# sair-lab/AirSLAM

Hardware: AMD Instinct MI355X
Metric: stereo detect+match pairs/sec (2x PLNet @512x512 internal: points + lines, junctions on the left + LightGlue match) (higher is better)
Workload: dtype fp16

## Files before the change

### airslam_amd/_lib.py

```python
from __future__ import annotations

import ctypes as C
import os

_HERE = os.path.dirname(os.path.abspath(__file__))
LIB_PATH = os.path.join(_HERE, "libairfe.so")


class Tuning(C.Structure):
    _fields_ = [(n, C.c_int) for n in (
        "fuse_lg_block", "gemm_small_max_m", "gemm8_min_m", "gemmr_min_m", "gemmr_wgs", "qkv_pair", "block_min_m", "lgb_tokens", "sg_kenc_gemm",
        "fold_qkv", "overlap_lines", "kf_graph", "kf_spec_rows", "fuse_dec", "assign_fused", "fold_out_proj", "desc_gather_stream", "copy_wgs")] + [("reserved", C.c_int * 5)]


class Cfg(C.Structure):
    _fields_ = [
        ("device", C.c_int), ("precision", C.c_int), ("max_batch", C.c_int), ("enc_chunk", C.c_int),
        ("max_keypoints", C.c_int), ("keypoint_threshold", C.c_float), ("remove_borders", C.c_int),
        ("nms_radius", C.c_int), ("line_threshold", C.c_float), ("line_length_threshold", C.c_float),
        ("matcher", C.c_int), ("image_width", C.c_int), ("image_height", C.c_int), ("sinkhorn_iters", C.c_int),
        ("superpoint_pack", C.c_char_p), ("plnet_s1_pack", C.c_char_p), ("lightglue_pack", C.c_char_p),
        ("superglue_pack", C.c_char_p), ("matcher_precision", C.c_int), ("line_precision", C.c_int), ("check_launches", C.c_int),
        ("tuning", C.POINTER(Tuning)),
    ]


class Stage0(C.Structure):
    _fields_ = [(n, C.c_void_p) for n in (
        "juncs_pred", "lines_pred", "iskeep", "idx_junc_to_end_min", "idx_junc_to_end_max",
        "loi_features", "loi_features_thin", "loi_features_aux")]


class BowdbFilter(C.Structure):
    _fields_ = [("ratio", C.c_float), ("min_words", C.c_int), ("d_max_index", C.c_void_p), ("d_exclude", C.c_void_p), ("exclude_words", C.c_int)]


class RelocCfg(C.Structure):
    _fields_ = [("ratio", C.c_float), ("min_words", C.c_int), ("K", C.c_int), ("outlier_rejection", C.c_int), ("min_inlier", C.c_int),
                ("pose_refinement", C.c_int), ("cam", C.c_double * 5), ("thr", C.c_double * 2)]


class LoopCfg(C.Structure):
    _fields_ = [("ratio", C.c_float), ("min_words", C.c_int), ("K", C.c_int), ("outlier_rejection", C.c_int), ("distance_rate", C.c_double),
                ("min_matches", C.c_int), ("min_points", C.c_int), ("min_inliers", C.c_int), ("cam", C.c_double * 5), ("thr", C.c_double * 2)]


class SeqPolicy(C.Structure):
    _fields_ = [("min_init_stereo_feature", C.c_int), ("min_num_match", C.c_int), ("max_num_match", C.c_int), ("tracking_point_rate", C.c_float),
                ("tracking_parallax_rate", C.c_float), ("min_x_diff", C.c_double), ("max_x_diff", C.c_double), ("max_y_diff", C.c_double),
                ("image_width", C.c_int), ("image_height", C.c_int)]


class SeqFrame(C.Structure):
    _fields_ = ([(n, C.c_int) for n in ("frame_type", "candidate", "promoted", "dropped", "enough_match", "good_stereo_point", "n_left", "n_right", "n_lines_left",
                                        "n_lines_right", "n_junctions", "n_stereo", "n_matches")] + [("_pad", C.c_int)]
                + [(n, C.c_void_p) for n in ("features_left", "features_right", "lines_left", "lines_right", "junctions", "stereo_idx", "stereo_score", "matches_idx",
                                             "matches_score")])


class DebugLinearArgs(C.Structure):
    _fields_ = ([(n, C.c_int) for n in ("prec", "M", "K", "K1", "N")] + [(n, C.c_void_p) for n in ("x1", "x2", "w", "b")]
                + [("epi", C.c_int), ("act", C.c_int), ("rowidx", C.c_void_p), ("src_rows", C.c_int), ("rot_cos", C.c_void_p), ("rot_sin", C.c_void_p),
                   ("Np", C.c_int), ("H", C.c_int), ("x32", C.c_void_p), ("d2s_hc", C.c_int), ("d2s_wc", C.c_int), ("flag", C.c_void_p),
                   ("kernel", C.c_int), ("gr_wgs", C.c_int), ("out", C.c_void_p), ("out2", C.c_void_p)])


class DebugLgBlockArgs(C.Structure):
    _fields_ = ([("prec", C.c_int), ("M", C.c_int)] + [(n, C.c_void_p) for n in ("attn", "x32", "xb", "wo", "bo", "w1", "b1", "gamma", "beta", "w2", "b2")]
                + [(n, C.c_int) for n in ("relu", "tokens_per_wg", "mixed", "nqk_n")]
                + [(n, C.c_void_p) for n in ("nqk_w", "nqk_b", "nv_w", "nv_b", "rot_cos", "rot_sin")]
                + [("Np", C.c_int)] + [(n, C.c_void_p) for n in ("q", "k", "vt")] + [("rows_past", C.c_int * 5)])


class DebugConvArgs(C.Structure):
    _fields_ = ([(n, C.c_void_p) for n in ("x", "img", "w1a", "b1a", "w", "b")] + [(n, C.c_int) for n in ("cin", "cout", "B", "H", "W", "pool", "out_pad", "relu", "wgs")]
                + [("y_words", C.c_size_t), ("y_raw", C.c_void_p)])


class DebugLgPrepareArgs(C.Structure):
    _fields_ = ([(n, C.c_int) for n in ("prec", "B", "cap", "ld", "kp_off", "normalize")] + [(n, C.c_float) for n in ("cx", "cy", "linv")]
                + [(n, C.c_void_p) for n in ("f0", "f1", "n0", "n1", "wr", "f0x", "f1x")] + [(n, C.c_int) for n in ("n0x", "n1x", "slack_rows", "rows")]
                + [(n, C.c_void_p) for n in ("x32", "xb", "rot_cos", "rot_sin", "lens")] + [("rows_past", C.c_int)])


class DebugLgAssignArgs(C.Structure):
    _fields_ = ([(n, C.c_int) for n in ("prec", "B", "n")] + [(n, C.c_void_p) for n in ("md", "x32", "w")] + [("b", C.c_float), ("lens", C.c_void_p), ("cap", C.c_int),
                ("thr", C.c_float), ("form", C.c_int)]
                + [(n, C.c_void_p) for n in ("pad", "z", "sim", "scores", "rowlse", "collse", "rowval", "rowarg", "colarg", "idx", "score", "nmatch")])


class DebugAttentionArgs(C.Structure):
    _fields_ = ([(n, C.c_int) for n in ("prec", "S", "H", "n", "cross")] + [(n, C.c_void_p) for n in ("q", "k", "v", "lens")]
                + [("canary", C.c_int), ("raw", C.c_int), ("out", C.c_void_p), ("Np", C.c_int), ("rows_past", C.c_int)])


class DebugDetectorTailArgs(C.Structure):
    _fields_ = ([(n, C.c_int) for n in ("B", "Bs", "h", "w", "cap")] + [(n, C.c_void_p) for n in ("heat", "act", "feat", "feat1", "n", "n1", "nms_map", "keep", "cand_cnt")]
                + [("nms_map_written", C.c_int)])


class DebugLinePostArgs(C.Structure):
    _fields_ = ([(n, C.c_int) for n in ("B", "nj", "ld", "h", "w", "capL", "capJ", "from_plane")]
                + [(n, C.c_void_p) for n in ("la", "sc", "m2", "heat", "lines", "nlines", "nfound", "junc", "njunc", "jfound", "jmap")])


class DebugLineMidArgs(C.Structure):
    _fields_ = ([(n, C.c_int) for n in ("B", "j2l", "s1_form", "wgs")]
                + [(n, C.c_void_p) for n in ("juncs_pred", "lines_pred", "thin", "aux", "loi", "iskeep_in", "idx_min_in", "idx_max_in", "iskeep", "idx_min", "idx_max", "counts",
                                             "keep", "pairs", "rep", "head4", "prop4", "ridx", "proj", "lines_adjusted", "scores_line", "table_dirty")])


class DebugS0DecodeArgs(C.Structure):
    _fields_ = ([(n, C.c_int) for n in ("B", "mode", "ld", "off", "want_ta8", "want_loi", "want_jnms", "prec", "wgs")] + [(n, C.c_void_p) for n in ("rows", "x", "w", "b")]
                + [("stage_floats", C.c_size_t)] + [(n, C.c_void_p) for n in ("stage", "jloc", "joff", "jnms", "ta8", "loi", "head_rows")])


SIGNATURES = {
    "airfe_copy_rows_dev": (C.c_int, [C.c_void_p, C.c_int, C.c_void_p, C.c_void_p, C.c_void_p, C.c_void_p, C.c_void_p, C.c_void_p]),
    "airfe_pack_rows_dev": (C.c_int, [C.c_void_p, C.c_int, C.c_void_p, C.c_void_p, C.c_void_p, C.c_void_p, C.c_void_p, C.c_void_p, C.c_void_p]),
    "airfe_seq_default_policy": (None, [C.POINTER(SeqPolicy)]),
    "airfe_seq_add_keyframe_check": (C.c_int, [C.POINTER(SeqPolicy), C.c_void_p, C.c_int, C.c_void_p, C.c_int, C.c_void_p, C.c_int]),
    "airfe_seq_good_stereo_points": (C.c_int, [C.POINTER(SeqPolicy), C.c_void_p, C.c_void_p, C.c_void_p, C.c_int]),
    "airfe_seq_create": (C.c_int, [C.c_void_p, C.c_void_p, C.c_int, C.POINTER(SeqPolicy), C.c_int, C.c_int, C.c_void_p, C.c_void_p, C.c_void_p, C.POINTER(C.c_void_p)]),
    "airfe_seq_destroy": (None, [C.c_void_p]),
    "airfe_seq_last_error": (C.c_char_p, [C.c_void_p]),
    "airfe_seq_begin": (C.c_int, [C.c_void_p, C.c_void_p, C.c_void_p, C.c_int, C.c_int, C.c_int, C.c_size_t]),
    "airfe_seq_end": (C.c_int, [C.c_void_p, C.POINTER(SeqFrame)]),
    "airfe_seq_step": (C.c_int, [C.c_void_p, C.c_void_p, C.c_void_p, C.c_int, C.c_int, C.c_int, C.c_size_t, C.POINTER(SeqFrame)]),
    "airfe_seq_stream": (C.c_void_p, [C.c_void_p]),
    "airfe_seq_set_outlier_rejection": (C.c_int, [C.c_void_p, C.c_int]),
    "airfe_seq_wall_split": (C.c_int, [C.c_void_p, C.POINTER(C.c_double), C.POINTER(C.c_double), C.POINTER(C.c_double), C.POINTER(C.c_int), C.POINTER(C.c_int)]),
    "airfe_default_cfg": (None, [C.POINTER(Cfg)]),
    "airfe_default_tuning": (None, [C.POINTER(Tuning)]),
    "airfe_debug_fail_next_launch": (C.c_int, [C.c_void_p, C.c_int]),
    "airfe_create": (C.c_int, [C.POINTER(Cfg), C.POINTER(C.c_void_p)]),
    "airfe_destroy": (None, [C.c_void_p]),
    "airfe_last_error": (C.c_char_p, [C.c_void_p]),
    "airfe_detect_points": (C.c_int, [C.c_void_p, C.c_void_p, C.c_int, C.c_int, C.c_int, C.c_void_p, C.c_int,
                                      C.POINTER(C.c_int)]),
    "airfe_has_line_branch": (C.c_int, [C.c_void_p]),
    "airfe_detect_plnet": (C.c_int, [C.c_void_p, C.c_void_p, C.c_int, C.c_int, C.c_int, C.POINTER(Stage0), C.c_void_p,
                                     C.c_int, C.POINTER(C.c_int), C.c_void_p, C.c_int, C.POINTER(C.c_int), C.c_void_p,
                                     C.c_int, C.POINTER(C.c_int), C.c_int]),
    "airfe_stereo_keyframe": (C.c_int, [C.c_void_p, C.c_void_p, C.c_void_p, C.c_int, C.c_int, C.c_int, C.c_void_p, C.c_void_p, C.c_int,
                                        C.POINTER(C.c_int), C.POINTER(C.c_int), C.c_void_p, C.c_void_p, C.c_int, C.POINTER(C.c_int),
                                        C.POINTER(C.c_int), C.c_void_p, C.c_int, C.POINTER(C.c_int), C.c_void_p, C.c_void_p, C.c_int,
                                        C.POINTER(C.c_int)]),
    "airfe_stereo_keyframe_tracked": (C.c_int, [C.c_void_p, C.c_void_p, C.c_void_p, C.c_int, C.c_int, C.c_int, C.c_void_p, C.c_void_p, C.c_int,
                                                C.POINTER(C.c_int), C.POINTER(C.c_int), C.c_void_p, C.c_void_p, C.c_int, C.POINTER(C.c_int),
                                                C.POINTER(C.c_int), C.c_void_p, C.c_int, C.POINTER(C.c_int), C.c_void_p, C.c_void_p, C.c_int,
                                                C.POINTER(C.c_int), C.c_void_p, C.c_int, C.c_void_p, C.c_void_p, C.POINTER(C.c_int)]),
    "airfe_track_frame": (C.c_int, [C.c_void_p, C.c_void_p, C.c_int, C.c_int, C.c_int, C.c_void_p, C.c_int, C.c_void_p, C.c_int, C.POINTER(C.c_int),
                                    C.c_void_p, C.c_void_p, C.c_int, C.POINTER(C.c_int)]),
    "airfe_promote_frame": (C.c_int, [C.c_void_p, C.c_void_p, C.c_int, C.c_int, C.c_int, C.c_void_p, C.c_int, C.POINTER(C.c_int), C.c_void_p, C.c_void_p, C.c_int,
                                      C.POINTER(C.c_int)]),
    "airfe_adopt_reference": (C.c_int, [C.c_void_p]),
    "airfe_match_lightglue": (C.c_int, [C.c_void_p, C.c_void_p, C.c_int, C.c_void_p, C.c_int, C.c_void_p, C.c_void_p,
                                        C.c_int, C.POINTER(C.c_int)]),
    "airfe_match_superglue": (C.c_int, [C.c_void_p, C.c_void_p, C.c_int, C.c_void_p, C.c_int, C.c_void_p, C.c_void_p,
                                        C.c_void_p, C.c_void_p]),
    "airfe_assign_points_to_lines": (C.c_int, [C.c_void_p, C.c_void_p, C.c_int, C.c_void_p, C.c_int, C.c_void_p, C.c_void_p,
                                               C.c_void_p, C.c_int, C.c_void_p]),
    "airfe_match_lines": (C.c_int, [C.c_void_p, C.c_void_p, C.c_void_p, C.c_int, C.c_int, C.c_void_p, C.c_void_p, C.c_int, C.c_int,
                                    C.c_void_p, C.c_int, C.c_void_p]),
    "airfe_bow_load": (C.c_int, [C.c_void_p, C.c_void_p, C.c_void_p, C.c_void_p, C.c_void_p, C.c_void_p, C.c_int]),
    "airfe_bow_transform": (C.c_int, [C.c_void_p, C.c_void_p, C.c_int, C.c_void_p, C.c_void_p]),
    "airfe_bow_transform_dev": (C.c_int, [C.c_void_p, C.c_void_p, C.c_int, C.c_void_p, C.c_void_p, C.c_void_p]),
    "airfe_bow_vector": (C.c_int, [C.c_void_p, C.c_void_p, C.c_int, C.c_void_p, C.c_void_p, C.POINTER(C.c_int), C.c_void_p]),
    "airfe_bow_vector_batch_dev": (C.c_int, [C.c_void_p, C.c_void_p, C.c_void_p, C.c_int, C.c_int] + [C.c_void_p] * 5),
    "airfe_bowdb_create": (C.c_int, [C.c_void_p, C.c_int, C.c_int, C.c_int, C.POINTER(C.c_void_p)]),
    "airfe_bowdb_destroy": (C.c_int, [C.c_void_p]),
    "airfe_bowdb_clear": (C.c_int, [C.c_void_p]),
    "airfe_bowdb_size": (C.c_int, [C.c_void_p]),
    "airfe_bowdb_add_batch_dev": (C.c_int, [C.c_void_p] * 6 + [C.c_int, C.c_int, C.c_void_p]),
    "airfe_bowdb_add": (C.c_int, [C.c_void_p] * 6 + [C.c_int, C.c_int]),
    "airfe_bowdb_query_batch_dev": (C.c_int, [C.c_void_p] * 4 + [C.c_int, C.c_int, C.POINTER(BowdbFilter)] + [C.c_void_p] * 3 + [C.c_int] + [C.c_void_p] * 4),
    "airfe_bowdb_topk_dev": (C.c_int, [C.c_void_p] * 4 + [C.c_int, C.c_int, C.c_int, C.c_void_p, C.c_void_p, C.c_void_p]),
    "airfe_bowdb_match_candidates_batch_dev": (C.c_int, [C.c_void_p] * 4 + [C.c_int, C.c_int, C.c_void_p, C.c_int, C.c_int] + [C.c_void_p] * 3 + [C.c_int] + [C.c_void_p] * 3),
    "airfe_bowdb_attach_map": (C.c_int, [C.c_void_p, C.c_int]),
    "airfe_bowdb_set_points_dev": (C.c_int, [C.c_void_p, C.c_int, C.c_int, C.c_void_p, C.c_void_p]),
    "airfe_bowdb_set_points": (C.c_int, [C.c_void_p, C.c_int, C.c_int, C.c_void_p]),
    "airfe_bowdb_get_points": (C.c_int, [C.c_void_p, C.c_int, C.c_int, C.c_void_p]),
    "airfe_bowdb_set_covisibility": (C.c_int, [C.c_void_p, C.c_void_p, C.c_void_p, C.c_void_p, C.c_int]),
    "airfe_bowdb_get_covisibility": (C.c_int, [C.c_void_p, C.c_void_p, C.c_void_p, C.c_void_p, C.c_int, C.POINTER(C.c_int)]),
    "airfe_bowdb_set_positions": (C.c_int, [C.c_void_p, C.c_int, C.c_int, C.c_void_p]),
    "airfe_bowdb_group_dev": (C.c_int, [C.c_void_p, C.c_int] + [C.c_void_p] * 3 + [C.c_int] * 3 + [C.c_void_p] * 8),
    "airfe_relocalize_batch_dev": (C.c_int, [C.c_void_p, C.c_void_p, C.POINTER(RelocCfg), C.c_void_p, C.c_void_p, C.c_int, C.c_int] + [C.c_void_p] * 9 +
                                   [C.c_int] + [C.c_void_p] * 3),
    "airfe_bowdb_set_poses": (C.c_int, [C.c_void_p, C.c_int, C.c_int, C.c_void_p]),
    "airfe_bowdb_get_poses": (C.c_int, [C.c_void_p, C.c_int, C.c_int, C.c_void_p]),
    "airfe_bowdb_set_u_right_dev": (C.c_int, [C.c_void_p, C.c_int, C.c_int, C.c_void_p, C.c_void_p]),
    "airfe_bowdb_set_u_right": (C.c_int, [C.c_void_p, C.c_int, C.c_int, C.c_void_p]),
    "airfe_bowdb_get_u_right": (C.c_int, [C.c_void_p, C.c_int, C.c_int, C.c_void_p]),
    "airfe_bowdb_attach_point_ids": (C.c_int, [C.c_void_p, C.c_int]),
    "airfe_bowdb_set_point_ids_dev": (C.c_int, [C.c_void_p, C.c_int, C.c_int, C.c_void_p, C.c_void_p]),
    "airfe_bowdb_set_point_ids": (C.c_int, [C.c_void_p, C.c_int, C.c_int, C.c_void_p]),
    "airfe_bowdb_get_point_ids": (C.c_int, [C.c_void_p, C.c_int, C.c_int, C.c_void_p]),
    "airfe_bowdb_build_covisibility_dev": (C.c_int, [C.c_void_p, C.c_void_p, C.c_void_p]),
    "airfe_bowdb_build_covisibility": (C.c_int, [C.c_void_p, C.POINTER(C.c_int)]),
    "airfe_bowdb_query_stored_batch_dev": (C.c_int, [C.c_void_p, C.c_void_p, C.c_int, C.c_float, C.c_int, C.c_int] + [C.c_void_p] * 3 + [C.c_int] +
                                           [C.c_void_p] * 4),
    "airfe_loop_detect_batch_dev": (C.c_int, [C.c_void_p, C.c_void_p, C.POINTER(LoopCfg), C.c_void_p, C.c_int] + [C.c_void_p] * 10 + [C.c_int] +
                                    [C.c_void_p] * 3),
    "airfe_set_rectify_maps": (C.c_int, [C.c_void_p, C.c_int, C.c_void_p, C.c_void_p, C.c_int, C.c_int]),
    "airfe_rectify_detect_points": (C.c_int, [C.c_void_p, C.c_int, C.c_void_p, C.c_int, C.c_int, C.c_int, C.c_void_p, C.c_void_p, C.c_int,
                                              C.POINTER(C.c_int)]),
    "airfe_rectify_batch_dev": (C.c_int, [C.c_void_p, C.c_int, C.c_void_p, C.c_int, C.c_int, C.c_int, C.c_int, C.c_size_t, C.c_void_p,
                                          C.c_int, C.c_size_t, C.c_void_p]),
    "airfe_detect_points_batch_dev": (C.c_int, [C.c_void_p, C.c_void_p, C.c_int, C.c_int, C.c_int, C.c_int, C.c_size_t,
                                                C.c_void_p, C.c_int, C.c_void_p, C.c_void_p]),
    "airfe_match_lightglue_batch_dev": (C.c_int, [C.c_void_p, C.c_void_p, C.c_void_p, C.c_void_p, C.c_void_p, C.c_int,
                                                  C.c_int, C.c_void_p, C.c_void_p, C.c_int, C.c_void_p, C.c_void_p]),
    "airfe_match_superglue_batch_dev": (C.c_int, [C.c_void_p, C.c_void_p, C.c_void_p, C.c_void_p, C.c_void_p, C.c_int, C.c_int,
                                                  C.c_void_p, C.c_void_p, C.c_void_p, C.c_void_p, C.c_void_p]),
    "airfe_stereo_batch_dev": (C.c_int, [C.c_void_p, C.c_void_p, C.c_void_p, C.c_int, C.c_int, C.c_int, C.c_int,
                                         C.c_size_t, C.c_void_p, C.c_void_p, C.c_int, C.c_void_p, C.c_void_p, C.c_void_p,
                                         C.c_void_p, C.c_int, C.c_void_p, C.c_void_p]),
    "airfe_detect_plnet_batch_dev": (C.c_int, [C.c_void_p, C.c_void_p, C.c_int, C.c_int, C.c_int, C.c_int, C.c_size_t, C.c_void_p,
                                               C.c_int, C.c_void_p, C.c_void_p, C.c_int, C.c_void_p, C.c_void_p, C.c_int, C.c_void_p,
                                               C.c_int, C.c_void_p, C.c_void_p]),
    "airfe_stereo_plnet_batch_dev": (C.c_int, [C.c_void_p, C.c_void_p, C.c_void_p, C.c_int, C.c_int, C.c_int, C.c_int, C.c_size_t,
                                               C.c_void_p, C.c_void_p, C.c_int, C.c_void_p, C.c_void_p, C.c_void_p, C.c_int, C.c_void_p,
                                               C.c_void_p, C.c_int, C.c_void_p, C.c_void_p, C.c_void_p, C.c_void_p, C.c_int, C.c_void_p,
                                               C.c_void_p]),
    "airfe_debug_plnet_j2l": (C.c_int, [C.c_void_p, C.c_int, C.c_void_p, C.c_void_p, C.c_void_p]),
    "airfe_assign_points_to_lines_batch_dev": (C.c_int, [C.c_void_p, C.c_void_p, C.c_void_p, C.c_int, C.c_void_p, C.c_void_p, C.c_int, C.c_int,
                                                         C.c_void_p, C.c_void_p, C.c_void_p, C.c_int, C.c_void_p, C.c_void_p]),
    "airfe_match_lines_batch_dev": (C.c_int, [C.c_void_p] + [C.c_void_p] * 8 + [C.c_int, C.c_int, C.c_void_p, C.c_void_p, C.c_int, C.c_int,
                                              C.c_void_p, C.c_void_p, C.c_void_p, C.c_int, C.c_void_p, C.c_void_p]),
    "airfe_fundamental_ransac": (C.c_int, [C.c_void_p, C.c_void_p, C.c_int, C.c_void_p, C.c_int, C.c_void_p, C.c_void_p, C.c_int, C.POINTER(C.c_int)]),
    "airfe_fundamental_ransac_batch_dev": (C.c_int, [C.c_void_p, C.c_void_p, C.c_void_p, C.c_void_p, C.c_void_p, C.c_int, C.c_int, C.c_void_p, C.c_void_p,
                                                     C.c_int, C.c_void_p, C.c_void_p, C.c_void_p]),
    "airfe_set_outlier_rejection": (C.c_int, [C.c_void_p, C.c_int]),
    "airfe_pnp_ransac": (C.c_int, [C.c_void_p, C.c_void_p, C.c_void_p, C.c_int, C.c_void_p, C.c_void_p, C.c_void_p, C.c_void_p, C.POINTER(C.c_int)]),
    "airfe_pnp_ransac_batch_dev": (C.c_int, [C.c_void_p, C.c_void_p, C.c_void_p, C.c_void_p, C.c_int, C.c_int, C.c_void_p, C.c_void_p, C.c_void_p,
                                             C.c_void_p, C.c_void_p, C.c_void_p]),
    "airfe_stereo_points": (C.c_int, [C.c_void_p, C.c_void_p, C.c_void_p, C.c_int, C.c_void_p, C.c_int, C.c_void_p, C.c_int, C.c_void_p, C.c_void_p,
                                      C.c_void_p, C.POINTER(C.c_int)]),
    "airfe_stereo_points_batch_dev": (C.c_int, [C.c_void_p] * 6 + [C.c_int, C.c_int, C.c_void_p, C.c_void_p, C.c_int] + [C.c_void_p] * 5),
    "airfe_stereo_lines": (C.c_int, [C.c_void_p, C.c_void_p, C.c_void_p, C.c_int, C.c_void_p, C.c_int] + [C.c_void_p] * 8),
    "airfe_stereo_lines_batch_dev": (C.c_int, [C.c_void_p] * 6 + [C.c_int, C.c_void_p, C.c_void_p, C.c_int] + [C.c_void_p] * 7),
    "airfe_stereo_line_landmarks_batch_dev": (C.c_int, [C.c_void_p] * 6 + [C.c_int] + [C.c_void_p] * 4 + [C.c_int, C.c_void_p, C.c_void_p, C.c_int,
                                                        C.c_void_p, C.c_int] + [C.c_void_p] * 8 + [C.c_int] + [C.c_void_p] * 8),
    "airfe_track_pose_batch_dev": (C.c_int, [C.c_void_p, C.c_void_p, C.c_void_p, C.c_int, C.c_void_p, C.c_int, C.c_void_p, C.c_void_p, C.c_int, C.c_int,
                                             C.c_void_p, C.c_void_p, C.c_void_p, C.c_void_p, C.c_void_p]),
    "airfe_frame_optimize": (C.c_int, [C.c_void_p, C.c_void_p, C.c_void_p, C.c_int] + [C.c_void_p] * 7 + [C.POINTER(C.c_int)]),
    "airfe_frame_optimize_batch_dev": (C.c_int, [C.c_void_p, C.c_void_p, C.c_void_p, C.c_void_p, C.c_int, C.c_int] + [C.c_void_p] * 9),
    "airfe_track_pose_opt_batch_dev": (C.c_int, [C.c_void_p, C.c_void_p, C.c_void_p, C.c_int, C.c_void_p, C.c_int, C.c_void_p, C.c_int, C.c_void_p,
                                                 C.c_void_p, C.c_int, C.c_int] + [C.c_void_p] * 9),
    "airfe_sync": (C.c_int, [C.c_void_p]),
    "airfe_superglue_status": (C.c_int, [C.c_void_p, C.c_void_p]),
    "airfe_profile_enable": (C.c_int, [C.c_void_p, C.c_int]),
    "airfe_profile_stages": (C.c_int, []),
    "airfe_profile_stage_name": (C.c_char_p, [C.c_int]),
    "airfe_profile_read": (C.c_int, [C.c_void_p, C.c_void_p, C.c_void_p, C.c_void_p, C.c_void_p]),
    "airfe_debug_detector_maps": (C.c_int, [C.c_void_p, C.c_int, C.c_void_p, C.c_void_p, C.c_void_p]),
    "airfe_debug_lightglue_scores": (C.c_int, [C.c_void_p, C.c_void_p, C.c_int, C.c_void_p, C.c_int, C.c_void_p]),
    "airfe_debug_superglue_scores": (C.c_int, [C.c_void_p, C.c_void_p, C.c_int, C.c_void_p, C.c_int, C.c_void_p]),
    "airfe_debug_lg_filter": (C.c_int, [C.c_void_p, C.c_void_p, C.c_int, C.c_int, C.c_void_p, C.c_void_p, C.c_int, C.POINTER(C.c_int)]),
    "airfe_debug_sg_decode": (C.c_int, [C.c_void_p, C.c_void_p, C.c_int, C.c_int, C.c_void_p, C.c_void_p, C.c_void_p, C.c_void_p]),
    "airfe_debug_sg_sinkhorn": (C.c_int, [C.c_void_p, C.c_void_p, C.c_void_p, C.c_int, C.c_int, C.c_float, C.c_int, C.c_int, C.c_void_p, C.POINTER(C.c_int)]),
    "airfe_debug_detector_tail": (C.c_int, [C.c_void_p, C.POINTER(DebugDetectorTailArgs)]),
    "airfe_debug_line_post": (C.c_int, [C.c_void_p, C.POINTER(DebugLinePostArgs)]),
    "airfe_debug_junctions_topk": (C.c_int, [C.c_void_p, C.c_void_p, C.c_void_p, C.c_int, C.c_void_p]),
    "airfe_debug_line_mid": (C.c_int, [C.c_void_p, C.POINTER(DebugLineMidArgs)]),
    "airfe_debug_s0_decode": (C.c_int, [C.c_void_p, C.POINTER(DebugS0DecodeArgs)]),
    "airfe_debug_lg_prepare": (C.c_int, [C.c_void_p, C.POINTER(DebugLgPrepareArgs)]),
    "airfe_debug_lg_assign": (C.c_int, [C.c_void_p, C.POINTER(DebugLgAssignArgs)]),
    "airfe_debug_plnet_stage0": (C.c_int, [C.c_void_p] + [C.c_void_p] * 10),
    "airfe_debug_plnet_s1": (C.c_int, [C.c_void_p, C.POINTER(Stage0), C.c_void_p, C.c_void_p, C.c_int, C.POINTER(C.c_int)]),
    "airfe_debug_plnet_s1_last": (C.c_int, [C.c_void_p, C.c_void_p, C.c_void_p, C.c_int, C.POINTER(C.c_int)]),
    "airfe_debug_preprocess": (C.c_int, [C.c_void_p, C.c_void_p, C.c_int, C.c_int, C.c_int, C.c_void_p]),
    "airfe_debug_conv3x3": (C.c_int, [C.c_void_p, C.c_void_p, C.c_int, C.c_int, C.c_int, C.c_int, C.c_void_p, C.c_void_p,
                                      C.c_int, C.c_int, C.c_void_p]),
    "airfe_debug_conv": (C.c_int, [C.c_void_p, C.POINTER(DebugConvArgs)]),
    "airfe_debug_trace": (C.c_int, [C.c_void_p, C.c_int]),
    "airfe_debug_trace_stop": (C.c_int, [C.c_void_p, C.c_int]),
    "airfe_debug_trace_buffer": (C.c_int, [C.c_void_p, C.c_int, C.c_void_p, C.c_size_t]),
    "airfe_debug_trace_slots": (C.c_int, [C.c_void_p]),
    "airfe_debug_trace_slot": (C.c_int, [C.c_void_p, C.c_int, C.c_char_p, C.c_int, C.POINTER(C.c_uint), C.POINTER(C.c_uint), C.POINTER(C.c_uint)]),
    "airfe_debug_trace_read": (C.c_int, [C.c_void_p, C.c_void_p, C.c_void_p, C.c_void_p]),
    "airfe_debug_gemm": (C.c_int, [C.c_void_p, C.c_void_p, C.c_int, C.c_int, C.c_void_p, C.c_void_p, C.c_int, C.c_int,
                                   C.c_void_p]),
    "airfe_debug_linear": (C.c_int, [C.c_void_p, C.POINTER(DebugLinearArgs)]),
    "airfe_debug_qkv": (C.c_int, [C.c_void_p] + [C.c_int] * 3 + [C.c_void_p] * 3 + [C.c_int] + [C.c_void_p] * 4 + [C.c_int] * 2 + [C.c_void_p] * 3),
    "airfe_debug_lg_block": (C.c_int, [C.c_void_p, C.POINTER(DebugLgBlockArgs)]),
    "airfe_debug_ln_gelu": (C.c_int, [C.c_void_p, C.c_int, C.c_void_p, C.c_void_p, C.c_void_p, C.c_int]),
    "airfe_debug_attention_args": (C.c_int, [C.c_void_p, C.POINTER(DebugAttentionArgs)]),
    "airfe_debug_attention": (C.c_int, [C.c_void_p, C.c_void_p, C.c_void_p, C.c_void_p, C.c_void_p, C.c_int, C.c_int, C.c_int, C.c_int, C.c_void_p]),
}

_lib = None


def lib() -> C.CDLL:
    global _lib
    if _lib is None:
        if not os.path.exists(LIB_PATH):
            raise RuntimeError(
                f"{LIB_PATH} is missing: build it with `python -m airslam_amd.build` "
                "(hipcc, gfx950).  airslam_amd has no CPU fallback.")
        try:
            import torch
        except Exception:
            pass
        l = C.CDLL(LIB_PATH)
        for name, (res, args) in SIGNATURES.items():
            fn = getattr(l, name)
            fn.restype = res
            fn.argtypes = args
        _lib = l
    return _lib
```

### airslam_amd/api.py

```python
from __future__ import annotations

import ctypes as C
import os
import tempfile
from typing import Dict, Optional

import numpy as np

from . import _lib, weights as W

FEAT = 259


def _pack_arg(x, tmpfiles) -> Optional[bytes]:
    if x is None:
        return None
    if isinstance(x, (str, bytes, os.PathLike)):
        return os.fsencode(x)
    f = tempfile.NamedTemporaryFile(suffix=".airfe", delete=False)
    f.close()
    W.save_pack(f.name, x)
    tmpfiles.append(f.name)
    return f.name.encode()

# ... 355 lines not shown
        n0, n1 = np.ascontiguousarray(n0, np.int32), np.ascontiguousarray(n1, np.int32)
        b, cap, ld = f0.shape
        bt = 2 if second is not None else b
        rows = 2 * bt * self.np_rows + int(slack_rows)
        out = {"x32": np.empty((rows, 256), np.float32), "xb": np.empty((rows, 256), np.float32), "rot_cos": np.empty((rows, 32), np.float32),
               "rot_sin": np.empty((rows, 32), np.float32), "lens": np.empty((2 * bt,), np.int32)}
        cx, cy, linv = normalize if normalize is not None else (0.0, 0.0, 1.0)
        a = _lib.DebugLgPrepareArgs(prec=prec, B=b, cap=cap, ld=ld, kp_off=kp_off, normalize=int(normalize is not None), cx=cx, cy=cy, linv=linv,
                                    f0=f0.ctypes.data, f1=f1.ctypes.data, n0=n0.ctypes.data, n1=n1.ctypes.data, wr=wr.ctypes.data, slack_rows=int(slack_rows),
                                    rows=rows, **{k: v.ctypes.data for k, v in out.items()})
        if second is not None:
            x0, x1 = f32(second[0]).reshape(-1, ld), f32(second[1]).reshape(-1, ld)
            k0, k1 = np.zeros((max(len(x0), 1), ld), np.float32), np.zeros((max(len(x1), 1), ld), np.float32)
            k0[:len(x0)], k1[:len(x1)] = x0, x1
            a.f0x, a.f1x, a.n0x, a.n1x = k0.ctypes.data, k1.ctypes.data, len(x0), len(x1)
        self._chk(self._l.airfe_debug_lg_prepare(self._h, C.byref(a)), "airfe_debug_lg_prepare")
        out["rows_past"], out["Np"] = int(a.rows_past), self.np_rows
        return out

    def debug_lg_assign(self, md, x32, lens, w, b, prec, form, cap=None, thr=0.1, pad=None):
        f32 = lambda t: np.ascontiguousarray(t, np.float32)
        md, x32, w = f32(md), f32(x32), f32(w)
        lens = np.ascontiguousarray(lens, np.int32).reshape(-1)
        s, n, _ = md.shape
        bb = s // 2
        cap = self.np_rows if cap is None else int(cap)
        out = {"z": np.empty((s, n), np.float32), "sim": np.empty((bb, n, n), np.float32), "scores": np.empty((bb, n, n), np.float32),
               "rowlse": np.empty((bb, n), np.float32), "collse": np.empty((bb, n), np.float32), "rowval": np.empty((bb, n), np.float32),
               "rowarg": np.empty((bb, n), np.int32), "colarg": np.empty((bb, n), np.int32), "idx": np.empty((bb, cap, 2), np.int32),
               "score": np.empty((bb, cap), np.float32), "nmatch": np.empty((bb,), np.int32)}
        assert x32.shape == md.shape and len(lens) == s and s % 2 == 0
        a = _lib.DebugLgAssignArgs(prec=prec, B=bb, n=n, md=md.ctypes.data, x32=x32.ctypes.data, w=w.ctypes.data, b=float(b), lens=lens.ctypes.data, cap=cap,
                                   thr=float(thr), form=int(form), **{k: v.ctypes.data for k, v in out.items()})
        if pad is not None:
            pad = f32(pad)
            a.pad = pad.ctypes.data
        self._chk(self._l.airfe_debug_lg_assign(self._h, C.byref(a)), "airfe_debug_lg_assign")
        return out

    def detector_maps(self, b: int = 1):
        heat = np.empty((b, 512, 512), np.float32)
        nms = np.empty((b, 512, 512), np.float32)
        desc = np.empty((b, 64, 64, 256), np.float32)
        self._chk(self._l.airfe_debug_detector_maps(self._h, b, heat.ctypes.data, nms.ctypes.data, desc.ctypes.data),
                  "airfe_debug_detector_maps")
        return heat, nms, desc

    def debug_detector_tail(self, heat, act, cap, Bs=0, h=512, w=512, sentinel=7.0, want_keep=True):
        heat, act = np.ascontiguousarray(heat, np.float32), np.ascontiguousarray(act, np.float32)
        b = heat.shape[0]
        assert heat.shape == (b, 512, 512) and act.shape == (b, 64, 64, 256)
        b0 = Bs if Bs else b
        feat, n = np.full((b0, cap, FEAT), sentinel, np.float32), np.full((b0,), -1, np.int32)
        feat1, n1 = np.full((b - b0, cap, FEAT), sentinel, np.float32), np.full((b - b0,), -1, np.int32)
        nms = np.full((b, 512, 512), np.nan, np.float32)
        keep = np.zeros((b, 64, 64), np.uint64) if want_keep and self.cfg.nms_radius == 4 else None
        cnt = np.full((b,), -1, np.int32)
        a = _lib.DebugDetectorTailArgs(B=b, Bs=int(Bs), h=int(h), w=int(w), cap=int(cap), heat=heat.ctypes.data, act=act.ctypes.data, feat=feat.ctypes.data, n=n.ctypes.data,
                                       nms_map=nms.ctypes.data, cand_cnt=cnt.ctypes.data)
        if Bs:
            a.feat1, a.n1 = feat1.ctypes.data, n1.ctypes.data
        if keep is not None:
            a.keep = keep.ctypes.data
        self._chk(self._l.airfe_debug_detector_tail(self._h, C.byref(a)), "airfe_debug_detector_tail")
        return {"feat": np.concatenate([feat, feat1]), "n": np.concatenate([n, n1]), "cand_cnt": cnt, "keep": keep, "nms_map": nms if a.nms_map_written else None}

    def debug_line_post(self, la, sc, m2, heat, cap_lines, cap_junctions, nj=None, from_plane=False, h=512, w=512, sentinel=7.0, jmap=None):
        la, sc, heat = np.ascontiguousarray(la, np.float32), np.ascontiguousarray(sc, np.float32), np.ascontiguousarray(heat, np.float32)
        m2 = np.ascontiguousarray(m2, np.int32).reshape(-1)
        b, ld = sc.shape
        nj = b if nj is None else int(nj)
        assert la.shape == (b, ld, 4) and heat.shape == (b, 512, 512) and len(m2) == b
        out = {"lines": np.full((b, cap_lines, 4), sentinel, np.float64), "nlines": np.full((b,), -1, np.int32), "nfound": np.full((b,), -1, np.int32),
               "junc": np.full((nj, cap_junctions, FEAT), sentinel, np.float32), "njunc": np.full((nj,), -1, np.int32), "jfound": np.full((nj,), -1, np.int32)}
        a = _lib.DebugLinePostArgs(B=b, nj=nj, ld=ld, h=int(h), w=int(w), capL=int(cap_lines), capJ=int(cap_junctions), from_plane=int(bool(from_plane)), la=la.ctypes.data,
                                   sc=sc.ctypes.data, m2=m2.ctypes.data, heat=heat.ctypes.data, **{k: v.ctypes.data for k, v in out.items()})
        if jmap is not None:
            jmap = np.ascontiguousarray(jmap, np.uint8)
            assert jmap.shape == (nj, 512, 512)
            a.jmap = jmap.ctypes.data
        self._chk(self._l.airfe_debug_line_post(self._h, C.byref(a)), "airfe_debug_line_post")
        return out

    def debug_line_mid(self, juncs_pred, lines_pred, thin, aux, loi, iskeep=None, idx_min=None, idx_max=None, j2l=0, s1_form=2, wgs=0):
        f = lambda x: np.ascontiguousarray(x, np.float32)
        juncs_pred, lines_pred, thin, aux, loi = f(juncs_pred), f(lines_pred), f(thin), f(aux), f(loi)
        b, n, cap = juncs_pred.shape[0], 3 * 128 * 128, 45056
        assert juncs_pred.shape == (b, 300, 2) and lines_pred.shape == (b, n, 4) and thin.shape == aux.shape == (b, 4, 128, 128) and loi.shape == (b, 128 * 128, 128)
        poison = lambda shape, dt: np.full(shape, -1, np.int32).view(dt) if dt == np.float32 else np.full(shape, -1, np.int32)
        out = {"iskeep": poison((b, n), np.float32), "idx_min": poison((b, n), np.float32), "idx_max": poison((b, n), np.float32), "counts": poison((b, 2), np.int32),
               "keep": poison((b, n), np.int32), "pairs": poison((b, cap, 2), np.int32), "rep": poison((b, cap), np.int32), "head4": poison((b, cap, 4), np.float32),
               "prop4": poison((b, cap, 4), np.float32), "ridx": poison((b, 300, 4), np.int32), "proj": poison((b, 300, 256), np.float32),
               "lines_adjusted": poison((b, cap, 4), np.float32), "scores_line": poison((b, cap), np.float32), "table_dirty": poison((b,), np.int32)}
        a = _lib.DebugLineMidArgs(B=b, j2l=int(j2l), s1_form=int(s1_form), wgs=int(wgs), juncs_pred=juncs_pred.ctypes.data, lines_pred=lines_pred.ctypes.data,
                                  thin=thin.ctypes.data, aux=aux.ctypes.data, loi=loi.ctypes.data, **{k: v.ctypes.data for k, v in out.items()})
        ins = [None if x is None else f(x) for x in (iskeep, idx_min, idx_max)]
        for name, x in zip(("iskeep_in", "idx_min_in", "idx_max_in"), ins):
            if x is not None:
                assert x.shape == (b, n)
                setattr(a, name, x.ctypes.data)
        self._chk(self._l.airfe_debug_line_mid(self._h, C.byref(a)), "airfe_debug_line_mid")
        return out

    S0_STAGE = {"lines_pred": (600, 3 * 16384 * 4), "thin": (600 + 7 * 3 * 16384, 4 * 16384), "aux": (600 + 7 * 3 * 16384 + 4 * 16384, 4 * 16384)}
    S0_STAGE_FLOATS = (600 + 7 * 3 * 16384 + 8 * 16384 + 63) // 64 * 64

    def debug_s0_decode(self, rows=None, ld=160, off=128, ta8=True, loi=False, jnms=True, x=None, w=None, b=None, prec=1, wgs=0, two_pass=False):
        f = lambda t: np.ascontiguousarray(t, np.float32)
        npx, sf = 128 * 128, self.S0_STAGE_FLOATS
        a = _lib.DebugS0DecodeArgs(want_ta8=int(bool(ta8)), want_loi=int(bool(loi)), want_jnms=int(bool(jnms)), prec=int(prec), wgs=int(wgs), stage_floats=sf)
        if rows is not None:
            assert x is None and not two_pass
            rows = f(rows)
            bb = rows.shape[0]
            assert rows.shape == (bb, npx, ld)
            a.mode, a.ld, a.off, a.rows = 0, int(ld), int(off), rows.ctypes.data
        else:
            x, w, b = f(x), f(w), f(b)
            bb = x.shape[0] // npx
            assert x.shape == (bb * npx, 128) and w.shape == (17, 128) and b.shape == (17,)
            a.mode, a.x, a.w, a.b = (2 if two_pass else 1), x.ctypes.data, w.ctypes.data, b.ctypes.data
        poison = lambda *shape: np.full(shape, -1, np.int32).view(np.float32)
        out = {"stage": poison(bb, sf), "jloc": poison(bb, 128, 128), "joff": poison(bb, 2, 128, 128), "jnms": poison(bb, 128, 128), "ta8": poison(bb, npx, 8),
               "loi": poison(128, 128, 128)}
        if two_pass:
            out["head_rows"] = poison(bb, npx, 32)
        a.B = bb
        for k, v in out.items():
            setattr(a, k, v.ctypes.data)
        self._chk(self._l.airfe_debug_s0_decode(self._h, C.byref(a)), "airfe_debug_s0_decode")
        for k, (o, n) in self.S0_STAGE.items():
            v = out["stage"][:, o:o + n]
            out[k] = v.reshape(bb, 3 * npx, 4) if k == "lines_pred" else v.reshape(bb, 4, 128, 128)
        return out

    def debug_junctions_topk(self, jloc, joff):
        jloc, joff = np.ascontiguousarray(jloc, np.float32), np.ascontiguousarray(joff, np.float32)
        b = jloc.shape[0]
        assert jloc.shape == (b, 128, 128) and joff.shape == (b, 2, 128, 128)
        out = np.full((b, 300, 2), np.nan, np.float32)
        self._chk(self._l.airfe_debug_junctions_topk(self._h, jloc.ctypes.data, joff.ctypes.data, b, out.ctypes.data), "airfe_debug_junctions_topk")
        return out

    def debug_preprocess(self, gray):
        gray = np.ascontiguousarray(gray, np.uint8)
        out = np.empty((512, 512), np.float32)
        self._chk(self._l.airfe_debug_preprocess(self._h, gray.ctypes.data, gray.shape[0], gray.shape[1], gray.strides[0],
                                                 out.ctypes.data), "airfe_debug_preprocess")
        return out

    def debug_conv3x3(self, x, w, b, pool=False):
        x = np.ascontiguousarray(x, np.float32); w = np.ascontiguousarray(w, np.float32); b = np.ascontiguousarray(b, np.float32)
        bb, cin, hh, ww = x.shape
        cout = w.shape[0]
        ho, wo = (hh // 2, ww // 2) if pool else (hh, ww)
        y = np.empty((bb, cout, ho, wo), np.float32)
        self._chk(self._l.airfe_debug_conv3x3(self._h, x.ctypes.data, bb, cin, hh, ww, w.ctypes.data, b.ctypes.data, cout,
                                              int(pool), y.ctypes.data), "airfe_debug_conv3x3")
        return y

    def debug_conv(self, w, b, prec, x=None, img=None, w1a=None, b1a=None, pool=False, out_pad=1, relu=True, wgs=256):
        f32 = lambda t: None if t is None else np.ascontiguousarray(t, np.float32)
        x, img, w1a, b1a, w, b = map(f32, (x, img, w1a, b1a, w, b))
        src = x if x is not None else img
        bb, hh, ww = src.shape[0], src.shape[-2], src.shape[-1]
        cout, cin = w.shape[0], w.shape[1]
# ... 698 lines not shown
```

### airslam_amd/csrc/airfe.hip

```cpp
#include "airfe_host.h"

namespace airfe_host {
thread_local std::string g_err;

int fail(airfe_ctx* c, const std::string& m) {
  if (c) c->err = m;
  g_err = m;
  return 1;
}

int fail_noexcept(airfe_ctx* c, const char* what, const char* detail) noexcept {
  try {
    std::string m = std::string("airfe: C++ exception at the C boundary (") + what + "): " + (detail ? detail : "unknown");
    if (c) c->err = m;
    g_err = m;
  } catch (...) {
  }
  return 1;
}

int launch_status(airfe_ctx* c) {
  std::string m;
  if (c->launch_err.empty()) {
    const hipError_t e = hipGetLastError();
// ... 705 lines not shown


int airfe_has_line_branch(const airfe_ctx* c) { return c && c->has_s0 && c->has_s1; }

static int upload_stage0(airfe_ctx* c, const airfe_plnet_stage0* s0, hipStream_t st) {
  c->wf_counted = false;
  const size_t NP = KEEP_CAP;
  float* d = c->s0_stage;
  HIPCHK(c, hipMemcpyAsync(d + SG_JUNCS, s0->juncs_pred, 600 * 4, hipMemcpyHostToDevice, st));
  HIPCHK(c, hipMemcpyAsync(d + SG_LP, s0->lines_pred, NP * 16, hipMemcpyHostToDevice, st));
  HIPCHK(c, hipMemcpyAsync(d + SG_KEEP, s0->iskeep, NP * 4, hipMemcpyHostToDevice, st));
  HIPCHK(c, hipMemcpyAsync(d + SG_MIN, s0->idx_junc_to_end_min, NP * 4, hipMemcpyHostToDevice, st));
  HIPCHK(c, hipMemcpyAsync(d + SG_MAX, s0->idx_junc_to_end_max, NP * 4, hipMemcpyHostToDevice, st));
  HIPCHK(c, hipMemcpyAsync(c->s0_loi, s0->loi_features, (size_t)128 * 128 * 128 * 4, hipMemcpyHostToDevice, st));
  HIPCHK(c, hipMemcpyAsync(d + SG_THIN, s0->loi_features_thin, (size_t)4 * 128 * 128 * 4, hipMemcpyHostToDevice, st));
  HIPCHK(c, hipMemcpyAsync(d + SG_AUX, s0->loi_features_aux, (size_t)4 * 128 * 128 * 4, hipMemcpyHostToDevice, st));
  return 0;
}

int airfe_detect_plnet(airfe_ctx* c, const uint8_t* gray, int h, int w, int stride, const airfe_plnet_stage0* s0, float* feat,
                       int cap, int* n, double* lines, int capL, int* nlines, float* junc, int capJ, int* njunc,
                       int want_junctions) try {
  AIRFE_ENTER(c);
  if (nlines) *nlines = 0;
  if (njunc) *njunc = 0;
  const bool lines_on = (s0 || c->has_s0);
  if (!lines_on) return airfe_detect_points(c, gray, h, w, stride, feat, cap, n);
  if (!c->has_s1) return fail(c, "PLNet stage-1 weights were not loaded (cfg.plnet_s1_pack)");
  if (cap < c->cfg.max_keypoints) return fail(c, "feature capacity < max_keypoints");
  hipStream_t st = c->stream;
  if (upload_image(c, gray, h, w, stride)) return 1;
  if (detect_dev(c, c->st_img.p, 1, h, w, stride, (size_t)h * stride, c->st_feat0, c->Np, c->st_n0, st)) return 1;
  if (s0) {
    if (upload_stage0(c, s0, st)) return 1;
  } else if (line_branch_dev(c, st, 0, 1, false)) {
    return 1;
  }
  int* nl_d = c->d_nlines;
  int *nj_d = c->d_njunc, *njf_d = c->d_njunc + c->Lmax;
  if (line_tail_dev(c, 0, 1, s0 ? c->s0_loi : nullptr, h, w, c->d_lines, LINE_CAP, nl_d, nl_d + c->Lmax, c->junc_feat, JUNC_CAP, nj_d, njf_d,
                    want_junctions ? 1 : 0, st))
    return 1;
  const size_t fbytes = 64 + (size_t)c->cfg.max_keypoints * AIRFE_FEAT_DIM * 4;
  if (ensure_pin(c, fbytes + 64)) return 1;
  int* cnt = reinterpret_cast<int*>(c->pin + fbytes);
  cnt[0] = cnt[1] = cnt[2] = 0;
  HIPCHK(c, hipMemcpyAsync(c->pin, c->io_in, fbytes, hipMemcpyDeviceToHost, st));
  HIPCHK(c, hipMemcpyAsync(cnt, nl_d, 4, hipMemcpyDeviceToHost, st));
  if (want_junctions) {
    HIPCHK(c, hipMemcpyAsync(cnt + 1, nj_d, 4, hipMemcpyDeviceToHost, st));
    HIPCHK(c, hipMemcpyAsync(cnt + 2, njf_d, 4, hipMemcpyDeviceToHost, st));
  }
  HIPCHK(c, hipStreamSynchronize(st));
  if (saturation_status(c)) return 1;
  const int nn = std::min(*reinterpret_cast<const int*>(c->pin), c->cfg.max_keypoints);
  if (nn > 0) memcpy(feat, c->pin + 64, (size_t)nn * AIRFE_FEAT_DIM * 4);
  *n = nn;
  const int nl = cnt[0], nj = cnt[1], njf = cnt[2];
  if (njf > JUNC_CAP) return fail(c, "detect_plnet: more junctions than the device arena holds (JUNC_CAP)");
  if (nl > capL || nj > capJ) return fail(c, "detect_plnet: lines / junctions do not fit the caller's buffers (capL, capJ)");
  const size_t lb = (nl > 0 && lines) ? (size_t)nl * 32 : 0, jb = (nj > 0 && junc) ? (size_t)nj * AIRFE_FEAT_DIM * 4 : 0;
  if (lb + jb) {
    if (ensure_pin(c, lb + jb)) return 1;
    if (lb) HIPCHK(c, hipMemcpyAsync(c->pin, c->d_lines, lb, hipMemcpyDeviceToHost, st));
    if (jb) HIPCHK(c, hipMemcpyAsync(c->pin + lb, c->junc_feat, jb, hipMemcpyDeviceToHost, st));
    HIPCHK(c, hipStreamSynchronize(st));
    if (lb) memcpy(lines, c->pin, lb);
    if (jb) memcpy(junc, c->pin + lb, jb);
  }
  if (nlines) *nlines = nl;
  if (njunc) *njunc = nj;
  return 0;
} AIRFE_CATCH(c)

static int plnet_lines_batch(airfe_ctx* c, int B, int h, int w, double* d_lines, int capL, int* d_nlines, float* d_junc, int capJ,
                             int* d_njunc, int nj, int* d_found, hipStream_t st, int phase = 3) {
  if (!c->has_s0 || !c->has_s1) return fail(c, "the batched PLNet path needs the line branch (line.* in the detector pack) and cfg.plnet_s1_pack");
  if (c->prec == 2) return fail(c, "plnet_lines_batch is the 2-byte batch path (fp32 mode goes image by image: plnet_batch_f32)");
  if (B > c->Lmax) return fail(c, "batch exceeds the line-path arena");
  if (capL < 1 || !d_lines || !d_nlines) return fail(c, "detect_plnet_batch: no line output");
  if (nj < 0 || nj > B || (nj > 0 && (!d_junc || !d_njunc || capJ < 1))) return fail(c, "detect_plnet_batch: bad junction arguments");
  if ((phase & 1) && line_branch_dev(c, st, 0, B, false)) return 1;
  bool partial = false;
  if ((phase & 2) && nj > 0 && !c->desc_dense_valid) {
    dense_desc_head(c, nj, st);
    c->desc_dense_valid = true;
    partial = nj != c->last_B;
  }
  int* lfound = d_found ? d_found : c->d_nlines + c->Lmax;
  int* jfound = d_found ? d_found + B : c->d_njunc + c->Lmax;
  const int rc = line_tail_dev(c, 0, B, nullptr, h, w, d_lines, capL, d_nlines, lfound, d_junc, capJ, d_njunc, jfound, nj, st, phase);
  if (partial) c->desc_dense_valid = false;
  return rc;
}

static int plnet_batch_f32(airfe_ctx* c, const uint8_t* d_gray, int B, int h, int w, int stride, size_t img_stride, float* d_feat, int cap, int* d_n,
                           double* d_lines, int capL, int* d_nlines, float* d_junc, int capJ, int* d_njunc, int nj, int* lfound, int* jfound, hipStream_t st) {
  if (!c->has_s0 || !c->has_s1) return fail(c, "the batched PLNet path needs the line branch (line.* in the detector pack) and cfg.plnet_s1_pack");
  if (capL < 1 || !d_lines || !d_nlines) return fail(c, "detect_plnet_batch: no line output");
  if (nj < 0 || nj > B || (nj > 0 && (!d_junc || !d_njunc || capJ < 1))) return fail(c, "detect_plnet_batch: bad junction arguments");
  for (int b = 0; b < B; ++b) {
    const bool jn = b < nj;
    const int rc = detect_dev(c, d_gray + (size_t)b * img_stride, 1, h, w, stride, img_stride, d_feat + (size_t)b * cap * AIRFE_FEAT_DIM, cap, d_n + b, st);
    if (rc || line_branch_dev(c, st, 0, 1, false)) return 1;
    if (line_tail_dev(c, 0, 1, nullptr, h, w, d_lines + (size_t)b * capL * 4, capL, d_nlines + b, lfound ? lfound + b : c->d_nlines + c->Lmax,
                      jn ? d_junc + (size_t)b * capJ * AIRFE_FEAT_DIM : nullptr, capJ, jn ? d_njunc + b : nullptr, jn ? (jfound ? jfound + b : c->d_njunc + c->Lmax) : nullptr,
                      jn ? 1 : 0, st, 3))
      return 1;
  }
  return 0;
}

int airfe_detect_plnet_batch_dev(airfe_ctx* c, const uint8_t* d_gray, int B, int h, int w, int stride, size_t img_stride, float* d_feat,
                                 int cap, int* d_n, double* d_lines, int capL, int* d_nlines, float* d_junc, int capJ, int* d_njunc,
                                 int junction_images, int* d_found, void* stream) try {
  AIRFE_ENTER(c);
  hipStream_t st = stream ? (hipStream_t)stream : c->stream;
  if (c->prec == 2)
    return plnet_batch_f32(c, d_gray, B, h, w, stride, img_stride, d_feat, cap, d_n, d_lines, capL, d_nlines, d_junc, capJ, d_njunc, junction_images, d_found,
                           d_found ? d_found + B : nullptr, st);
  if (detect_dev(c, d_gray, B, h, w, stride, img_stride, d_feat, cap, d_n, st)) return 1;
  return plnet_lines_batch(c, B, h, w, d_lines, capL, d_nlines, d_junc, capJ, d_njunc, junction_images, d_found, st);
} AIRFE_CATCH(c)

static int stereo_plnet_dev(airfe_ctx* c, const uint8_t* d_left, const uint8_t* d_right, int B, int h, int w, int stride,
                            size_t img_stride, float* d_featL, float* d_featR, int cap, int* d_nL, int* d_nR, double* d_lines,
                            int capL, int* d_nlines, float* d_juncL, int capJ, int* d_njuncL, int* d_found, int32_t* d_idx,
                            float* d_score, int mcap, int* d_nmatch, hipStream_t st, const std::function<int(hipStream_t)>* after_detect = nullptr,
                            const std::function<int(hipStream_t)>* after_lines = nullptr, const LgSecondPair* x2 = nullptr) {
  if (c->prec == 2) {
    if (x2) return fail(c, "stereo_plnet_batch: the second (temporal) pair rides in a 2-byte forward (precision fp16 / bf16)");
    if (plnet_batch_f32(c, d_left, B, h, w, stride, img_stride, d_featL, cap, d_nL, d_lines, capL, d_nlines, d_juncL, capJ, d_njuncL, d_juncL ? B : 0, d_found,
                        d_found ? d_found + 2 * B : nullptr, st) ||
        plnet_batch_f32(c, d_right, B, h, w, stride, img_stride, d_featR, cap, d_nR, d_lines + (size_t)B * capL * 4, capL, d_nlines + B, nullptr, 0, nullptr, 0,
                        d_found ? d_found + B : nullptr, nullptr, st))
      return 1;
    if (after_detect && (*after_detect)(st)) return 1;
    if (after_lines && (*after_lines)(st)) return 1;
    if (!d_idx) return 0;
    return lightglue_dev(c, d_featL, d_nL, d_featR, d_nR, B, cap, AIRFE_FEAT_DIM, 1, 1, d_idx, d_score, mcap, d_nmatch, nullptr, st, nullptr);
  }
  if (!(2 * B <= c->Dmax))
    return fail(c, "stereo_plnet_batch: needs the one-pass stereo detector (detector + LightGlue packs loaded, 2 B <= 2 max_batch)");
  const uint32_t enc_only = (1u << ST_PREPROCESS) | (1u << ST_CONV1_FUSED) | (1u << ST_CONV3X3_C64);
  const bool overlap = c->overlap_lines && (c->prof_mask & ~enc_only) == 0;
  if (detect_dev2(c, d_left, d_right, B, h, w, stride, img_stride, d_featL, d_featR, cap, d_nL, d_nR, st)) return 1;
  if (after_detect && (!d_idx || !overlap) && (*after_detect)(st)) return 1;
  if (!d_idx) {
    if (plnet_lines_batch(c, 2 * B, h, w, d_lines, capL, d_nlines, d_juncL, capJ, d_njuncL, d_juncL ? B : 0, d_found, st)) return 1;
    return after_lines ? (*after_lines)(st) : 0;
  }
  if (!overlap) {
    if (plnet_lines_batch(c, 2 * B, h, w, d_lines, capL, d_nlines, d_juncL, capJ, d_njuncL, d_juncL ? B : 0, d_found, st)) return 1;
    if (after_lines && (*after_lines)(st)) return 1;
    return lightglue_dev(c, d_featL, d_nL, d_featR, d_nR, B, cap, AIRFE_FEAT_DIM, 1, 1, d_idx, d_score, mcap, d_nmatch, nullptr, st, x2);
  }
  HIPCHK(c, hipEventRecord(c->ev_fork, st));
  HIPCHK(c, hipStreamWaitEvent(c->stream2, c->ev_fork, 0));
  int rc = 0;
  if (after_detect && (*after_detect)(c->stream2)) rc = 1;
  const bool lg_first = B <= 4;
  if (!rc && lg_first) rc = lightglue_dev(c, d_featL, d_nL, d_featR, d_nR, B, cap, AIRFE_FEAT_DIM, 1, 1, d_idx, d_score, mcap, d_nmatch, nullptr, st, x2);
  if (!rc) rc = plnet_lines_batch(c, 2 * B, h, w, d_lines, capL, d_nlines, d_juncL, capJ, d_njuncL, d_juncL ? B : 0, d_found, c->stream2);
  if (!rc && after_lines && (*after_lines)(c->stream2)) rc = 1;
  if (!rc && !lg_first) rc = lightglue_dev(c, d_featL, d_nL, d_featR, d_nR, B, cap, AIRFE_FEAT_DIM, 1, 1, d_idx, d_score, mcap, d_nmatch, nullptr, st, x2);
  HIPCHK(c, hipEventRecord(c->ev_join, c->stream2));
  HIPCHK(c, hipStreamWaitEvent(st, c->ev_join, 0));
// ... 509 lines not shown
```

### airslam_amd/csrc/airfe_debug.hip

```cpp
#include "airfe_host.h"

struct DbgTmp {
  airfe_ctx h;
  DbgTmp() {}
  explicit DbgTmp(int prec) { h.prec = h.pack_prec = prec; }
  ~DbgTmp() { for (void* p : h.allocs) (void)hipFree(p); }
};

static std::vector<uint16_t> dbg_conv_x(const float* x, int B, int cin, int H, int W, int prec) {
  std::vector<uint16_t> xin((size_t)B * (H + 2) * (W + 2) * cin, 0);
  for (int bb = 0; bb < B; ++bb)
    for (int ci = 0; ci < cin; ++ci)
      for (int yy = 0; yy < H; ++yy)
        for (int xx = 0; xx < W; ++xx)
          xin[(((size_t)bb * (H + 2) + yy + 1) * (W + 2) + xx + 1) * cin + ci] = cvt2(x[(((size_t)bb * cin + ci) * H + yy) * W + xx], prec);
  return xin;
}
static std::vector<uint16_t> dbg_conv_slabs(const float* w, int cin, int cout, int prec) {
  const int nci = cin / 64;
  return pack_slabs(cout / 64, 9 * nci, prec, [&](int feat, int s, int k) {
    const int tap = s / nci, cc = s % nci, ci = cc * 64 + k;
    return w[((size_t)feat * cin + ci) * 9 + tap];
  });
}
// ... 13 lines not shown
} AIRFE_CATCH(c)

int airfe_debug_conv3x3(airfe_ctx* c, const float* x, int B, int cin, int H, int W, const float* w, const float* b, int cout,
                        int pool, float* y) try {
  AIRFE_ENTER(c);
  if ((cin != 64 && cin != 128) || cout % 64 || W % 16 || H % 16) return fail(c, "debug_conv3x3: unsupported shape");
  const int prec = c->prec;
  const int Ho = pool ? H / 2 : H, Wo = pool ? W / 2 : W;
  const size_t ywords = (size_t)B * (Ho + 2) * (Wo + 2) * cout;
  DbgTmp t(prec);
  airfe_ctx& tmp = t.h;
  ConvArgs a;
  a.X = dupload(&tmp, dbg_conv_x(x, B, cin, H, W, prec)); a.Wp = dupload(&tmp, dbg_conv_slabs(w, cin, cout, prec));
  a.bias = dupload(&tmp, std::vector<float>(b, b + cout)); a.Y = dalloc<uint16_t>(&tmp, ywords);
  if (!a.X || !a.Wp || !a.bias || !a.Y) return fail(c, "debug_conv3x3: allocation failed");
  a.B = B; a.H = H; a.W = W; a.CIN = cin; a.COUT = cout;
  a.pool = pool; a.out_pad = 1; a.relu = 1;
  launch_conv3x3(prec, a, c->stream);
  HIPCHK(c, hipStreamSynchronize(c->stream));
  std::vector<uint16_t> yo(ywords);
  HIPCHK(c, hipMemcpy(yo.data(), a.Y, ywords * 2, hipMemcpyDeviceToHost));
  for (int bb = 0; bb < B; ++bb)
    for (int co = 0; co < cout; ++co)
      for (int yy = 0; yy < Ho; ++yy)
        for (int xx = 0; xx < Wo; ++xx)
          y[(((size_t)bb * cout + co) * Ho + yy) * Wo + xx] = back2(yo[(((size_t)bb * (Ho + 2) + yy + 1) * (Wo + 2) + xx + 1) * cout + co], prec);
  return 0;
} AIRFE_CATCH(c)

int airfe_debug_fail_next_launch(airfe_ctx* c, int stage) try {
  AIRFE_ENTER(c);
  if (stage < -1 || stage >= ST_COUNT) return fail(c, "debug_fail_next_launch: no such stage");
  c->fail_stage = stage;
  return 0;
} AIRFE_CATCH(c)

int airfe_debug_gemm(airfe_ctx* c, const float* x, int M, int K, const float* w, const float* b, int N, int relu, float* y) try {
  AIRFE_ENTER(c);
  if (K != 128 && K != 256 && K != 512) return fail(c, "debug_gemm: K must be 128, 256 or 512");
  const int prec = c->prec, Mp = (M + 127) / 128 * 128, Np8 = (N + 7) / 8 * 8;
  std::vector<uint16_t> xin((size_t)Mp * K, 0);
  for (size_t i = 0; i < (size_t)M * K; ++i) xin[i] = cvt2(x[i], prec);
  DbgTmp t(prec);
  airfe_ctx& tmp = t.h;
  LinW lw;
  if (!make_linear(&tmp, w, b, K, N, lw)) return fail(c, "debug_gemm: allocation failed");
  uint16_t* dx = dupload(&tmp, xin);
  float* dy = dalloc<float>(&tmp, (size_t)Mp * Np8);
  int rc = 0;
  if (!dx || !dy) rc = fail(c, "debug_gemm: allocation failed");
  if (!rc) {
    GemmArgs g;
    g.X1 = dx; g.ld1 = K; g.K1 = K; g.Wp = lw.w; g.bias = lw.b; g.M = Mp; g.N = N; g.cb_total = lw.cbt;
    g.epi = EPI_STORE_F32; g.act = relu ? ACT_RELU : ACT_NONE; g.out = dy; g.ldo = Np8;
    g.small_max = c->gemm_small_max; g.g8_min = c->gemm8_min; g.gr_min = c->gemmr_min; g.gr_wgs = c->gemmr_wgs;
    launch_gemm(prec, K, false, g, c->stream);
    if (hipStreamSynchronize(c->stream) != hipSuccess) rc = fail(c, "debug_gemm: kernel failed");
  }
  if (!rc) {
    std::vector<float> yo((size_t)Mp * Np8);
    (void)hipMemcpy(yo.data(), dy, yo.size() * 4, hipMemcpyDeviceToHost);
    for (int m = 0; m < M; ++m)
      for (int n = 0; n < N; ++n) y[(size_t)m * N + n] = yo[(size_t)m * Np8 + n];
  }
  return rc;
} AIRFE_CATCH(c)

}

static std::vector<uint16_t> dbg_rows2(const float* x, int rows, int cols, int rows_cap, int prec) {
  std::vector<uint16_t> v((size_t)rows_cap * cols, 0);
  if (x)
    for (size_t i = 0; i < (size_t)rows * cols; ++i) v[i] = cvt2(x[i], prec);
  return v;
}
static std::vector<float> dbg_rows4(const float* x, int rows, int cols, int rows_cap) {
  std::vector<float> v((size_t)rows_cap * cols, 0.f);
  if (x) memcpy(v.data(), x, (size_t)rows * cols * sizeof(float));
  return v;
}
template <class T>
static T* dbg_canary(airfe_ctx* tmp, size_t n) {
  T* p = dalloc<T>(tmp, n, false);
  if (p) (void)hipMemset(p, 0xFF, std::max<size_t>(n, 1) * sizeof(T));
  return p;
}
static void dbg_back2(const std::vector<uint16_t>& v, size_t n, int prec, float* out) {
  for (size_t i = 0; i < n; ++i) out[i] = back2(v[i], prec);
}

extern "C" {

int airfe_debug_conv(airfe_ctx* c, airfe_debug_conv_args* a) try {
  AIRFE_ENTER(c);
  if (!a || !a->w || !a->b || !a->y_raw) return fail(c, "debug_conv: null argument");
  const bool fused = a->img != nullptr;
  if (fused == (a->x != nullptr)) return fail(c, "debug_conv: exactly one of x (plain form) and img (fused conv1a -> conv1b) must be given");
  const int cin = a->cin, cout = a->cout, B = a->B, H = a->H, W = a->W, pool = a->pool, opad = a->out_pad, prec = c->prec;
  if (prec != 0 && prec != 1) return fail(c, "debug_conv: the context's precision must be fp16 or bf16");
  if (a->wgs < 1 || a->wgs > 256) return fail(c, "debug_conv: wgs must lie in 1 .. 256");
  if (cin != 64 && cin != 128) return fail(c, "debug_conv: cin must be 64 or 128");
  if (cout < 64 || cout % 64 || (cin == 128 && cout % 128)) return fail(c, "debug_conv: cout must be a multiple of 64 (of 128 when cin is 128)");
  if (B < 1 || H < 16 || W < 16 || H % 16 || W % 16) return fail(c, "debug_conv: B >= 1, H and W multiples of 16");
  if ((pool != 0 && pool != 1) || (opad != 0 && opad != 1) || (a->relu != 0 && a->relu != 1)) return fail(c, "debug_conv: pool, out_pad and relu are 0 or 1");
  if (pool && !opad) return fail(c, "debug_conv: a pooled layer always feeds another conv (out_pad = 1); pool with out_pad = 0 is no form of the arena");
  if (fused && (cin != 64 || cout != 64 || !pool || !opad || !a->relu || !a->w1a || !a->b1a))
    return fail(c, "debug_conv: the fused form is conv1a -> conv1b: cin = cout = 64, pool = 1, out_pad = 1, relu = 1, w1a and b1a given");
  const int Ho = pool ? H / 2 : H, Wo = pool ? W / 2 : W;
  const size_t guard = (size_t)(Wo + 2 * opad) * cout, words = (size_t)B * (Ho + 2 * opad) * guard, total = words + 2 * guard;
  if (a->y_words != total) return fail(c, "debug_conv: y_words must be (B (Ho + 2 out_pad) + 2) (Wo + 2 out_pad) cout");
  DbgTmp t(prec);
  airfe_ctx& tmp = t.h;
  ConvArgs g;
  if (fused) {
    std::vector<float> im((size_t)B * (H + 2) * (W + 2), 0.f);
    for (int bb = 0; bb < B; ++bb)
      for (int yy = 0; yy < H; ++yy) memcpy(&im[((size_t)bb * (H + 2) + yy + 1) * (W + 2) + 1], a->img + ((size_t)bb * H + yy) * W, (size_t)W * sizeof(float));
    g.img = dupload(&tmp, im);
    g.w1a = dupload(&tmp, std::vector<float>(a->w1a, a->w1a + 64 * 9));
    g.b1a = dupload(&tmp, std::vector<float>(a->b1a, a->b1a + 64));
  } else {
    g.X = dupload(&tmp, dbg_conv_x(a->x, B, cin, H, W, prec));
  }
  g.Wp = dupload(&tmp, dbg_conv_slabs(a->w, cin, cout, prec));
  g.bias = dupload(&tmp, std::vector<float>(a->b, a->b + cout));
  uint16_t* dy = dbg_canary<uint16_t>(&tmp, total);
  if ((fused ? !g.img || !g.w1a || !g.b1a : !g.X) || !g.Wp || !g.bias || !dy) return fail(c, "debug_conv: allocation failed");
  g.Y = dy + guard;
  g.B = B; g.H = H; g.W = W; g.CIN = cin; g.COUT = cout; g.pool = pool; g.out_pad = opad; g.relu = a->relu; g.wgs = a->wgs;
  if (fused) launch_conv64r(prec, g, c->stream);
  else launch_conv3x3(prec, g, c->stream);
  if (hipStreamSynchronize(c->stream) != hipSuccess || launch_status(c)) return fail(c, "debug_conv: kernel failed");
  HIPCHK(c, hipMemcpy(a->y_raw, dy, total * 2, hipMemcpyDeviceToHost));
  return 0;
} AIRFE_CATCH(c)

int airfe_debug_linear(airfe_ctx* c, const airfe_debug_linear_args* a) try {
  AIRFE_ENTER(c);
  if (!a || !a->x1 || !a->w || !a->b || !a->out) return fail(c, "debug_linear: null argument");
  const int prec = a->prec, M = a->M, K = a->K, N = a->N, epi = a->epi, kern = a->kernel, K1 = a->x2 ? a->K1 : K;
  if ((prec != 0 && prec != 1) || M < 1 || N < 1 || (K != 128 && K != 256 && K != 512) || K1 < 32 || K1 % 32 || K1 > K || (a->x2 && K1 == K) ||
      epi < EPI_STORE || epi > EPI_SOFTMAX_D2S || kern < AIRFE_DEBUG_KERNEL_DISPATCH || kern > AIRFE_DEBUG_KERNEL_GEMMR_GATHER128 || (a->act != ACT_NONE && a->act != ACT_RELU))
    return fail(c, "debug_linear: bad argument");
  const bool trans = epi == EPI_HEADS_T, heads = epi == EPI_HEADS || trans, d2s = epi == EPI_SOFTMAX_D2S;
  if (heads && ((a->H != 4 && a->H != 0) || a->Np < 16 || a->Np % 16 || M % a->Np || (epi == EPI_HEADS ? (N != 256 && N != 512) || (N == 512 && !a->out2) : N != 256)))
    return fail(c, "debug_linear: head layouts need H = 4, M = S * Np with Np a multiple of 16, N = 256 (or 512 with out2 for EPI_HEADS)");
  if ((a->rot_cos || a->rot_sin) && (epi != EPI_HEADS || !a->rot_cos || !a->rot_sin)) return fail(c, "debug_linear: rotary is an EPI_HEADS form");
  if (epi == EPI_RESID && (!a->x32 || N % 64)) return fail(c, "debug_linear: EPI_RESID needs x32 and N a multiple of 64");
  if (d2s && (K != 256 || N != 65 || a->x2 || a->rowidx || a->act || a->d2s_hc < 1 || a->d2s_wc < 1 || M % (a->d2s_hc * a->d2s_wc) || M % 16 ||
              (kern != AIRFE_DEBUG_KERNEL_DISPATCH && kern != AIRFE_DEBUG_KERNEL_GEMM8)))
    return fail(c, "debug_linear: EPI_SOFTMAX_D2S is launch_gemm8's head kernel: K = 256, N = 65, dense rows, M = B * hc * wc, M % 16 == 0");
  if (a->rowidx) {
    if (kern != AIRFE_DEBUG_KERNEL_GEMM8 && kern != AIRFE_DEBUG_KERNEL_GEMMR_GATHER && kern != AIRFE_DEBUG_KERNEL_GEMMR_GATHER128)
      return fail(c, "debug_linear: a row gather runs in gemm8, gemmr_gather or gemmr_gather128 only");
    if (a->src_rows < 1) return fail(c, "debug_linear: rowidx needs src_rows");
    for (int r = 0; r < M; ++r)
      if (a->rowidx[r] < 0 || a->rowidx[r] >= a->src_rows) return fail(c, "debug_linear: rowidx entry outside 0 .. src_rows - 1");
  }
  static const int row_tile[7] = {128, 32, 128, 256, 32, 32, 64};
  const int Mp = d2s ? M : (M + row_tile[kern] - 1) / row_tile[kern] * row_tile[kern];
  const int xrows = a->rowidx ? a->src_rows : Mp;
  const int ldo = (epi == EPI_STORE || epi == EPI_STORE_F32) ? (N + 7) / 8 * 8 : N;
  const int Sg = heads ? (Mp + a->Np - 1) / a->Np : 0, S = heads ? M / a->Np : 0;
  DbgTmp t(prec);
  airfe_ctx& tmp = t.h;
  LinW lw;
  if (!make_linear(&tmp, a->w, a->b, K, N, lw)) return fail(c, "debug_linear: allocation failed");
// ... 462 lines not shown
  if (a->h < 1 || a->w < 1 || cap < c->cfg.max_keypoints) return fail(c, "debug_detector_tail: empty image or feature capacity < max_keypoints");
  if (a->keep && c->cfg.nms_radius != 4) return fail(c, "debug_detector_tail: the keep plane exists on the radius-4 path only");
  const size_t px = (size_t)B * R * R, cells = (size_t)B * (R / 8) * (R / 8);
  for (size_t i = 0; i < px; ++i)
    if (!(a->heat[i] >= 0.f && a->heat[i] <= 1.f)) return fail(c, "debug_detector_tail: scores must lie in [0, 1]");
  std::vector<uint16_t> act(cells * 256);
  for (size_t i = 0; i < act.size(); ++i) act[i] = cvt2(a->act[i], c->prec);
  const int B0 = two ? Bs : B, B1 = two ? B - Bs : 0;
  DbgTmp t;
  float* dfeat = dupload(&t.h, std::vector<float>(a->feat, a->feat + (size_t)B0 * cap * AIRFE_FEAT_DIM));
  int* dn = dupload(&t.h, std::vector<int>(a->n, a->n + B0));
  float* dfeat1 = two ? dupload(&t.h, std::vector<float>(a->feat1, a->feat1 + (size_t)B1 * cap * AIRFE_FEAT_DIM)) : nullptr;
  int* dn1 = two ? dupload(&t.h, std::vector<int>(a->n1, a->n1 + B1)) : nullptr;
  if (!dfeat || !dn || (two && (!dfeat1 || !dn1))) return fail(c, "debug_detector_tail: allocation failed");
  hipStream_t st = c->stream;
  clear_saturation(c);
  HIPCHK(c, hipMemcpyAsync(c->heat, a->heat, px * 4, hipMemcpyHostToDevice, st));
  HIPCHK(c, hipMemcpyAsync(c->aDa, act.data(), act.size() * 2, hipMemcpyHostToDevice, st));
  const bool sparse_desc = B > 2 && cap * 4 <= (R / 8) * (R / 8) && cap <= 1024;
  if (!sparse_desc && dense_desc_head(c, B, st)) { (void)hipStreamSynchronize(st); return 1; }
  c->desc_dense_valid = !sparse_desc;
  c->last_B = B;
  const int rc = detect_tail_dev(c, B, Bs, two, sparse_desc, a->h, a->w, dfeat, dfeat1, cap, dn, dn1, st);
  HIPCHK(c, hipStreamSynchronize(st));
  if (rc) return 1;
  if (saturation_status(c)) return 1;
  HIPCHK(c, hipMemcpy(a->feat, dfeat, (size_t)B0 * cap * AIRFE_FEAT_DIM * 4, hipMemcpyDeviceToHost));
  HIPCHK(c, hipMemcpy(a->n, dn, (size_t)B0 * 4, hipMemcpyDeviceToHost));
  if (two) {
    HIPCHK(c, hipMemcpy(a->feat1, dfeat1, (size_t)B1 * cap * AIRFE_FEAT_DIM * 4, hipMemcpyDeviceToHost));
    HIPCHK(c, hipMemcpy(a->n1, dn1, (size_t)B1 * 4, hipMemcpyDeviceToHost));
  }
  a->nms_map_written = c->cfg.nms_radius > 0 && c->nms_map_valid;
  if (a->nms_map && a->nms_map_written) HIPCHK(c, hipMemcpy(a->nms_map, c->heat_nms, px * 4, hipMemcpyDeviceToHost));
  if (a->keep) HIPCHK(c, hipMemcpy(a->keep, c->nms_mask, cells * 8, hipMemcpyDeviceToHost));
  if (a->cand_cnt) HIPCHK(c, hipMemcpy(a->cand_cnt, c->cand_cnt, (size_t)B * 4, hipMemcpyDeviceToHost));
  return 0;
} AIRFE_CATCH(c)

int airfe_debug_line_post(airfe_ctx* c, airfe_debug_line_post_args* a) try {
  AIRFE_ENTER(c);
  if (!c->has_sp || !c->has_s1 || !c->s1_la || !c->jmap) return fail(c, "debug_line_post: the line path is not loaded (cfg.plnet_s1_pack)");
  if (c->cfg.nms_radius != 4) return fail(c, "debug_line_post: both junction score sources exist on the radius-4 path only");
  if (!a || !a->la || !a->sc || !a->m2 || !a->heat || !a->lines || !a->nlines || !a->nfound) return fail(c, "debug_line_post: null argument");
  const int B = a->B, nj = a->nj, ld = a->ld, capL = a->capL, capJ = a->capJ, R = AIRFE_INTERNAL_SIZE;
  if (B < 1 || B > c->Lmax || B > c->Dmax || nj < 0 || nj > B || ld < 1 || ld > LINE_CAP || capL < 1 || capJ < 1 || a->h < 1 || a->w < 1)
    return fail(c, "debug_line_post: bad argument (1 <= B <= the arena's images, 0 <= nj <= B, 1 <= ld <= 45056, capL, capJ >= 1)");
  if (nj > 0 && (!a->junc || !a->njunc || !a->jfound)) return fail(c, "debug_line_post: nj > 0 needs the junction outputs");
  for (int b = 0; b < B; ++b)
    if (a->m2[b] < 0 || a->m2[b] > ld) return fail(c, "debug_line_post: every m2 must lie in 0 .. ld");
  DbgTmp t;
  double* dlines = dupload(&t.h, std::vector<double>(a->lines, a->lines + (size_t)B * capL * 4));
  float* djunc = nj > 0 ? dupload(&t.h, std::vector<float>(a->junc, a->junc + (size_t)nj * capJ * AIRFE_FEAT_DIM)) : nullptr;
  int* dcnt = dbg_canary<int>(&t.h, (size_t)4 * B);
  if (!dlines || (nj > 0 && !djunc) || !dcnt) return fail(c, "debug_line_post: allocation failed");
  hipStream_t st = c->stream;
  clear_saturation(c);
  std::vector<int> counts((size_t)B * LINE_CNT_LD, 0);
  for (int b = 0; b < B; ++b) {
    counts[(size_t)b * LINE_CNT_LD + 1] = a->m2[b];
    HIPCHK(c, hipMemcpyAsync(c->s1_la + (size_t)b * LINE_CAP * 4, a->la + (size_t)b * ld * 4, (size_t)ld * 16, hipMemcpyHostToDevice, st));
    HIPCHK(c, hipMemcpyAsync(c->s1_sc + (size_t)b * LINE_CAP, a->sc + (size_t)b * ld, (size_t)ld * 4, hipMemcpyHostToDevice, st));
  }
  HIPCHK(c, hipMemcpyAsync(c->wf_counts, counts.data(), counts.size() * 4, hipMemcpyHostToDevice, st));
  c->wf_counted = false;
  HIPCHK(c, hipMemcpyAsync(c->heat, a->heat, (size_t)B * R * R * 4, hipMemcpyHostToDevice, st));
  c->nms_map_valid = !a->from_plane;
  launch_nms512_candidates(c->heat, c->nms_map_valid ? c->heat_nms : nullptr, c->nms_mask, B, c->cfg.keypoint_threshold, c->cfg.remove_borders, c->cand, c->cand_cnt,
                           R * R, st);
  const float ws = (float)a->w / (float)R, hs = (float)a->h / (float)R;
  if (nj > 0) launch_zero16(c->jmap, (size_t)nj * R * R, st);
  launch_line_filter(c->s1_la, c->s1_sc, c->wf_counts, c->cfg.remove_borders, c->cfg.line_threshold, c->cfg.line_length_threshold, ws, hs, R, c->jmap, nj, dlines, capL,
                     dcnt, dcnt + B, LINE_CAP, B, st);
  if (nj > 0 && a->jmap) HIPCHK(c, hipMemcpyAsync(c->jmap, a->jmap, (size_t)nj * R * R, hipMemcpyHostToDevice, st));
  if (nj > 0) {
    const bool from_mask = c->cfg.nms_radius > 0 && !c->nms_map_valid;
    const float* hsel = c->cfg.nms_radius > 0 && !from_mask ? c->heat_nms : c->heat;
    const unsigned long long* mask = from_mask ? reinterpret_cast<const unsigned long long*>(c->nms_mask) : nullptr;
    launch_junction_scan(c->jmap, hsel, R, c->cfg.remove_borders, djunc, capJ, dcnt + 2 * B, dcnt + 3 * B, c->d_njunc + 2 * c->Lmax, nj, st, mask);
  }
  HIPCHK(c, hipStreamSynchronize(st));
  if (launch_status(c)) return 1;
  if (saturation_status(c)) return 1;
  HIPCHK(c, hipMemcpy(a->lines, dlines, (size_t)B * capL * 32, hipMemcpyDeviceToHost));
  HIPCHK(c, hipMemcpy(a->nlines, dcnt, (size_t)B * 4, hipMemcpyDeviceToHost));
  HIPCHK(c, hipMemcpy(a->nfound, dcnt + B, (size_t)B * 4, hipMemcpyDeviceToHost));
  if (nj > 0) {
    HIPCHK(c, hipMemcpy(a->junc, djunc, (size_t)nj * capJ * AIRFE_FEAT_DIM * 4, hipMemcpyDeviceToHost));
    HIPCHK(c, hipMemcpy(a->njunc, dcnt + 2 * B, (size_t)nj * 4, hipMemcpyDeviceToHost));
    HIPCHK(c, hipMemcpy(a->jfound, dcnt + 3 * B, (size_t)nj * 4, hipMemcpyDeviceToHost));
  }
  return 0;
} AIRFE_CATCH(c)

int airfe_debug_line_mid(airfe_ctx* c, airfe_debug_line_mid_args* a) try {
  AIRFE_ENTER(c);
  if (!c->has_sp || !c->has_s0 || !c->has_s1 || !c->s0_stage || !c->l_ta8) return fail(c, "debug_line_mid: the line path is not loaded (line.* tensors, cfg.plnet_s1_pack)");
  if (!a || !a->juncs_pred || !a->lines_pred || !a->thin || !a->aux || !a->loi || !a->iskeep || !a->idx_min || !a->idx_max || !a->counts || !a->keep || !a->pairs || !a->rep ||
      !a->head4 || !a->prop4 || !a->ridx || !a->proj || !a->lines_adjusted || !a->scores_line || !a->table_dirty)
    return fail(c, "debug_line_mid: null argument");
  const int B = a->B, form = a->s1_form, NP = KEEP_CAP, NPX = 128 * 128;
  if (B < 1 || B > c->Lmax) return fail(c, "debug_line_mid: 1 <= B <= the arena's images");
  if (a->j2l < 0 || a->j2l > 2 || form < 0 || form > 3) return fail(c, "debug_line_mid: j2l is 0 .. 2, s1_form 0 .. 3");
  if (form <= 1 && B != 1) return fail(c, "debug_line_mid: forms 0 and 1 (CHW tensors, head rows) hold one image");
  if (a->j2l == 0 && (!a->iskeep_in || !a->idx_min_in || !a->idx_max_in)) return fail(c, "debug_line_mid: j2l = 0 needs iskeep_in, idx_min_in and idx_max_in");
  if (a->wgs < 0 || a->wgs > 512) return fail(c, "debug_line_mid: wgs must lie in 0 .. 512");
  if (form == 3)
    for (int i = 0; i < 6; ++i)
      if (!c->s1_wsplit[i]) return fail(c, "debug_line_mid: form 3 needs the split stage-1 weights");
  for (size_t i = 0; i < (size_t)B * 600; ++i)
    if (!std::isfinite(a->juncs_pred[i])) return fail(c, "debug_line_mid: junction coordinates must be finite");
  for (size_t i = 0; i < (size_t)B * NP * 4; ++i)
    if (!std::isfinite(a->lines_pred[i])) return fail(c, "debug_line_mid: proposal coordinates must be finite");
  hipStream_t st = c->stream;
  float* d = c->s0_stage;
  clear_saturation(c);
  std::vector<float> ta8((size_t)B * NPX * 8);
  for (int b = 0; b < B; ++b)
    for (int ch = 0; ch < 8; ++ch) {
      const float* src = (ch < 4 ? a->thin : a->aux) + ((size_t)b * 4 + (ch & 3)) * NPX;
      for (int p = 0; p < NPX; ++p) ta8[((size_t)b * NPX + p) * 8 + ch] = src[p];
    }
  HIPCHK(c, hipMemcpyAsync(c->l_ta8, ta8.data(), ta8.size() * 4, hipMemcpyHostToDevice, st));
  for (int b = 0; b < B; ++b) {
    float* s = d + (size_t)b * SG_STRIDE;
    HIPCHK(c, hipMemcpyAsync(s + SG_JUNCS, a->juncs_pred + (size_t)b * 600, 600 * 4, hipMemcpyHostToDevice, st));
    HIPCHK(c, hipMemcpyAsync(s + SG_LP, a->lines_pred + (size_t)b * NP * 4, (size_t)NP * 16, hipMemcpyHostToDevice, st));
    HIPCHK(c, hipMemcpyAsync(s + SG_THIN, a->thin + (size_t)b * 4 * NPX, (size_t)4 * NPX * 4, hipMemcpyHostToDevice, st));
    HIPCHK(c, hipMemcpyAsync(s + SG_AUX, a->aux + (size_t)b * 4 * NPX, (size_t)4 * NPX * 4, hipMemcpyHostToDevice, st));
    if (a->j2l == 0) {
      HIPCHK(c, hipMemcpyAsync(s + SG_KEEP, a->iskeep_in + (size_t)b * NP, (size_t)NP * 4, hipMemcpyHostToDevice, st));
      HIPCHK(c, hipMemcpyAsync(s + SG_MIN, a->idx_min_in + (size_t)b * NP, (size_t)NP * 4, hipMemcpyHostToDevice, st));
      HIPCHK(c, hipMemcpyAsync(s + SG_MAX, a->idx_max_in + (size_t)b * NP, (size_t)NP * 4, hipMemcpyHostToDevice, st));
    } else {
      HIPCHK(c, hipMemsetAsync(s + SG_KEEP, 0xFF, (size_t)3 * NP * 4, st));
    }
  }
  static_assert(SG_MIN == SG_KEEP + KEEP_CAP && SG_MAX == SG_MIN + KEEP_CAP, "iskeep | min | max are contiguous");
  const size_t L = (size_t)B;
  HIPCHK(c, hipMemsetAsync(c->wf_counts, 0xFF, L * LINE_CNT_LD * 4, st));
  HIPCHK(c, hipMemsetAsync(c->wf_keep, 0xFF, L * KEEP_CAP * 4, st));
  HIPCHK(c, hipMemsetAsync(c->wf_pairs, 0xFF, L * LINE_CAP * 8, st));
  HIPCHK(c, hipMemsetAsync(c->wf_rep, 0xFF, L * LINE_CAP * 4, st));
  HIPCHK(c, hipMemsetAsync(c->wf_prop, 0xFF, L * LINE_CAP * 16, st));
  HIPCHK(c, hipMemsetAsync(c->s1_la, 0xFF, L * LINE_CAP * 16, st));
  HIPCHK(c, hipMemsetAsync(c->s1_sc, 0xFF, L * LINE_CAP * 4, st));
  HIPCHK(c, hipMemsetAsync(c->s1_jfeat, 0xFF, L * 300 * 256 * 4, st));
  HIPCHK(c, hipMemsetAsync(c->l_ridx, 0xFF, L * 1200 * 4, st));
  bool counted = false;
  if (a->j2l) counted = launch_s0_j2l(d + SG_LP, d + SG_JUNCS, 300, NP, 10.0f, d + SG_KEEP, d + SG_MIN, d + SG_MAX, c->wf_counts, B, SG_STRIDE, a->j2l == 1 ? 1 : 0, st);
  if (a->j2l == 2 && !counted) { (void)hipStreamSynchronize(st); return fail(c, "debug_line_mid: the cell search did not leave the per-workgroup counts (the line path's form)"); }
  launch_wireframe(d + SG_KEEP, d + SG_MIN, d + SG_MAX, NP, 300, c->wf_table, c->wf_keep, c->wf_pairs, c->wf_rep, KEEP_CAP, LINE_CAP, c->wf_counts, counted, d + SG_JUNCS,
                   d + SG_LP, c->s1_la, c->wf_prop, B, SG_STRIDE, st);
  c->wf_counted = false;
  HIPCHK(c, hipStreamSynchronize(st));
  if (launch_status(c)) return 1;
  HIPCHK(c, hipMemcpy(a->head4, c->s1_la, L * LINE_CAP * 16, hipMemcpyDeviceToHost));
  if (form != 3) HIPCHK(c, hipMemsetAsync(c->s1_la, 0xFF, L * LINE_CAP * 16, st));
  std::vector<float> chw, head, lrows;
  if (form == 0) {
    chw.resize((size_t)128 * NPX);
    for (int p = 0; p < NPX; ++p)
      for (int ch = 0; ch < 128; ++ch) chw[(size_t)ch * NPX + p] = a->loi[(size_t)p * 128 + ch];
    HIPCHK(c, hipMemcpyAsync(c->s0_loi, chw.data(), chw.size() * 4, hipMemcpyHostToDevice, st));
    launch_plnet_s1(d + SG_JUNCS, d + SG_LP, c->wf_keep, c->wf_pairs, c->wf_rep, c->wf_counts, c->s0_loi, 0, nullptr, nullptr, d + SG_THIN, d + SG_AUX, c->s1_w, c->s1_la,
                    c->s1_sc, KEEP_CAP, LINE_CAP, B, SG_STRIDE, st, a->wgs);
// ... 150 lines not shown
```

### airslam_amd/csrc/airfe_detect.hip

```cpp
#include "airfe_host.h"

namespace airfe_host {

int ensure_tables(airfe_ctx* c, int h, int w) {
  if (c->tab_w == w && c->tab_h == h) return 0;
  const auto xt = resize_table(AIRFE_INTERNAL_SIZE, w), yt = resize_table(AIRFE_INTERNAL_SIZE, h);
  if (c->tab_w != -1) HIPCHK(c, hipDeviceSynchronize());
  HIPCHK(c, hipMemcpyAsync(c->xtab, xt.data(), xt.size() * 4, hipMemcpyHostToDevice, c->stream));
  HIPCHK(c, hipMemcpyAsync(c->ytab, yt.data(), yt.size() * 4, hipMemcpyHostToDevice, c->stream));
  HIPCHK(c, hipStreamSynchronize(c->stream));
  c->tab_w = w;
  c->tab_h = h;
  return 0;
}

int run_conv(airfe_ctx* c, const ConvW& w, const uint16_t* x, uint16_t* y, int B, int H, int W, int pool, int out_pad,
             hipStream_t st) {
  ConvArgs a;
  a.X = x; a.Wp = w.w; a.bias = w.b; a.Y = y;
  a.B = B; a.H = H; a.W = W; a.CIN = w.cin; a.COUT = w.cout;
  a.pool = pool; a.out_pad = out_pad; a.relu = 1;
  const double px = (double)B * H * W;
  const double ob = px / (pool ? 4 : 1) * w.cout * 2;
  {
// ... 150 lines not shown
    if (run_conv(c, c->c4b, c->a4a, c->a4b, B, R / 8, R / 8, 0, 1, st)) return 1;
    if (run_conv(c, c->cPa, c->a4b, c->aPa, B, R / 8, R / 8, 0, 0, st)) return 1;
    if (run_conv(c, c->cDa, c->a4b, c->aDa, B, R / 8, R / 8, 0, 0, st)) return 1;
    const int cells = B * (R / 8) * (R / 8);
    {
      GemmArgs g;
      g.X1 = c->aPa; g.ld1 = 256; g.K1 = 256; g.Wp = c->cPb.w; g.bias = c->cPb.b;
      g.M = cells; g.N = 65; g.cb_total = c->cPb.cbt; g.epi = EPI_STORE_F32; g.out = c->logits; g.ldo = 72;
      g.small_max = c->gemm_small_max; g.g8_min = c->gemm8_min; g.gr_min = c->gemmr_min; g.gr_wgs = c->gemmr_wgs;
      g.epi = EPI_SOFTMAX_D2S; g.out = c->heat; g.d2s_hc = R / 8; g.d2s_wc = R / 8; g.flag = c->sat_flag;
      ProfScope ps(c, ST_HEAD_GEMM, st, 2.0 * cells * 256 * 65, (double)cells * (512 + 256));
      launch_gemm8(c->prec, 256, false, g, st);
    }
    sparse_desc = B > 2 && cap * 4 <= (R / 8) * (R / 8) && cap <= 1024;
    if (!sparse_desc && dense_desc_head(c, B, st)) return 1;
    c->desc_dense_valid = !sparse_desc;
    c->last_B = B;
  }
  return detect_tail_dev(c, B, Bs, d_gray1 != nullptr, sparse_desc, h, w, d_feat, d_feat1, cap, d_n, d_n1, st);
}

int detect_dev(airfe_ctx* c, const uint8_t* d_gray, int B, int h, int w, int stride, size_t img_stride, float* d_feat,
               int cap, int* d_n, hipStream_t st) {
  return detect_dev2(c, d_gray, nullptr, B, h, w, stride, img_stride, d_feat, nullptr, cap, d_n, nullptr, st);
}

void junctions_topk_dev(airfe_ctx* c, int nb, hipStream_t st) {
  const int F = 128, ccap = F * F;
  launch_candidates_nms3(c->l_jloc, nb, F, F, 1e-30f, c->l_cand, c->l_cand_cnt, ccap, st);
  SelectExtra jx;
  jx.sort_all = 1;
  launch_select_list(c->l_cand, c->l_cand_cnt, ccap, nb, F, 300, 320, c->l_sel, c->l_nsel, st, &jx);
  launch_s0_juncs(c->l_sel, c->l_nsel, c->l_joff, c->s0_stage + SG_JUNCS, 300, 320, nb, SG_STRIDE, st);
}

int line_branch_dev(airfe_ctx* c, hipStream_t st, int i0, int nb, bool chw) {
  if (!c->has_s0) return fail(c, "the detector pack carries no line branch (line.* tensors)");
  if (!c->s0_stage) return fail(c, "the line path arena is not allocated (cfg.plnet_s1_pack)");
  if (nb < 1 || nb > c->Lmax || i0 < 0 || i0 + nb > c->Dmax) return fail(c, "line branch: image range outside the arena");
  const int NP = KEEP_CAP, F = 128;
  float* d = c->s0_stage;
  const bool fused = c->prec == 2 || chw;
  if (fused && (nb != 1 || i0 != 0)) return fail(c, "the fused line head (fp32 mode, inspection hook) runs one image at a time");
  c->line_sparse = !fused;
  bool head_done = false;
  if (c->prec == 2) {
    launch_conv3x3_f32(c->f3a, c->f_cL1.w, c->f_cL1.b, c->fL1, 1, F, F, 128, 128, 0, st);
    GemmF32Args g;
    g.X1 = c->fL1; g.ld1 = 128; g.K1 = 128; g.K = 128; g.W = c->f_cLh.w; g.bias = c->f_cLh.b; g.M = F * F; g.N = 145; g.Y = c->l_head; g.ldy = 160;
    launch_gemm_f32(g, st);
  } else {
    if (run_conv(c, c->cL1, c->a3a + (size_t)i0 * (F + 2) * (F + 2) * 128, c->l_feat, nb, F, F, 0, 0, st)) return 1;
    if (!fused && c->fuse_dec) {
      ProfScope ps(c, ST_PL_DECODE, st, 2.0 * nb * F * F * 128 * 17, (double)nb * F * F * (256 + 92));
      launch_s0_head_decode(c->prec, c->l_feat, c->cLh_dec.w, c->cLh_dec.b, d + SG_LP, c->l_jloc, nullptr, c->l_joff, c->l_ta8, nb, SG_STRIDE,
                            st);
      head_done = true;
    } else {
      const LinW& hw = fused ? c->cLh : c->cLh_dec;
      GemmArgs g;
      g.X1 = c->l_feat; g.ld1 = 128; g.K1 = 128; g.Wp = hw.w; g.bias = hw.b;
      g.M = nb * F * F; g.N = hw.N; g.cb_total = hw.cbt; g.epi = EPI_STORE_F32; g.out = fused ? c->l_head : c->l_dec; g.ldo = fused ? 160 : 32;
      g.small_max = c->gemm_small_max; g.g8_min = c->gemm8_min; g.gr_min = c->gemmr_min; g.gr_wgs = c->gemmr_wgs;
      if (!fused) g.small_max = 1 << 30;
      ProfScope ps(c, ST_HEAD_GEMM, st, 2.0 * nb * F * F * 128 * hw.N, (double)nb * F * F * (256 + 4.0 * g.ldo));
      launch_gemm(c->prec, 128, false, g, st);
    }
  }
  {
  ProfScope ps(c, ST_PL_DECODE, st, 0, (double)nb * (128.0 * 128 * (17 * 4 + 3 * 16 + 11 * 4) + 3.0 * 49152 * (16 + 12)));
  if (head_done) {
  } else if (fused)
    launch_s0_decode(c->l_head, 160, 128, d + SG_LP, c->l_jloc, nullptr, c->l_joff, d + SG_THIN, d + SG_AUX, chw ? c->s0_loi : nullptr, c->l_ta8, nb,
                     SG_STRIDE, st);
  else
    launch_s0_decode(c->l_dec, 32, 0, d + SG_LP, c->l_jloc, nullptr, c->l_joff, d + SG_THIN, d + SG_AUX, nullptr, c->l_ta8, nb, SG_STRIDE, st);
  hipStream_t s3 = st;
  junctions_topk_dev(c, nb, s3);
  c->wf_counted = launch_s0_j2l(d + SG_LP, d + SG_JUNCS, 300, NP, 10.0f, d + SG_KEEP, d + SG_MIN, d + SG_MAX, c->wf_counts, nb, SG_STRIDE, chw ? 1 : 0, s3);
  }
  return launch_status(c);
}

int line_tail_dev(airfe_ctx* c, int i0, int nb, const float* loi_chw, int h, int w, double* d_lines, int capL, int* d_nlines, int* d_lfound,
                  float* d_junc, int capJ, int* d_njunc, int* d_jfound, int nj, hipStream_t st, int phase) {
  if (!c->has_s1) return fail(c, "PLNet stage-1 weights were not loaded (cfg.plnet_s1_pack)");
  if (nb < 1 || nb > c->Lmax || nj < 0 || nj > nb) return fail(c, "line path: image range outside the arena");
  const int R = AIRFE_INTERNAL_SIZE, NP = KEEP_CAP;
  float* d = c->s0_stage;
  const float ws = (float)w / (float)R, hs = (float)h / (float)R;
  if (phase & 1) {
  hipStream_t s4 = st;
  if (nj > 0) launch_zero16(c->jmap, (size_t)nj * R * R, s4);
  {
  ProfScope ps(c, ST_PL_STAGE1, st, 0, (double)nb * 49152 * 12);
  launch_wireframe(d + SG_KEEP, d + SG_MIN, d + SG_MAX, NP, 300, c->wf_table, c->wf_keep, c->wf_pairs, c->wf_rep, KEEP_CAP, LINE_CAP,
                   c->wf_counts, c->wf_counted, d + SG_JUNCS, d + SG_LP, c->s1_la, c->wf_prop, nb, SG_STRIDE, s4);
  c->wf_counted = false;
  if (loi_chw) {
    launch_plnet_s1(d + SG_JUNCS, d + SG_LP, c->wf_keep, c->wf_pairs, c->wf_rep, c->wf_counts, loi_chw, 0, nullptr, nullptr, d + SG_THIN, d + SG_AUX,
                    c->s1_w, c->s1_la, c->s1_sc, KEEP_CAP, LINE_CAP, nb, SG_STRIDE, st);
  } else {
    if (c->line_sparse) {
      const int M = nb * 1200, Mp = (M + 255) / 256 * 256;
      hipStream_t s5 = st;
      launch_s1_junc_rows(d + SG_JUNCS, 300, c->l_ridx, nb, SG_STRIDE, s5);
      if (Mp > M) HIPCHK(c, hipMemsetAsync(c->l_ridx + M, 0, (size_t)(Mp - M) * 4, s5));
      GemmArgs g;
      g.X1 = c->l_feat; g.ld1 = 128; g.K1 = 128; g.Wp = c->cLh_loi.w; g.bias = c->cLh_loi.b; g.rowidx = c->l_ridx;
      g.M = Mp; g.N = 128; g.cb_total = c->cLh_loi.cbt; g.epi = EPI_STORE_F32; g.out = c->l_lrows; g.ldo = 128;
      g.gr_wgs = c->gemmr_wgs;
      if (c->desc_gather_stream && Mp >= c->gemmr_min && c->prec != 2 && gemmr_gather128_applicable(g)) launch_gemmr_gather128(c->prec, g, s5);
      else launch_gemm8(c->prec, 128, false, g, s5);
      if (c->cfg.line_precision == 3) launch_s1h_junc_proj(d + SG_JUNCS, c->l_lrows, 300, c->s1_wsplit[4], c->s1_wsplit[5], c->s1_jfeat, nb, SG_STRIDE, s5);
      else launch_s1_junc_proj(d + SG_JUNCS, nullptr, 0, 0, c->l_lrows, 300, c->s1_w[0], c->s1_jfeat, nb, SG_STRIDE, s5);
    } else {
      launch_s1_junc_proj(d + SG_JUNCS, c->l_head, (size_t)128 * 128 * 160, 160, nullptr, 300, c->s1_w[0], c->s1_jfeat, nb, SG_STRIDE, st);
    }
    if (c->cfg.line_precision == 3)
      launch_plnet_s1h(c->wf_pairs, c->wf_counts, c->s1_jfeat, c->l_ta8, c->s1_wsplit, c->s1_w, c->s1_la, c->wf_prop, c->s1_sc, LINE_CAP, nb, st);
    else
      launch_plnet_s1(d + SG_JUNCS, d + SG_LP, c->wf_keep, c->wf_pairs, c->wf_rep, c->wf_counts, nullptr, 0, c->s1_jfeat, c->l_ta8, d + SG_THIN,
                      d + SG_AUX, c->s1_w, c->s1_la, c->s1_sc, KEEP_CAP, LINE_CAP, nb, SG_STRIDE, st);
  }
  }
  ProfScope ps(c, ST_PL_FILTER, st, 0, (double)nb * R * R);
  launch_line_filter(c->s1_la, c->s1_sc, c->wf_counts, c->cfg.remove_borders, c->cfg.line_threshold, c->cfg.line_length_threshold, ws, hs, R,
                     c->jmap, nj, d_lines, capL, d_nlines, d_lfound, LINE_CAP, nb, st);
  }
  if ((phase & 2) && nj > 0) {
    ProfScope ps(c, ST_PL_FILTER, st, 0, (double)nj * R * R * 2);
    const bool from_mask = c->cfg.nms_radius > 0 && !c->nms_map_valid;
    if (from_mask && c->cfg.nms_radius != 4) return fail(c, "line path: the NMS'd score maps of this batch were not kept");
    const float* hsel = (c->cfg.nms_radius > 0 && !from_mask ? c->heat_nms : c->heat) + (size_t)i0 * R * R;
    const unsigned long long* mask = from_mask ? reinterpret_cast<const unsigned long long*>(c->nms_mask) + (size_t)i0 * (R / 8) * (R / 8) : nullptr;
    launch_junction_scan(c->jmap, hsel, R, c->cfg.remove_borders, d_junc, capJ, d_njunc, d_jfound, c->d_njunc + 2 * c->Lmax, nj, st, mask);
    if (!c->desc_dense_valid) return fail(c, "line path: the dense descriptor map of this batch was not made");
    launch_sample_desc(c->desc + (size_t)i0 * (R / 8) * (R / 8) * 256, nj, R / 8, R / 8, d_junc, d_njunc, capJ, ws, hs,
                       c->desc_normalised ? 0 : 1, st);
  }
  return launch_status(c);
}

}
```

### airslam_amd/csrc/airfe_host.h

```cpp
#pragma once
#include "../../include/airfe.h"
#include "../../include/airfe_debug.h"

#include <hip/hip_runtime.h>

#include <algorithm>
#include <cmath>
#include <cstdio>
#include <cstdlib>
#include <cstring>
#include <functional>
#include <map>
#include <string>
#include <vector>

#include "kernels.h"
#include "common.h"

using namespace airfe;


namespace airfe_host {

extern thread_local std::string g_err;
// ... 245 lines not shown
  ProfScope(airfe_ctx* c_, int stage_, hipStream_t st_, double flops, double bytes) : c(c_), st(st_), on((c_->prof_mask >> stage_) & 1u), stage(stage_) {
    if (c->fail_stage == stage) { c->fail_stage = -1; fail_launch_now(st); if (c->cfg.check_launches) note_launch(c, stage); }
    if (!on) return;
    auto get = [&]() {
      hipEvent_t e;
      if (!c->ev_pool.empty()) { e = c->ev_pool.back(); c->ev_pool.pop_back(); }
      else (void)hipEventCreate(&e);
      return e;
    };
    m.stage = stage; m.flops = flops; m.bytes = bytes; m.a = get(); m.b = get();
    (void)hipEventRecord(m.a, st);
  }
  ~ProfScope() {
    if (c->cfg.check_launches) note_launch(c, stage);
    if (!on) return;
    (void)hipEventRecord(m.b, st);
    try { c->marks.push_back(m); } catch (...) { c->ev_pool.clear(); }
  }
};

namespace airfe_host {

#define HIPCHK(ctx, expr)                                                                         \
  do {                                                                                            \
    hipError_t e_ = (expr);                                                                       \
    if (e_ != hipSuccess) {                                                                       \
      (ctx)->err = std::string(#expr) + ": " + hipGetErrorString(e_);                             \
      g_err = (ctx)->err;                                                                         \
      return 1;                                                                                   \
    }                                                                                             \
  } while (0)

int fail(airfe_ctx* c, const std::string& m);
int fail_noexcept(airfe_ctx* c, const char* what, const char* detail) noexcept;
int launch_status(airfe_ctx* c);
int saturation_status(airfe_ctx* c);

template <class T>
T* dalloc(airfe_ctx* c, size_t n, bool zero = true) {
  void* p = nullptr;
  if (hipMalloc(&p, std::max<size_t>(n, 1) * sizeof(T)) != hipSuccess) return nullptr;
  if (zero) (void)hipMemset(p, 0, std::max<size_t>(n, 1) * sizeof(T));
  c->allocs.push_back(p);
  return reinterpret_cast<T*>(p);
}
template <class T>
T* dupload(airfe_ctx* c, const std::vector<T>& v) {
  T* p = dalloc<T>(c, v.size(), false);
  if (p && !v.empty()) (void)hipMemcpy(p, v.data(), v.size() * sizeof(T), hipMemcpyHostToDevice);
  return p;
}

int load_superpoint(airfe_ctx* c, const char* path);
int load_lightglue(airfe_ctx* c, const char* path);
int load_superglue(airfe_ctx* c, const char* path);
int load_plnet_s1(airfe_ctx* c, const char* path);
std::vector<int> resize_table(int dsize, int ssize);
std::vector<uint16_t> pack_slabs(int cbt, int nslab, int prec, const std::function<float(int, int, int)>& get);
uint16_t f2bf(float f);
uint16_t f2h(float f);
float h2f(uint16_t h);
inline uint16_t cvt2(float f, int prec) { return prec == 1 ? f2h(f) : f2bf(f); }
inline float back2(uint16_t v, int prec) {
  if (prec == 1) return h2f(v);
  uint32_t u = (uint32_t)v << 16;
  float f;
  memcpy(&f, &u, 4);
  return f;
}
bool make_linear(airfe_ctx* c, const float* W, const float* bias, int K, int N, LinW& out, float scale = 1.f,
                 const std::function<int(int)>* src_row = nullptr, const std::function<int(int)>* src_col = nullptr);
int ensure_tables(airfe_ctx* c, int h, int w);
int run_conv(airfe_ctx* c, const ConvW& w, const uint16_t* x, uint16_t* y, int B, int H, int W, int pool, int out_pad, hipStream_t st);
int dense_desc_head(airfe_ctx* c, int B, hipStream_t st);
int detect_tail_dev(airfe_ctx* c, int B, int Bs, bool two, bool sparse_desc, int h, int w, float* d_feat, float* d_feat1, int cap, int* d_n, int* d_n1,
                    hipStream_t st);
int detect_dev2(airfe_ctx* c, const uint8_t* d_gray, const uint8_t* d_gray1, int Bs, int h, int w, int stride, size_t img_stride,
                float* d_feat, float* d_feat1, int cap, int* d_n, int* d_n1, hipStream_t st);
int detect_dev(airfe_ctx* c, const uint8_t* d_gray, int B, int h, int w, int stride, size_t img_stride, float* d_feat, int cap, int* d_n, hipStream_t st);
void junctions_topk_dev(airfe_ctx* c, int nb, hipStream_t st);
int line_branch_dev(airfe_ctx* c, hipStream_t st, int i0, int nb, bool chw);
int line_tail_dev(airfe_ctx* c, int i0, int nb, const float* loi_chw, int h, int w, double* d_lines, int capL, int* d_nlines, int* d_lfound,
                  float* d_junc, int capJ, int* d_njunc, int* d_jfound, int nj, hipStream_t st, int phase = 3);
void trace(airfe_ctx* c, hipStream_t st, const char* what, size_t li, const char* blk, const void* p, size_t words, unsigned unit_words);
int trace_finish(airfe_ctx* c, hipStream_t st);
int run_linear(airfe_ctx* c, const LinW& w, const uint16_t* x1, int ld1, int K1, const uint16_t* x2, int ld2, int M, int epi, int act, void* out,
                int ldo, hipStream_t st, bool trans = false, void* out2 = nullptr, float* x32 = nullptr, const float* rc = nullptr, const float* rs = nullptr);
void reset_slack_rows(airfe_ctx* c, int M, hipStream_t st);
struct LgSecondPair { const float *f0, *f1; const int *n0, *n1; };
int lightglue_dev(airfe_ctx* c, const float* f0, const int* n0, const float* f1, const int* n1, int B, int cap, int ld, int kp_off, int normalize,
                  int32_t* d_idx, float* d_score, int mcap, int* d_nmatch, float* scores_out, hipStream_t st, const LgSecondPair* x2 = nullptr);
int superglue_dev(airfe_ctx* c, const float* f0, const int* n0, const float* f1, const int* n1, int B, int cap, int normalize, hipStream_t st);

}

#define AIRFE_CATCH(c)                                                                                                   \
  catch (const std::exception& e_) { return airfe_host::fail_noexcept((c), __func__, e_.what()); }                       \
  catch (...) { return airfe_host::fail_noexcept((c), __func__, nullptr); }
inline int enter_device(airfe_ctx* c) {
  int d = -1;
  if (hipGetDevice(&d) == hipSuccess && d == c->cfg.device) return 0;
  if (hipSetDevice(c->cfg.device) != hipSuccess) return fail(c, "hipSetDevice(cfg.device) failed");
  return 0;
}
#define AIRFE_ENTER(c) do { if (!(c)) return 1; if (enter_device(c)) return 1; } while (0)
int ensure_pin(airfe_ctx* c, size_t bytes);
int upload_image(airfe_ctx* c, const uint8_t* gray, int h, int w, int stride);
inline void clear_saturation(airfe_ctx* c) {
  if (c->sat_host) c->sat_host[0] = c->sat_host[1] = 0;
}
struct DrainOnError {
  airfe_ctx* c; bool armed = false, ref_uploaded = false;
  explicit DrainOnError(airfe_ctx* c_, bool armed_ = false) : c(c_), armed(armed_) { clear_saturation(c_); }
  ~DrainOnError() {
    if (!armed) return;
    (void)hipStreamSynchronize(c->stream);
    (void)hipStreamSynchronize(c->stream2);
    if (ref_uploaded) c->ref_n = -1;
  }
};
int fransac_queue(airfe_ctx* c, const float* d_f0, const float* d_f1, int B, int cap, int32_t* d_idx, float* d_score, int mcap, int* d_nmatch, double* d_F,
                  hipStream_t st);
int pnp_queue(airfe_ctx* c, const float* d_obj, const float* d_img, const int* d_n, int B, int ncap, const double* K, double* d_Twc, double* d_Rt, uint8_t* d_mask,
              int mcap, const int* d_map, int* d_count, hipStream_t st);
int poseopt_queue(airfe_ctx* c, const double* d_X, const double* d_obs, const int* d_n, int B, int ncap, const double* d_Twc0, const double* cam, const double* Tcb,
                  const double* thr, double* d_Twc, double* d_Rt, uint8_t* d_inlier, int mcap, const int* d_map, int* d_num, int lost, int* d_ok, hipStream_t st);
int stereo_lines_queue(airfe_ctx* c, const double* cam, const double* d_left, const int* d_nl, const double* d_right, const int* d_nr, int capL,
                       const int32_t* d_matches, const double* d_Twc, int B, double* d_sel, uint8_t* d_valid, int32_t* d_status, double* d_endpoints,
                       double* d_plucker, int32_t* d_count, hipStream_t st);
```

### airslam_amd/csrc/gemmr_body.h

```cpp
#pragma once
#include "common.h"
#include "kernels.h"
#include "desc_sample.h"

namespace airfe {

constexpr int GR_MT = 2;
constexpr int GR_TT = 16 * GR_MT;
constexpr int GR_XBYTES = GR_TT * 512;
constexpr int GR_RBYTES = 2 * GR_TT * 128;

template <int N>
__device__ __forceinline__ void gr_wait_vm() { asm volatile("s_waitcnt vmcnt(%0)" ::"n"(N) : "memory"); }

__device__ __forceinline__ void gr_glds16(const void* gsrc, unsigned lds_off) {
  unsigned keep;
  asm volatile("s_mov_b32 %0, m0\n\ts_mov_b32 m0, %2\n\ts_nop 0\n\tglobal_load_lds_dwordx4 %1, off\n\ts_mov_b32 m0, %0"
               : "=&s"(keep)
               : "v"(gsrc), "s"(lds_off)
               : "memory");
}

constexpr int GR_SAMPLE_SLOTS = 7;
constexpr int GR_STAGE_LD = 260;
constexpr int GR_STAGE_BYTES = GR_TT * GR_STAGE_LD * 4;
struct GrKeypoint { float x, y; int row, second; };

template <class P, bool TRANS, bool ROT, bool GATHER = false, bool SAMPLE = false>
__device__ __forceinline__ void gemmr_body(const GemmArgs& a, char* smem, int group, int first, int per_group, int ntiles, const DescSample* dsp = nullptr) {
  static_assert(!GATHER || (!TRANS && !ROT), "the gather form is the plain K = 256 linear with fp32 rows out");
  static_assert(!SAMPLE || GATHER, "sampling finishes the gather form's rows");
  constexpr int GR_SLOT = GR_XBYTES + (ROT ? GR_RBYTES : 0);
  constexpr int GR_SLOTS = ROT ? 6 : SAMPLE ? GR_SAMPLE_SLOTS : 8;
  constexpr int PER = ROT ? 3 : 2;
  const int tid = threadIdx.x, lane = tid & 63, l15 = lane & 15, g = lane >> 4;
  const int wave = __builtin_amdgcn_readfirstlane(tid >> 6);
  const int n = first < ntiles ? (ntiles - first + per_group - 1) / per_group : 0;
  if (n == 0) return;

  const int cb = group * 4 + (wave >> 1), tp = wave & 1;
  typename P::vec8 wreg[2][8];
  {
    const int sw = (l15 >> 1) & 7;
    const char* wb = reinterpret_cast<const char*>(a.Wp) + (size_t)cb * 4 * SLAB_BYTES + 2 * tp * 2048 + l15 * 128;
#pragma unroll
    for (int u = 0; u < 2; ++u)
#pragma unroll
      for (int ks = 0; ks < 8; ++ks)
        wreg[u][ks] = __builtin_bit_cast(typename P::vec8, *reinterpret_cast<const uint4*>(
            wb + u * 2048 + (ks >> 1) * SLAB_BYTES + ((((ks & 1) * 4 + g) ^ sw) << 4)));
  }
  f32x4 binit[2];
  float bt[2];
#pragma unroll
  for (int u = 0; u < 2; ++u) {
    binit[u] = *reinterpret_cast<const f32x4*>(a.bias + cb * 64 + tp * 32 + g * 8 + u * 4);
    bt[u] = a.bias[cb * 64 + slab_row_to_feature((2 * tp + u) * 16 + l15)];
  }
  [[maybe_unused]] float* stage = reinterpret_cast<float*>(smem + GR_SLOTS * GR_SLOT);
  [[maybe_unused]] int* idx_lds = reinterpret_cast<int*>(smem + GR_SLOTS * GR_SLOT + (SAMPLE ? GR_STAGE_BYTES : 0));
  [[maybe_unused]] GrKeypoint* kp_lds = reinterpret_cast<GrKeypoint*>(idx_lds + n * GR_TT);
  if constexpr (GATHER) {
    for (int e = tid; e < n * GR_TT; e += 512) {
      const int r = (first + (e >> 5) * per_group) * GR_TT + (e & 31);
      idx_lds[e] = a.rowidx ? a.rowidx[r] : r;
    }
  }
  if constexpr (SAMPLE) {
    const DescSample& ds = *dsp;
    for (int e = tid; e < n * 8; e += 512) {
      const int s = (first + (e >> 3) * per_group) * 8 + (e & 7);
      const int b = s / ds.cap, k = s - b * ds.cap;
      GrKeypoint kp{0.f, 0.f, -1, 0};
      if (b < ds.B) {
        const bool second = ds.feat1 && b >= ds.Bs;
        const int bl = second ? b - ds.Bs : b;
        if (k < (second ? ds.n1 : ds.n)[bl]) {
          const float* f = (second ? ds.feat1 : ds.feat) + ((size_t)bl * ds.cap + k) * 259;
          kp.row = bl * ds.cap + k;
          kp.second = second ? 1 : 0;
          kp.x = f[1];
          kp.y = f[2];
        }
      }
      kp_lds[e] = kp;
    }
  }
  asm volatile("s_waitcnt vmcnt(0)" ::: "memory");
  if constexpr (GATHER) __syncthreads();

  const int ld = a.ld1;
  auto dma = [&](int j, int slot) {
    [[maybe_unused]] const int t = first + j * per_group;
#pragma unroll
    for (int i = 0; i < 2; ++i) {
      const int inst = wave * 2 + i;
      const int r = inst * 2 + (lane >> 5), pp = lane & 31;
      size_t srow;
      if constexpr (GATHER) srow = (size_t)idx_lds[j * GR_TT + r];
      else srow = (size_t)(t * GR_TT + r);
      gr_glds16(a.X1 + srow * ld + ((pp ^ (r & 15)) << 3), (unsigned)(slot * GR_SLOT + inst * 1024));
    }
    if constexpr (ROT) {
      const float* src = (wave < 4 ? a.rot_cos : a.rot_sin) + ((size_t)t * GR_TT + (wave & 3) * 8) * 32 + lane * 4;
      gr_glds16(src, (unsigned)(slot * GR_SLOT + GR_XBYTES + wave * 1024));
    }
  };
#pragma unroll
  for (int j = 0; j < GR_SLOTS; ++j)
    if (j < n) dma(j, j);
  if (n >= GR_SLOTS) gr_wait_vm<PER * (GR_SLOTS - 1)>();
  else gr_wait_vm<0>();
  __syncthreads();

  const int boff0 = l15 * 512;
  for (int i = 0; i < n; ++i) {
    const int t = first + i * per_group, slot = i % GR_SLOTS;
    const char* xs = smem + slot * GR_SLOT + boff0;
    f32x4 acc[2][GR_MT];
#pragma unroll
    for (int u = 0; u < 2; ++u)
#pragma unroll
      for (int m = 0; m < GR_MT; ++m) acc[u][m] = f32x4{0.f, 0.f, 0.f, 0.f};
#pragma unroll
    for (int ks = 0; ks < 8; ++ks) {
      typename P::vec8 bf[GR_MT];
#pragma unroll
      for (int m = 0; m < GR_MT; ++m) bf[m] = lds_frag<P>(xs, m * 16 * 512 + (((ks * 4 + g) ^ l15) << 4));
#pragma unroll
      for (int u = 0; u < 2; ++u)
#pragma unroll
        for (int m = 0; m < GR_MT; ++m) {
          if constexpr (TRANS) acc[u][m] = P::mfma(bf[m], wreg[u][ks], acc[u][m]);
          else acc[u][m] = P::mfma(wreg[u][ks], bf[m], acc[u][m]);
        }
    }
    const int behind = n - 2 - i;
    if (behind >= GR_SLOTS - 2) gr_wait_vm<PER * (GR_SLOTS - 2)>();
    else if (behind == 5) gr_wait_vm<PER * 5>();
    else if (behind == 4) gr_wait_vm<PER * 4>();
    else if (behind == 3) gr_wait_vm<PER * 3>();
    else if (behind == 2) gr_wait_vm<PER * 2>();
    else if (behind == 1) gr_wait_vm<PER>();
    else gr_wait_vm<0>();

    if constexpr (!TRANS) {
      const int co = cb * 64 + tp * 32 + g * 8;
#pragma unroll
      for (int m = 0; m < GR_MT; ++m) {
        const int row = t * GR_TT + m * 16 + l15;
        float v[8];
// ... 61 lines not shown
```

### airslam_amd/csrc/kernels.h

```cpp
#pragma once
#include <hip/hip_runtime.h>
#include <stdint.h>

namespace airfe {

enum Epi {
  EPI_STORE = 0,
  EPI_STORE_F32 = 1,
  EPI_RESID = 2,
  EPI_HEADS = 3,
  EPI_HEADS_T = 4,
  EPI_SOFTMAX_D2S = 5
};
enum Act { ACT_NONE = 0, ACT_RELU = 1 };

struct GemmArgs {
  const uint16_t* X1 = nullptr;
  const uint16_t* X2 = nullptr;
  int ld1 = 0, ld2 = 0, K1 = 0;
  const uint16_t* Wp = nullptr;
  const float* bias = nullptr;
  int M = 0;
  int N = 0;
  int cb_total = 0;
// ... 13 lines not shown
  int d2s_hc = 0, d2s_wc = 0;
  int* flag = nullptr;
};

void launch_gemm(int prec, int K, bool trans, const GemmArgs& a, hipStream_t st);
void launch_gemm8(int prec, int K, bool trans, const GemmArgs& a, hipStream_t st);
bool gemmr_applicable(int K, bool trans, const GemmArgs& a);
void launch_gemmr(int prec, bool trans, const GemmArgs& a, hipStream_t st);
bool gemmr_gather_applicable(int K, const GemmArgs& a);
void launch_gemmr_gather(int prec, const GemmArgs& a, hipStream_t st);
bool gemmr_gather128_applicable(const GemmArgs& a);
void launch_gemmr_gather128(int prec, const GemmArgs& a, hipStream_t st);
bool gemmr_pair_applicable(const GemmArgs& a, const GemmArgs& b);
void launch_gemmr_pair(int prec, const GemmArgs& a, const GemmArgs& b, hipStream_t st);

struct LgBlockFArgs {
  const uint16_t* attn;
  uint16_t* xb;
  float* x32;
  const uint16_t *wo, *w1, *w2;
  const float *bo, *b1, *gamma, *beta, *b2;
  int M;
  int tokens_per_wg = 128;
  int mixed = 0, n_cu = 0;
  int relu = 0;
  const uint16_t *nqk_w = nullptr, *nv_w = nullptr;
  const float *nqk_b = nullptr, *nv_b = nullptr, *rot_cos = nullptr, *rot_sin = nullptr;
  int nqk_n = 0, Np = 0, H = 4;
  uint16_t *q_out = nullptr, *k_out = nullptr, *vt_out = nullptr;
};
void launch_lg_blockf(int prec, const LgBlockFArgs& a, hipStream_t st);
bool lg_blockf_frag_weights();

struct ConvArgs {
  const uint16_t* X = nullptr;
  const uint16_t* Wp = nullptr;
  const float* bias = nullptr;
  uint16_t* Y = nullptr;
  int B = 0, H = 0, W = 0, CIN = 0, COUT = 0;
  int pool = 0;
  int out_pad = 1;
  int relu = 1;
  int wgs = 256;
  const float* img = nullptr;
  const float* w1a = nullptr;
  const float* b1a = nullptr;
};
void launch_conv3x3(int prec, const ConvArgs& a, hipStream_t st);
void launch_conv64r(int prec, const ConvArgs& a, hipStream_t st);
void launch_conv128r(int prec, const ConvArgs& a, hipStream_t st);

void launch_preprocess(const uint8_t* src, int B, int h, int w, int stride, size_t img_stride,
                       const int* xtab , const int* ytab , const float* lut ,
                       float* out, int RH, int RW, hipStream_t st, const uint8_t* src1 = nullptr, int n0 = 0);

void launch_remap_linear(const uint8_t* src, int B, int h, int w, int stride, size_t img_stride, const float* mapx, const float* mapy,
                         uint8_t* dst, int dstride, size_t dimg_stride, hipStream_t st);

void launch_softmax_d2s(const float* logits, int ldl, float* heat, int B, int HC, int WC, hipStream_t st);
void launch_l2norm256(float* d, int rows, hipStream_t st);
void launch_simple_nms(const float* heat, float* out, float* tmp, int B, int H, int W, int radius, hipStream_t st);
void launch_nms512_candidates(const float* heat, float* out, void* planes, int B, float thr, int border, unsigned long long* cand,
                              int* cand_cnt, int cand_cap, hipStream_t st);
void launch_candidates(const float* heat, int B, int H, int W, float thr, int border, unsigned long long* cand,
                       int* cand_cnt, int cand_cap, hipStream_t st);
void launch_candidates_nms3(const float* heat, int B, int H, int W, float thr, unsigned long long* cand, int* cand_cnt, int cand_cap, hipStream_t st);
struct SelectExtra {
  float* feat1 = nullptr; int* n_out1 = nullptr; int Bs = 0;
  int* desc_idx = nullptr; int HC = 0, WC = 0;
  int sort_all = 0;
};
void launch_select_list(const unsigned long long* cand, const int* cand_cnt, int cand_cap, int B, int W, int topk, int cap,
                        float* feat, int* n_out, hipStream_t st, const SelectExtra* ex = nullptr);
void launch_sample_desc(const float* desc, int B, int HC, int WC, float* feat, const int* n, int cap,
                        float w_scale, float h_scale, int normalise, hipStream_t st, int compact = 0, int* flag = nullptr,
                        float* feat1 = nullptr, const int* n1 = nullptr, int Bs = 0);
struct DescSample {
  float* feat = nullptr; float* feat1 = nullptr;
  const int* n = nullptr; const int* n1 = nullptr;
  int Bs = 0, B = 0, cap = 0, HC = 0, WC = 0;
  float w_scale = 1.f, h_scale = 1.f;
  int* flag = nullptr;
  float sx = 0.f, bx = 0.f, sy = 0.f, by = 0.f;
};
bool gemmr_gather_sample_applicable(const GemmArgs& a);
void launch_gemmr_gather_sample(int prec, const GemmArgs& a, const DescSample& ds, hipStream_t st);

struct LgPrepArgs {
  const float* f0; const float* f1;
  const int* n0; const int* n1;
  int ld, kp_off;
  int normalize;
  float cx, cy, linv;
  const float* wr;
  int B, cap, Np;
  float* x32; uint16_t* xb;
  float* rot_cos; float* rot_sin;
  int* lens;
  const float *f0x = nullptr, *f1x = nullptr; const int *n0x = nullptr, *n1x = nullptr;
  int slack_rows = 0;
};
void launch_lg_prepare(int prec, const LgPrepArgs& a, hipStream_t st);
void launch_attention32(int prec, const uint16_t* Q, const uint16_t* K, const uint16_t* Vt, uint16_t* O, const int* lens,
                        int S, int H, int Np, int cross, hipStream_t st);
void launch_ln_gelu(int prec, uint16_t* h, const float* gamma, const float* beta, int M, hipStream_t st);
void launch_rowdot256(const float* x32, const float* w, float b, float* z, int M, hipStream_t st);
void launch_sim(int prec, const uint16_t* md, float* sim, int B, int Np, hipStream_t st);
void launch_lg_assign(const float* sim, const float* z, const int* lens, int B, int Np, int cap, float thr,
                      float* rowlse, float* collse, float* scores_out, int* rowarg, float* rowval, int* colarg,
                      int32_t* idx, float* score, int* nmatch, hipStream_t st);

void launch_trace_hash(const void* p, unsigned unit_words, unsigned units, unsigned long long* out, hipStream_t st);
void launch_trace_digest(const unsigned long long* tab, const unsigned* off, int slots, unsigned long long* dig, hipStream_t st);
size_t lg_assign_part_floats(int B, int Np);
void launch_lg_assign_fused(int prec, const uint16_t* md, const float* z, const int* lens, int B, int Np, int cap, float thr, float* part, float* argpart,
                            float* rowlse, float* collse, float* sim_out, float* scores_out, int* rowarg, float* rowval, int* colarg, int32_t* idx,
                            float* score, int* nmatch, hipStream_t st);
void launch_lg_filter_scores(const float* scores, const int* lens, int B, int Np, int cap, float thr, int* rowarg, float* rowval,
                             int* colarg, int32_t* idx, float* score, int* nmatch, hipStream_t st);

constexpr int LINE_CNT_LD = 64;
constexpr int WF_WGS = 48;
void launch_wireframe(const float* iskeep, const float* imin, const float* imax, int n, int jn, int* table, int* keep,
                      int* pairs, int* rep, int cap, int line_cap, int* counts, bool counted, const float* juncs, const float* lines_pred, float* head4,
                      float* prop4, int B, size_t stage_stride, hipStream_t st);
constexpr int S1_WPAD = 128;
void launch_s1_junc_rows(const float* juncs, int jn, int* ridx, int B, size_t stage_stride, hipStream_t st);
void launch_s1_junc_proj(const float* juncs, const float* head, size_t head_img, int ps, const float* lrows, int jn, const float* w0t,
                         float* proj, int B, size_t stage_stride, hipStream_t st);
void launch_plnet_s1(const float* juncs, const float* lines_pred, const int* keep, const int* pairs, const int* rep,
                     const int* counts, const float* loi, size_t loi_img, const float* proj, const float* ta8, const float* thin,
                     const float* aux, const float* const* w, float* lines_adjusted, float* scores_line, int keep_cap, int line_cap, int B,
                     size_t stage_stride, hipStream_t st, int wgs = 0);
void launch_plnet_s1h(const int* pairs, const int* counts, const float* proj, const float* ta8, const uint16_t* const* wsplit, const float* const* w,
                      const float* lines_adjusted, const float* prop4, float* scores_line, int line_cap, int B, hipStream_t st, int wgs = 0);
void launch_s1h_junc_proj(const float* juncs, const float* lrows, int jn, const uint16_t* wa, const uint16_t* wb, float* proj, int B, size_t stage_stride,
                          hipStream_t st);
void launch_line_filter(const float* la, const float* sc, const int* counts, int border, float line_thr, float len_thr,
                        float w_scale, float h_scale, int R, unsigned char* jmap, int nj, double* lines_out, int capL, int* nlines, int* nfound,
                        int line_cap, int B, hipStream_t st);
void launch_zero16(void* p, size_t bytes, hipStream_t st);
void launch_junction_scan(const unsigned char* jmap, const float* heat, int R, int border, float* feat, int cap, int* n_kept, int* n_found,
                          int* wg_counts, int B, hipStream_t st, const unsigned long long* mask = nullptr);

struct GemmF32Args {
  const float* X1 = nullptr; int ld1 = 0, K1 = 0;
  const float* X2 = nullptr; int ld2 = 0;
  const float* W = nullptr;
  const float* bias = nullptr;
  float* Y = nullptr; int ldy = 0;
  int M = 0, N = 0, K = 0;
  float scale = 1.f;
  int relu = 0, accumulate = 0;
};
void launch_conv1a_f32(const float* img, const float* w, const float* bias, float* out, int B, int H, int W, hipStream_t st);
void launch_conv3x3_f32(const float* X, const float* Wt, const float* bias, float* Y, int B, int H, int W, int CIN, int COUT, int opad,
                        hipStream_t st);
void launch_maxpool2_f32(const float* X, float* Y, int B, int H, int W, int C, hipStream_t st);
void launch_gemm_f32(const GemmF32Args& a, hipStream_t st);
void launch_rotary_f32(float* qk, int ld, const float* rc, const float* rs, int M, hipStream_t st);
void launch_attention_f32(const float* Q, int ldq, const float* K, int ldk, const float* V, int ldv, float* O, const int* lens, int S, int H,
                          int Np, int cross, float scale, hipStream_t st);
void launch_ln_gelu_f32(float* h, const float* gamma, const float* beta, int M, hipStream_t st);

void launch_s0_decode(const float* head, int ld, int off, float* lines_pred, float* jloc, float* jnms, float* joff, float* thin, float* aux,
                      float* loi, float* ta8, int B, size_t stage_stride, hipStream_t st);
void launch_s0_head_decode(int prec, const uint16_t* X, const uint16_t* Wp, const float* bias, float* lines_pred, float* jloc, float* jnms,
                           float* joff, float* ta8, int B, size_t stage_stride, hipStream_t st, int wgs = 0);
void launch_s0_juncs(const float* sel, const int* n_sel, const float* joff, float* juncs, int jn, int sel_cap, int B, size_t stage_stride,
                     hipStream_t st);
bool launch_s0_j2l(const float* lines_pred, const float* juncs, int jn, int n, float thr, float* iskeep, float* imin, float* imax, int* counts,
                   int B, size_t stage_stride, int exact_all, hipStream_t st);

void launch_sg_prepare(int prec, const float* f0, const float* f1, const int* n0, const int* n1, int ld, int normalize,
                       float cx, float cy, float linv, const float* const* w, int B, int cap, int Np, float* x32,
                       uint16_t* xb, int* lens, uint16_t* h128, hipStream_t st);
void launch_sg_sinkhorn(const float* sim, const int* lens, int B, int Np, int Lz, float alpha, int iters, float* u, float* v,
                        float* Z, unsigned* counters , unsigned* fail_flag , float* xch,
                        hipStream_t st, int form = 0 , int* form_ran = nullptr);
void launch_sg_decode(const float* Z, const int* lens, int B, int Np, int Lz, float thr, int* idx0, float* max0, int* idx1,
                      int32_t* out0, int32_t* out1, float* ms0, float* ms1, hipStream_t st);

void launch_bow_transform(const float* feat, int ld, int off, int N, const float* node_desc, const int* first_child,
                          const int* n_children, const int* word_id, const float* weight, unsigned* out_word, float* out_weight, int* out_node ,
                          hipStream_t st);

struct PlAssignArgs {
  const double* lines = nullptr;
  const int* nlines = nullptr;
  const float* feat = nullptr;
  const int* npts = nullptr;
  int capL = 0, cap = 0, capE = 0;
  int* counts = nullptr;
  int* row_ptr = nullptr;
  int* pt_idx = nullptr;
  double* pt_dist = nullptr;
  int* total = nullptr;
};
void launch_assign_points_to_lines(const PlAssignArgs& a, int B, hipStream_t st);
struct MlArgs {
  const int *row_ptr0 = nullptr, *pt_idx0 = nullptr, *nlines0 = nullptr, *npts0 = nullptr;
  const int *row_ptr1 = nullptr, *pt_idx1 = nullptr, *nlines1 = nullptr, *npts1 = nullptr;
  const int* matches = nullptr;
  const int* nmatch = nullptr;
  int capL = 0, capE = 0, mcap = 0, W = 0, cap = 0;
  int filter_on = 0;
  double min_x_diff = 0, max_x_diff = 0, max_y_diff = 0;
  const float *feat0 = nullptr, *feat1 = nullptr;
  unsigned *bits0 = nullptr, *bits1 = nullptr;
  int* row_loc = nullptr;
  int* line_matches = nullptr;
};
void launch_match_lines(const MlArgs& a, int B, hipStream_t st);

#define FR_MAX_MATCHES 1024
struct FransacArgs {
  const float *f0 = nullptr, *f1 = nullptr;
  int cap = 0, mcap = 0;
  int32_t* idx = nullptr;
  float* score = nullptr;
  int* nmatch = nullptr;
  double* F = nullptr;
  int* scores = nullptr;
  int* state = nullptr;
};
void launch_fransac(const FransacArgs& a, int B, hipStream_t st);
// ... 203 lines not shown
```

### airslam_amd/csrc/kernels_ext.hip

```cpp
#include <float.h>
#include <algorithm>
#include <stdlib.h>

#include "common.h"
#include "kernels.h"

namespace airfe {

__device__ __forceinline__ unsigned block_excl_scan_1024(unsigned v, unsigned* wsum , unsigned* total) {
  const int tid = threadIdx.x, lane = tid & 63, wv = tid >> 6;
  unsigned incl = v;
#pragma unroll
  for (int o = 1; o < 64; o <<= 1) {
    const unsigned t = __shfl_up(incl, o);
    if (lane >= o) incl += t;
  }
  __syncthreads();
  if (lane == 63) wsum[wv] = incl;
  __syncthreads();
  unsigned off = 0, tot = 0;
  for (int w = 0; w < 16; ++w) {
    const unsigned t = wsum[w];
    if (w < wv) off += t;
    tot += t;
// ... 782 lines not shown
  S1Loi sl{nullptr, 0, 128 * 128, 1, proj, 300, ta8};
  const int gx = wgs > 0 ? wgs : (B == 1 ? 512 : (B <= 8 ? 128 : 64));
  hipLaunchKernelGGL(plnet_s1h_kernel, dim3(gx, B), dim3(256), 0, st, pairs, counts, sl, sw, lines_adjusted, prop4, scores_line, line_cap);
}

void launch_plnet_s1(const float* juncs, const float* lines_pred, const int* keep, const int* pairs, const int* rep,
                     const int* counts, const float* loi, size_t loi_img, const float* proj, const float* ta8, const float* thin,
                     const float* aux, const float* const* w, float* lines_adjusted, float* scores_line, int keep_cap, int line_cap, int B,
                     size_t stage_stride, hipStream_t st, int wgs) {
  S1Weights sw{w[0], w[1], w[2], w[3], w[4], w[5], w[6], w[7], w[8], w[9], w[10]};
  S1Loi sl{loi, loi_img, 128 * 128, 1, proj, 300, ta8};
  const int gx = wgs > 0 ? wgs : (B == 1 ? 512 : (B <= 8 ? 128 : 64));
  if (proj && ta8)
    hipLaunchKernelGGL(plnet_s1_kernel<true>, dim3(gx, B), dim3(256), 0, st, juncs, lines_pred, keep, pairs, rep, counts, sl, thin, aux, sw,
                       lines_adjusted, scores_line, keep_cap, line_cap, stage_stride);
  else
    hipLaunchKernelGGL(plnet_s1_kernel<false>, dim3(gx, B), dim3(256), 0, st, juncs, lines_pred, keep, pairs, rep, counts, sl, thin, aux, sw,
                       lines_adjusted, scores_line, keep_cap, line_cap, stage_stride);
}

__global__ __launch_bounds__(1024) void line_filter_kernel(const float* __restrict__ la, const float* __restrict__ sc,
                                                           const int* __restrict__ counts, int border, float line_thr,
                                                           float len_thr, float w_scale, float h_scale, int R,
                                                           unsigned char* __restrict__ jmap, double* __restrict__ lines_out,
                                                           int capL, int* __restrict__ nlines, int* __restrict__ nfound, int line_cap, int nj) {
  __shared__ unsigned wsum[16];
  const bool mark = (int)blockIdx.x < nj;
  {
    const size_t img = blockIdx.x;
    la += img * line_cap * 4; sc += img * line_cap; counts += img * LINE_CNT_LD; jmap += img * R * R;
    lines_out += img * capL * 4; nlines += img;
    if (nfound) nfound += img;
  }
  const int tid = threadIdx.x, m2 = counts[1];
  const int per = (m2 + 1023) / 1024, lo = tid * per, hi = min(lo + per, m2);
  const float thr2 = __fmul_rn(len_thr, len_thr);
  border = max(border, 0);
  unsigned cnt = 0;
  for (int pass = 0; pass < 2; ++pass) {
    unsigned off = 0, tot = 0;
    if (pass == 1) off = block_excl_scan_1024(cnt, wsum, &tot);
    for (int i = lo; i < hi; ++i) {
      const float s = sc[i];
      if (s < 0.5f) continue;
      const float x1 = __fmul_rn(la[i * 4], 4.f), y1 = __fmul_rn(la[i * 4 + 1], 4.f);
      const float x2 = __fmul_rn(la[i * 4 + 2], 4.f), y2 = __fmul_rn(la[i * 4 + 3], 4.f);
      if (pass == 0 && mark) {
        const int xi1 = (int)((double)x1 + 0.1), yi1 = (int)((double)y1 + 0.1);
        const int xi2 = (int)((double)x2 + 0.1), yi2 = (int)((double)y2 + 0.1);
        const bool p1 = xi1 > border && xi1 < R - border && yi1 > border && yi1 < R - border;
        const bool p2 = xi2 > border && xi2 < R - border && yi2 > border && yi2 < R - border;
        if (xi1 >= 0 && xi1 < R && yi1 >= 0 && yi1 < R) jmap[yi1 * R + xi1] = p1;
        if (xi2 >= 0 && xi2 < R && yi2 >= 0 && yi2 < R) jmap[yi2 * R + xi2] = p2;
      }
      if (s < line_thr) continue;
      const float dx = __fsub_rn(x2, x1), dy = __fsub_rn(y2, y1);
      const float l2 = __fadd_rn(__fmul_rn(dx, dx), __fmul_rn(dy, dy));
      if (l2 < thr2) continue;
      if (pass == 0) ++cnt;
      else {
        if (off < (unsigned)capL) {
          lines_out[(size_t)off * 4 + 0] = (double)x1 * (double)w_scale;
          lines_out[(size_t)off * 4 + 1] = (double)y1 * (double)h_scale;
          lines_out[(size_t)off * 4 + 2] = (double)x2 * (double)w_scale;
          lines_out[(size_t)off * 4 + 3] = (double)y2 * (double)h_scale;
        }
        ++off;
      }
    }
    if (pass == 1 && tid == 0) {
      *nlines = min((int)tot, capL);
      if (nfound) *nfound = (int)tot;
    }
  }
}

void launch_line_filter(const float* la, const float* sc, const int* counts, int border, float line_thr, float len_thr,
                        float w_scale, float h_scale, int R, unsigned char* jmap, int nj, double* lines_out, int capL, int* nlines, int* nfound,
                        int line_cap, int B, hipStream_t st) {
  hipLaunchKernelGGL(line_filter_kernel, dim3(B), dim3(1024), 0, st, la, sc, counts, border, line_thr, len_thr, w_scale,
                     h_scale, R, jmap, lines_out, capL, nlines, nfound, line_cap, nj);
}

__global__ __launch_bounds__(256) void zero16_kernel(uint4* __restrict__ p, size_t n16) {
  for (size_t i = (size_t)blockIdx.x * 256 + threadIdx.x; i < n16; i += (size_t)gridDim.x * 256) p[i] = make_uint4(0, 0, 0, 0);
}
void launch_zero16(void* p, size_t bytes, hipStream_t st) {
  const size_t n16 = bytes / 16;
  if (n16 == 0) return;
  hipLaunchKernelGGL(zero16_kernel, dim3((unsigned)std::min<size_t>((n16 + 255) / 256, 4096)), dim3(256), 0, st, reinterpret_cast<uint4*>(p), n16);
}

constexpr int JS_WGS = 64, JS_PT = 16;

__device__ __forceinline__ unsigned js_mask16(const unsigned char* __restrict__ jmap, int i0, int N, int R, int border) {
  unsigned m = 0;
  if (i0 + JS_PT <= N && (R % JS_PT) == 0 && (i0 % JS_PT) == 0) {
    const uint4 q = *reinterpret_cast<const uint4*>(jmap + i0);
    const unsigned w[4] = {q.x, q.y, q.z, q.w};
    const int y = i0 / R, x0 = i0 - y * R;
    const bool yin = y >= border && y < R - border;
#pragma unroll
    for (int k = 0; k < JS_PT; ++k) {
      const int x = x0 + k;
      if (((w[k >> 2] >> (8 * (k & 3))) & 0xFFu) && yin && x >= border && x < R - border) m |= 1u << k;
    }
  } else {
    for (int k = 0; k < JS_PT; ++k) {
      const int i = i0 + k;
      if (i >= N) break;
      const int y = i / R, x = i - y * R;
      if (jmap[i] && x >= border && x < R - border && y >= border && y < R - border) m |= 1u << k;
    }
  }
  return m;
}

__global__ __launch_bounds__(256) void junction_count_kernel(const unsigned char* __restrict__ jmap, int R, int border, int* __restrict__ wg_counts) {
  __shared__ int wsum[4];
  const int N = R * R, per_wg = (N + JS_WGS - 1) / JS_WGS, per = (per_wg + 255) / 256;
  jmap += (size_t)blockIdx.y * N; wg_counts += (size_t)blockIdx.y * JS_WGS;
  border = max(border, 0);
  int cnt = 0;
  const int lo = blockIdx.x * per_wg + threadIdx.x * per, hi = min(min(lo + per, (blockIdx.x + 1) * per_wg), N);
  for (int i0 = lo; i0 < hi; i0 += JS_PT) cnt += __builtin_popcount(js_mask16(jmap, i0, min(hi, N), R, border));
  cnt = (int)wave_sum((float)cnt);
  if ((threadIdx.x & 63) == 0) wsum[threadIdx.x >> 6] = cnt;
  __syncthreads();
  if (threadIdx.x == 0) wg_counts[blockIdx.x] = wsum[0] + wsum[1] + wsum[2] + wsum[3];
}

__global__ __launch_bounds__(256) void junction_emit_kernel(const unsigned char* __restrict__ jmap, const float* __restrict__ heat, int R, int border,
                                                            float* __restrict__ feat, int cap, int* __restrict__ n_kept, int* __restrict__ n_found,
                                                            const int* __restrict__ wg_counts, const unsigned long long* __restrict__ mask) {
  __shared__ int wsum[4];
  const int N = R * R, per_wg = (N + JS_WGS - 1) / JS_WGS, per = (per_wg + 255) / 256;
  {
    const size_t img = blockIdx.y;
    jmap += img * N; heat += img * N; feat += img * cap * 259; wg_counts += img * JS_WGS;
    if (mask) mask += img * (size_t)(R / 8) * (R / 8);
    n_kept += img; n_found += img;
  }
  border = max(border, 0);
  int base = 0;
  for (int w = 0; w < (int)blockIdx.x; ++w) base += wg_counts[w];
  const int lo = blockIdx.x * per_wg + threadIdx.x * per, hi = min(min(lo + per, (blockIdx.x + 1) * per_wg), N);
  int cnt = 0;
  for (int i0 = lo; i0 < hi; i0 += JS_PT) cnt += __builtin_popcount(js_mask16(jmap, i0, min(hi, N), R, border));
  int incl = cnt;
#pragma unroll
  for (int o = 1; o < 64; o <<= 1) {
    const int t = __shfl_up(incl, o);
    if ((int)(threadIdx.x & 63) >= o) incl += t;
  }
  if ((threadIdx.x & 63) == 63) wsum[threadIdx.x >> 6] = incl;
  __syncthreads();
  int off = base + incl - cnt;
  for (int w = 0; w < (int)(threadIdx.x >> 6); ++w) off += wsum[w];
  for (int i0 = lo; i0 < hi; i0 += JS_PT) {
    unsigned m = js_mask16(jmap, i0, min(hi, N), R, border);
    while (m) {
      const int k = __builtin_ctz(m);
      m &= m - 1;
      const int i = i0 + k, y = i / R, x = i - y * R;
      if (off < cap) {
        float* f = feat + (size_t)off * 259;
// ... 699 lines not shown
```

### airslam_amd/csrc/kernels_gemmr_sample.hip

```cpp
#include "gemmr_body.h"

namespace airfe {

template <class P>
__global__ __launch_bounds__(512, 1) void gemmr_gather_kernel_sample(GemmArgs a, int ntiles, DescSample ds) {
  extern __shared__ __attribute__((aligned(16))) char smem[];
  gemmr_body<P, false, false, true, true>(a, smem, 0, blockIdx.x, gridDim.x, ntiles, &ds);
}


constexpr int GR_SAMPLE_MAX_TILES = 60;
bool gemmr_gather_sample_applicable(const GemmArgs& a) {
  const int wgs = std::max(a.gr_wgs, 1);
  return gemmr_gather_applicable(256, a) && a.rowidx && (a.M / GR_TT + wgs - 1) / wgs <= GR_SAMPLE_MAX_TILES;
}

void launch_gemmr_gather_sample(int prec, const GemmArgs& a, const DescSample& ds0, hipStream_t st) {
  DescSample ds = ds0;
  desc_grid_coeffs(ds.HC, ds.WC, ds.sx, ds.bx, ds.sy, ds.by);
  const int ntiles = a.M / GR_TT;
  const int nwg = std::max(std::min(a.gr_wgs, ntiles), 1);
  const int nmax = (ntiles + nwg - 1) / nwg;
  const int lds = GR_SAMPLE_SLOTS * GR_XBYTES + GR_STAGE_BYTES + nmax * (GR_TT * 4 + 8 * (int)sizeof(GrKeypoint));
  if (prec == 1) {
    static PerDeviceOnce once;
    if (auto once_token = once.first()) (void)hipFuncSetAttribute(reinterpret_cast<const void*>(gemmr_gather_kernel_sample<PF16>), hipFuncAttributeMaxDynamicSharedMemorySize, 160 * 1024);
    hipLaunchKernelGGL(gemmr_gather_kernel_sample<PF16>, dim3((unsigned)nwg), dim3(512), lds, st, a, ntiles, ds);
  } else {
    static PerDeviceOnce once;
    if (auto once_token = once.first()) (void)hipFuncSetAttribute(reinterpret_cast<const void*>(gemmr_gather_kernel_sample<PBF16>), hipFuncAttributeMaxDynamicSharedMemorySize, 160 * 1024);
    hipLaunchKernelGGL(gemmr_gather_kernel_sample<PBF16>, dim3((unsigned)nwg), dim3(512), lds, st, a, ntiles, ds);
  }
}

}
```

### include/airfe_debug.h

```cpp
#ifndef AIRFE_DEBUG_H_
#define AIRFE_DEBUG_H_
#include "airfe.h"
#ifdef __cplusplus
extern "C" {
#endif

int airfe_debug_detector_maps(airfe_ctx* ctx, int B, float* heat_raw, float* heat_nms, float* desc);
int airfe_debug_lightglue_scores(airfe_ctx* ctx, const float* f0, int n0, const float* f1, int n1, float* scores);
int airfe_debug_lg_filter(airfe_ctx* ctx, const float* scores, int n0, int n1, int32_t* idx, float* score, int cap, int* nmatch);
int airfe_debug_sg_decode(airfe_ctx* ctx, const float* Z, int n0, int n1, int32_t* idx0, int32_t* idx1, double* ms0, double* ms1);
int airfe_debug_sg_sinkhorn(airfe_ctx* ctx, const float* sim, const int* lens , int B, int ld ,
                            float alpha, int iters, int form , float* Z , int* form_ran);
int airfe_debug_superglue_scores(airfe_ctx* ctx, const float* f0, int n0, const float* f1, int n1, float* scores);
int airfe_debug_plnet_stage0(airfe_ctx* ctx, float* juncs_pred, float* lines_pred, float* iskeep, float* idx_min, float* idx_max,
                             float* loi, float* thin, float* aux, float* jloc, float* joff);
int airfe_debug_plnet_j2l(airfe_ctx* ctx, int fast, float* iskeep, float* idx_min, float* idx_max);
int airfe_debug_plnet_s1(airfe_ctx* ctx, const airfe_plnet_stage0* stage0, float* lines_adjusted, float* scores_line,
                         int cap, int* m2);
int airfe_debug_plnet_s1_last(airfe_ctx* ctx, float* lines_adjusted, float* scores_line, int cap, int* m2);
int airfe_debug_preprocess(airfe_ctx* ctx, const uint8_t* gray, int h, int w, int stride, float* out);
int airfe_debug_conv3x3(airfe_ctx* ctx, const float* x, int B, int cin, int H, int W, const float* w, const float* b,
                        int cout, int pool, float* y);
int airfe_debug_gemm(airfe_ctx* ctx, const float* x, int M, int K, const float* w, const float* b, int N, int relu, float* y);
typedef struct airfe_debug_conv_args {
// ... 53 lines not shown
  int nqk_n;
  const float *nqk_w, *nqk_b;
  const float *nv_w, *nv_b;
  const float *rot_cos, *rot_sin;
  int Np;
  float *q, *k, *vt;
  int rows_past[5];
} airfe_debug_lg_block_args;
int airfe_debug_lg_block(airfe_ctx* ctx, airfe_debug_lg_block_args* a);
int airfe_debug_ln_gelu(airfe_ctx* ctx, int prec, float* h, const float* gamma, const float* beta, int M);
int airfe_debug_attention(airfe_ctx* ctx, const float* q, const float* k, const float* v, const int* lens, int S, int H, int n, int cross, float* out);
typedef struct airfe_debug_attn_args {
  int prec;
  int S, H, n, cross;
  const float *q, *k, *v;
  const int* lens;
  int canary, raw;
  float* out;
  int Np, rows_past;
} airfe_debug_attn_args;
int airfe_debug_attention_args(airfe_ctx* ctx, airfe_debug_attn_args* a);
typedef struct airfe_debug_lg_prepare_args {
  int prec;
  int B, cap, ld, kp_off;
  int normalize;
  float cx, cy, linv;
  const float *f0, *f1;
  const int *n0, *n1;
  const float* wr;
  const float *f0x, *f1x;
  int n0x, n1x;
  int slack_rows;
  int rows;
  float *x32, *xb;
  float *rot_cos, *rot_sin;
  int* lens;
  int rows_past;
} airfe_debug_lg_prepare_args;
int airfe_debug_lg_prepare(airfe_ctx* ctx, airfe_debug_lg_prepare_args* a);
typedef struct airfe_debug_lg_assign_args {
  int prec, B, n;
  const float* md;
  const float* x32;
  const float* w;
  float b;
  const int* lens;
  int cap;
  float thr;
  int form;
  const float* pad;
  float* z;
  float *sim, *scores;
  float *rowlse, *collse, *rowval;
  int32_t *rowarg, *colarg;
  int32_t* idx;
  float* score;
  int32_t* nmatch;
} airfe_debug_lg_assign_args;
int airfe_debug_lg_assign(airfe_ctx* ctx, airfe_debug_lg_assign_args* a);
typedef struct airfe_debug_detector_tail_args {
  int B, Bs, h, w, cap;
  const float* heat;
  const float* act;
  float *feat, *feat1;
  int *n, *n1;
  float* nms_map;
  unsigned long long* keep;
  int* cand_cnt;
  int nms_map_written;
} airfe_debug_detector_tail_args;
int airfe_debug_detector_tail(airfe_ctx* ctx, airfe_debug_detector_tail_args* a);
typedef struct airfe_debug_line_post_args {
  int B, nj, ld, h, w, capL, capJ, from_plane;
  const float *la, *sc;
  const int* m2;
  const float* heat;
  double* lines;
  int *nlines, *nfound;
  float* junc;
  int *njunc, *jfound;
  const unsigned char* jmap;
} airfe_debug_line_post_args;
int airfe_debug_line_post(airfe_ctx* ctx, airfe_debug_line_post_args* a);
int airfe_debug_junctions_topk(airfe_ctx* ctx, const float* jloc, const float* joff, int B, float* juncs_pred);
typedef struct airfe_debug_line_mid_args {
  int B, j2l, s1_form, wgs;
  const float* juncs_pred;
  const float* lines_pred;
  const float *thin, *aux;
  const float* loi;
  const float *iskeep_in, *idx_min_in, *idx_max_in;
  float *iskeep, *idx_min, *idx_max;
  int32_t* counts;
  int32_t* keep;
  int32_t *pairs, *rep;
  float *head4, *prop4;
  int32_t* ridx;
  float* proj;
  float *lines_adjusted, *scores_line;
  int32_t* table_dirty;
} airfe_debug_line_mid_args;
int airfe_debug_line_mid(airfe_ctx* ctx, airfe_debug_line_mid_args* a);
typedef struct airfe_debug_s0_decode_args {
  int B, mode;
  int ld, off;
  int want_ta8, want_loi, want_jnms;
  int prec, wgs;
  const float* rows;
  const float* x;
  const float *w, *b;
  size_t stage_floats;
  float* stage;
  float *jloc, *joff, *jnms;
  float* ta8;
  float* loi;
  float* head_rows;
} airfe_debug_s0_decode_args;
int airfe_debug_s0_decode(airfe_ctx* ctx, airfe_debug_s0_decode_args* a);
int airfe_debug_fail_next_launch(airfe_ctx* ctx, int stage);
int airfe_debug_trace(airfe_ctx* ctx, int on);
int airfe_debug_trace_stop(airfe_ctx* ctx, int slot);
int airfe_debug_trace_buffer(airfe_ctx* ctx, int slot, void* host, size_t bytes);
int airfe_debug_trace_slots(airfe_ctx* ctx);
int airfe_debug_trace_slot(airfe_ctx* ctx, int i, char* name, int name_cap, unsigned* off, unsigned* units, unsigned* unit_words);
int airfe_debug_trace_read(airfe_ctx* ctx, void* stream, unsigned long long* digests, unsigned long long* table);

#ifdef __cplusplus
}
#endif
#endif
```

Before: 7985.

## Fuse junction marking and scan into line filter, sample descriptors inside gather GEMM

The line-filter kernel now marks junction endpoints in a shared-memory bitmap and compacts the junction list in the same block. This replaces zeroing a full-resolution junction map, a separate junction scan, and the dense descriptor head over every cell. A new gather-GEMM variant computes descriptors only for tiles covering live junctions and samples them directly. The fused path applies only under specific conditions (2-byte precision, radius-4 NMS, no NMS map, gather stream enabled). It adds complexity and depends on the junction count fitting the tile limit.

```diff
diff --git a/airslam_amd/_lib.py b/airslam_amd/_lib.py
--- a/airslam_amd/_lib.py
+++ b/airslam_amd/_lib.py
@@ -102,6 +102,11 @@
 class DebugLinePostArgs(C.Structure):
     _fields_ = ([(n, C.c_int) for n in ("B", "nj", "ld", "h", "w", "capL", "capJ", "from_plane")]
                 + [(n, C.c_void_p) for n in ("la", "sc", "m2", "heat", "lines", "nlines", "nfound", "junc", "njunc", "jfound", "jmap")])
+
+
+class DebugJunctionTailArgs(C.Structure):
+    _fields_ = ([(n, C.c_int) for n in ("B", "nj", "ld", "h", "w", "capL", "capJ")]
+                + [(n, C.c_void_p) for n in ("la", "sc", "m2", "heat", "act", "lines", "nlines", "nfound", "junc", "njunc", "jfound")] + [("fused", C.c_int)])
 
 
 class DebugLineMidArgs(C.Structure):
@@ -262,6 +267,7 @@
     "airfe_debug_sg_sinkhorn": (C.c_int, [C.c_void_p, C.c_void_p, C.c_void_p, C.c_int, C.c_int, C.c_float, C.c_int, C.c_int, C.c_void_p, C.POINTER(C.c_int)]),
     "airfe_debug_detector_tail": (C.c_int, [C.c_void_p, C.POINTER(DebugDetectorTailArgs)]),
     "airfe_debug_line_post": (C.c_int, [C.c_void_p, C.POINTER(DebugLinePostArgs)]),
+    "airfe_debug_junction_tail": (C.c_int, [C.c_void_p, C.POINTER(DebugJunctionTailArgs)]),
     "airfe_debug_junctions_topk": (C.c_int, [C.c_void_p, C.c_void_p, C.c_void_p, C.c_int, C.c_void_p]),
     "airfe_debug_line_mid": (C.c_int, [C.c_void_p, C.POINTER(DebugLineMidArgs)]),
     "airfe_debug_s0_decode": (C.c_int, [C.c_void_p, C.POINTER(DebugS0DecodeArgs)]),
diff --git a/airslam_amd/api.py b/airslam_amd/api.py
--- a/airslam_amd/api.py
+++ b/airslam_amd/api.py
@@ -461,6 +461,21 @@
         self._chk(self._l.airfe_debug_line_post(self._h, C.byref(a)), "airfe_debug_line_post")
         return out
 
+    def debug_junction_tail(self, la, sc, m2, heat, act, cap_lines, cap_junctions, nj=None, h=512, w=512, sentinel=7.0):
+        la, sc, heat = np.ascontiguousarray(la, np.float32), np.ascontiguousarray(sc, np.float32), np.ascontiguousarray(heat, np.float32)
+        act = np.ascontiguousarray(act, np.float32)
+        m2 = np.ascontiguousarray(m2, np.int32).reshape(-1)
+        b, ld = sc.shape
+        nj = b if nj is None else int(nj)
+        assert la.shape == (b, ld, 4) and heat.shape == (b, 512, 512) and act.shape == (b, 64, 64, 256) and len(m2) == b
+        out = {"lines": np.full((b, cap_lines, 4), sentinel, np.float64), "nlines": np.full((b,), -1, np.int32), "nfound": np.full((b,), -1, np.int32),
+               "junc": np.full((nj, cap_junctions, FEAT), sentinel, np.float32), "njunc": np.full((nj,), -1, np.int32), "jfound": np.full((nj,), -1, np.int32)}
+        a = _lib.DebugJunctionTailArgs(B=b, nj=nj, ld=ld, h=int(h), w=int(w), capL=int(cap_lines), capJ=int(cap_junctions), la=la.ctypes.data, sc=sc.ctypes.data,
+                                       m2=m2.ctypes.data, heat=heat.ctypes.data, act=act.ctypes.data, **{k: v.ctypes.data for k, v in out.items()})
+        self._chk(self._l.airfe_debug_junction_tail(self._h, C.byref(a)), "airfe_debug_junction_tail")
+        out["fused"] = bool(a.fused)
+        return out
+
     def debug_line_mid(self, juncs_pred, lines_pred, thin, aux, loi, iskeep=None, idx_min=None, idx_max=None, j2l=0, s1_form=2, wgs=0):
         f = lambda x: np.ascontiguousarray(x, np.float32)
         juncs_pred, lines_pred, thin, aux, loi = f(juncs_pred), f(lines_pred), f(thin), f(aux), f(loi)
diff --git a/airslam_amd/csrc/airfe.hip b/airslam_amd/csrc/airfe.hip
--- a/airslam_amd/csrc/airfe.hip
+++ b/airslam_amd/csrc/airfe.hip
@@ -811,7 +811,7 @@
   if (nj < 0 || nj > B || (nj > 0 && (!d_junc || !d_njunc || capJ < 1))) return fail(c, "detect_plnet_batch: bad junction arguments");
   if ((phase & 1) && line_branch_dev(c, st, 0, B, false)) return 1;
   bool partial = false;
-  if ((phase & 2) && nj > 0 && !c->desc_dense_valid) {
+  if ((phase & 2) && nj > 0 && !c->desc_dense_valid && !(phase == 3 && junction_tail_fused(c, nj, capJ))) {
     dense_desc_head(c, nj, st);
     c->desc_dense_valid = true;
     partial = nj != c->last_B;
diff --git a/airslam_amd/csrc/airfe_debug.hip b/airslam_amd/csrc/airfe_debug.hip
--- a/airslam_amd/csrc/airfe_debug.hip
+++ b/airslam_amd/csrc/airfe_debug.hip
@@ -119,7 +119,10 @@
 template <class T>
 static T* dbg_canary(airfe_ctx* tmp, size_t n) {
   T* p = dalloc<T>(tmp, n, false);
-  if (p) (void)hipMemset(p, 0xFF, std::max<size_t>(n, 1) * sizeof(T));
+  if (p) {
+    (void)hipMemset(p, 0xFF, std::max<size_t>(n, 1) * sizeof(T));
+    (void)hipStreamSynchronize(nullptr);
+  }
   return p;
 }
 static void dbg_back2(const std::vector<uint16_t>& v, size_t n, int prec, float* out) {
@@ -748,6 +751,75 @@
   HIPCHK(c, hipStreamSynchronize(st));
   if (launch_status(c)) return 1;
   if (saturation_status(c)) return 1;
+  HIPCHK(c, hipMemcpy(a->lines, dlines, (size_t)B * capL * 32, hipMemcpyDeviceToHost));
+  HIPCHK(c, hipMemcpy(a->nlines, dcnt, (size_t)B * 4, hipMemcpyDeviceToHost));
+  HIPCHK(c, hipMemcpy(a->nfound, dcnt + B, (size_t)B * 4, hipMemcpyDeviceToHost));
+  if (nj > 0) {
+    HIPCHK(c, hipMemcpy(a->junc, djunc, (size_t)nj * capJ * AIRFE_FEAT_DIM * 4, hipMemcpyDeviceToHost));
+    HIPCHK(c, hipMemcpy(a->njunc, dcnt + 2 * B, (size_t)nj * 4, hipMemcpyDeviceToHost));
+    HIPCHK(c, hipMemcpy(a->jfound, dcnt + 3 * B, (size_t)nj * 4, hipMemcpyDeviceToHost));
+  }
+  return 0;
+} AIRFE_CATCH(c)
+
+int airfe_debug_junction_tail(airfe_ctx* c, airfe_debug_junction_tail_args* a) try {
+  AIRFE_ENTER(c);
+  if (!c->has_sp || !c->has_s1 || !c->s1_la || !c->jmap) return fail(c, "debug_junction_tail: the line path is not loaded (cfg.plnet_s1_pack)");
+  if (c->prec != 0 && c->prec != 1) return fail(c, "debug_junction_tail drives the 2-byte detector (cfg.precision fp16 / bf16)");
+  if (c->cfg.nms_radius != 4) return fail(c, "debug_junction_tail: the keep plane exists on the radius-4 path only");
+  if (!a || !a->la || !a->sc || !a->m2 || !a->heat || !a->act || !a->lines || !a->nlines || !a->nfound) return fail(c, "debug_junction_tail: null argument");
+  const int B = a->B, nj = a->nj, ld = a->ld, capL = a->capL, capJ = a->capJ, R = AIRFE_INTERNAL_SIZE;
+  if (B < 1 || B > c->Lmax || B > c->Bmax || nj < 0 || nj > B || ld < 1 || ld > LINE_CAP || capL < 1 || capJ < 1 || a->h < 1 || a->w < 1)
+    return fail(c, "debug_junction_tail: bad argument (1 <= B <= max_batch, 0 <= nj <= B, 1 <= ld <= 45056, capL, capJ >= 1)");
+  if (nj > 0 && (!a->junc || !a->njunc || !a->jfound)) return fail(c, "debug_junction_tail: nj > 0 needs the junction outputs");
+  for (int b = 0; b < B; ++b)
+    if (a->m2[b] < 0 || a->m2[b] > ld) return fail(c, "debug_junction_tail: every m2 must lie in 0 .. ld");
+  const size_t px = (size_t)B * R * R, cells = (size_t)B * (R / 8) * (R / 8);
+  for (size_t i = 0; i < px; ++i)
+    if (!(a->heat[i] >= 0.f && a->heat[i] <= 1.f)) return fail(c, "debug_junction_tail: scores must lie in [0, 1]");
+  std::vector<uint16_t> act(cells * 256);
+  for (size_t i = 0; i < act.size(); ++i) act[i] = cvt2(a->act[i], c->prec);
+  DbgTmp t;
+  double* dlines = dupload(&t.h, std::vector<double>(a->lines, a->lines + (size_t)B * capL * 4));
+  float* djunc = nj > 0 ? dupload(&t.h, std::vector<float>(a->junc, a->junc + (size_t)nj * capJ * AIRFE_FEAT_DIM)) : nullptr;
+  int* dcnt = dbg_canary<int>(&t.h, (size_t)4 * B);
+  if (!dlines || (nj > 0 && !djunc) || !dcnt) return fail(c, "debug_junction_tail: allocation failed");
+  hipStream_t st = c->stream;
+  clear_saturation(c);
+  std::vector<int> counts((size_t)B * LINE_CNT_LD, 0);
+  for (int b = 0; b < B; ++b) {
+    counts[(size_t)b * LINE_CNT_LD + 1] = a->m2[b];
+    HIPCHK(c, hipMemcpyAsync(c->s1_la + (size_t)b * LINE_CAP * 4, a->la + (size_t)b * ld * 4, (size_t)ld * 16, hipMemcpyHostToDevice, st));
+    HIPCHK(c, hipMemcpyAsync(c->s1_sc + (size_t)b * LINE_CAP, a->sc + (size_t)b * ld, (size_t)ld * 4, hipMemcpyHostToDevice, st));
+  }
+  HIPCHK(c, hipMemcpyAsync(c->wf_counts, counts.data(), counts.size() * 4, hipMemcpyHostToDevice, st));
+  c->wf_counted = false;
+  HIPCHK(c, hipMemcpyAsync(c->heat, a->heat, px * 4, hipMemcpyHostToDevice, st));
+  HIPCHK(c, hipMemcpyAsync(c->aDa, act.data(), act.size() * 2, hipMemcpyHostToDevice, st));
+  c->nms_map_valid = B <= 2;
+  launch_nms512_candidates(c->heat, c->nms_map_valid ? c->heat_nms : nullptr, c->nms_mask, B, c->cfg.keypoint_threshold, c->cfg.remove_borders, c->cand, c->cand_cnt,
+                           R * R, st);
+  c->desc_dense_valid = false;
+  c->last_B = B;
+  int rc = 0;
+  if (B <= 2) {
+    rc = dense_desc_head(c, B, st);
+    c->desc_dense_valid = true;
+  }
+  const bool fused = junction_tail_fused(c, nj, capJ);
+  bool partial = false;
+  if (!rc && nj > 0 && !c->desc_dense_valid && !fused) {
+    rc = dense_desc_head(c, nj, st);
+    c->desc_dense_valid = true;
+    partial = nj != B;
+  }
+  if (!rc && nj > 0 && !fused) launch_zero16(c->jmap, (size_t)nj * R * R, st);
+  if (!rc) rc = line_post_dev(c, 0, B, a->h, a->w, dlines, capL, dcnt, dcnt + B, djunc, capJ, dcnt + 2 * B, dcnt + 3 * B, nj, st, 3, fused);
+  if (partial) c->desc_dense_valid = false;
+  HIPCHK(c, hipStreamSynchronize(st));
+  if (rc || launch_status(c)) return 1;
+  if (saturation_status(c)) return 1;
+  a->fused = fused ? 1 : 0;
   HIPCHK(c, hipMemcpy(a->lines, dlines, (size_t)B * capL * 32, hipMemcpyDeviceToHost));
   HIPCHK(c, hipMemcpy(a->nlines, dcnt, (size_t)B * 4, hipMemcpyDeviceToHost));
   HIPCHK(c, hipMemcpy(a->nfound, dcnt + B, (size_t)B * 4, hipMemcpyDeviceToHost));
diff --git a/airslam_amd/csrc/airfe_detect.hip b/airslam_amd/csrc/airfe_detect.hip
--- a/airslam_amd/csrc/airfe_detect.hip
+++ b/airslam_amd/csrc/airfe_detect.hip
@@ -256,16 +256,33 @@
   return launch_status(c);
 }
 
+static void junction_gemm_args(airfe_ctx* c, int i0, int nj, float* d_junc, int capJ, const int* d_njunc, int h, int w, GemmArgs& g, DescSample& ds) {
+  const int R = AIRFE_INTERNAL_SIZE;
+  g.X1 = c->aDa + (size_t)i0 * (R / 8) * (R / 8) * 256; g.ld1 = 256; g.K1 = 256; g.Wp = c->cDb.w; g.bias = c->cDb.b;
+  g.M = (capJ + 7) / 8 * nj * 32; g.N = 256; g.cb_total = c->cDb.cbt; g.epi = EPI_STORE_F32; g.out = c->desc; g.ldo = 256;
+  g.gr_wgs = c->gemmr_wgs;
+  ds.feat = d_junc; ds.n = d_njunc; ds.Bs = nj; ds.B = nj; ds.cap = capJ; ds.HC = R / 8; ds.WC = R / 8;
+  ds.w_scale = (float)w / (float)R; ds.h_scale = (float)h / (float)R; ds.flag = nullptr;
+  ds.junc = 1;
+}
+bool junction_tail_fused(airfe_ctx* c, int nj, int capJ) {
+  if (nj < 1 || capJ < 1 || c->prec == 2 || c->cfg.nms_radius != 4 || c->nms_map_valid || c->desc_dense_valid || !c->desc_gather_stream) return false;
+  GemmArgs g;
+  DescSample ds;
+  junction_gemm_args(c, 0, nj, nullptr, capJ, nullptr, 1, 1, g, ds);
+  return g.M >= c->gemmr_min && gemmr_gather_sample_junc_applicable(g, ds);
+}
+
 int line_tail_dev(airfe_ctx* c, int i0, int nb, const float* loi_chw, int h, int w, double* d_lines, int capL, int* d_nlines, int* d_lfound,
                   float* d_junc, int capJ, int* d_njunc, int* d_jfound, int nj, hipStream_t st, int phase) {
   if (!c->has_s1) return fail(c, "PLNet stage-1 weights were not loaded (cfg.plnet_s1_pack)");
   if (nb < 1 || nb > c->Lmax || nj < 0 || nj > nb) return fail(c, "line path: image range outside the arena");
   const int R = AIRFE_INTERNAL_SIZE, NP = KEEP_CAP;
   float* d = c->s0_stage;
-  const float ws = (float)w / (float)R, hs = (float)h / (float)R;
+  const bool fused = phase == 3 && junction_tail_fused(c, nj, capJ);
   if (phase & 1) {
   hipStream_t s4 = st;
-  if (nj > 0) launch_zero16(c->jmap, (size_t)nj * R * R, s4);
+  if (nj > 0 && !fused) launch_zero16(c->jmap, (size_t)nj * R * R, s4);
   {
   ProfScope ps(c, ST_PL_STAGE1, st, 0, (double)nb * 49152 * 12);
   launch_wireframe(d + SG_KEEP, d + SG_MIN, d + SG_MAX, NP, 300, c->wf_table, c->wf_keep, c->wf_pairs, c->wf_rep, KEEP_CAP, LINE_CAP,
@@ -298,16 +315,39 @@
                       d + SG_AUX, c->s1_w, c->s1_la, c->s1_sc, KEEP_CAP, LINE_CAP, nb, SG_STRIDE, st);
   }
   }
-  ProfScope ps(c, ST_PL_FILTER, st, 0, (double)nb * R * R);
-  launch_line_filter(c->s1_la, c->s1_sc, c->wf_counts, c->cfg.remove_borders, c->cfg.line_threshold, c->cfg.line_length_threshold, ws, hs, R,
-                     c->jmap, nj, d_lines, capL, d_nlines, d_lfound, LINE_CAP, nb, st);
+  }
+  return line_post_dev(c, i0, nb, h, w, d_lines, capL, d_nlines, d_lfound, d_junc, capJ, d_njunc, d_jfound, nj, st, phase, fused);
+}
+
+int line_post_dev(airfe_ctx* c, int i0, int nb, int h, int w, double* d_lines, int capL, int* d_nlines, int* d_lfound, float* d_junc, int capJ, int* d_njunc,
+                  int* d_jfound, int nj, hipStream_t st, int phase, bool fused) {
+  const int R = AIRFE_INTERNAL_SIZE;
+  const float ws = (float)w / (float)R, hs = (float)h / (float)R;
+  const bool from_mask = c->cfg.nms_radius > 0 && !c->nms_map_valid;
+  const float* hsel = (c->cfg.nms_radius > 0 && !from_mask ? c->heat_nms : c->heat) + (size_t)i0 * R * R;
+  const unsigned long long* mask = from_mask ? reinterpret_cast<const unsigned long long*>(c->nms_mask) + (size_t)i0 * (R / 8) * (R / 8) : nullptr;
+  if (fused) {
+    if (phase != 3 || nj < 1) return fail(c, "line path: the fused junction tail runs both phases in one call");
+    {
+      ProfScope ps(c, ST_PL_FILTER, st, 0, (double)nb * LINE_CAP * 20);
+      launch_line_filter_junc(c->s1_la, c->s1_sc, c->wf_counts, c->cfg.remove_borders, c->cfg.line_threshold, c->cfg.line_length_threshold, ws, hs, d_lines, capL,
+                              d_nlines, d_lfound, LINE_CAP, nb, nj, hsel, mask, d_junc, capJ, d_njunc, d_jfound, st);
+    }
+    GemmArgs g;
+    DescSample ds;
+    junction_gemm_args(c, i0, nj, d_junc, capJ, d_njunc, h, w, g, ds);
+    ProfScope ps(c, ST_HEAD_GEMM, st, 2.0 * g.M * 256 * 256, (double)g.M * 512);
+    launch_gemmr_gather_sample_junc(c->prec, g, ds, st);
+    return launch_status(c);
+  }
+  if (phase & 1) {
+    ProfScope ps(c, ST_PL_FILTER, st, 0, (double)nb * R * R);
+    launch_line_filter(c->s1_la, c->s1_sc, c->wf_counts, c->cfg.remove_borders, c->cfg.line_threshold, c->cfg.line_length_threshold, ws, hs, R,
+                       c->jmap, nj, d_lines, capL, d_nlines, d_lfound, LINE_CAP, nb, st);
   }
   if ((phase & 2) && nj > 0) {
     ProfScope ps(c, ST_PL_FILTER, st, 0, (double)nj * R * R * 2);
-    const bool from_mask = c->cfg.nms_radius > 0 && !c->nms_map_valid;
     if (from_mask && c->cfg.nms_radius != 4) return fail(c, "line path: the NMS'd score maps of this batch were not kept");
-    const float* hsel = (c->cfg.nms_radius > 0 && !from_mask ? c->heat_nms : c->heat) + (size_t)i0 * R * R;
-    const unsigned long long* mask = from_mask ? reinterpret_cast<const unsigned long long*>(c->nms_mask) + (size_t)i0 * (R / 8) * (R / 8) : nullptr;
     launch_junction_scan(c->jmap, hsel, R, c->cfg.remove_borders, d_junc, capJ, d_njunc, d_jfound, c->d_njunc + 2 * c->Lmax, nj, st, mask);
     if (!c->desc_dense_valid) return fail(c, "line path: the dense descriptor map of this batch was not made");
     launch_sample_desc(c->desc + (size_t)i0 * (R / 8) * (R / 8) * 256, nj, R / 8, R / 8, d_junc, d_njunc, capJ, ws, hs,
diff --git a/airslam_amd/csrc/airfe_host.h b/airslam_amd/csrc/airfe_host.h
--- a/airslam_amd/csrc/airfe_host.h
+++ b/airslam_amd/csrc/airfe_host.h
@@ -351,6 +351,9 @@
 int line_branch_dev(airfe_ctx* c, hipStream_t st, int i0, int nb, bool chw);
 int line_tail_dev(airfe_ctx* c, int i0, int nb, const float* loi_chw, int h, int w, double* d_lines, int capL, int* d_nlines, int* d_lfound,
                   float* d_junc, int capJ, int* d_njunc, int* d_jfound, int nj, hipStream_t st, int phase = 3);
+bool junction_tail_fused(airfe_ctx* c, int nj, int capJ);
+int line_post_dev(airfe_ctx* c, int i0, int nb, int h, int w, double* d_lines, int capL, int* d_nlines, int* d_lfound, float* d_junc, int capJ, int* d_njunc,
+                  int* d_jfound, int nj, hipStream_t st, int phase, bool fused);
 void trace(airfe_ctx* c, hipStream_t st, const char* what, size_t li, const char* blk, const void* p, size_t words, unsigned unit_words);
 int trace_finish(airfe_ctx* c, hipStream_t st);
 int run_linear(airfe_ctx* c, const LinW& w, const uint16_t* x1, int ld1, int K1, const uint16_t* x2, int ld2, int M, int epi, int act, void* out,
diff --git a/airslam_amd/csrc/gemmr_body.h b/airslam_amd/csrc/gemmr_body.h
--- a/airslam_amd/csrc/gemmr_body.h
+++ b/airslam_amd/csrc/gemmr_body.h
@@ -26,10 +26,21 @@
 constexpr int GR_STAGE_BYTES = GR_TT * GR_STAGE_LD * 4;
 struct GrKeypoint { float x, y; int row, second; };
 
-template <class P, bool TRANS, bool ROT, bool GATHER = false, bool SAMPLE = false>
+__device__ __forceinline__ int gr_junc_live_tiles(const DescSample& ds, int ntiles) {
+  int kmax = 0;
+  for (int b = threadIdx.x & 63; b < ds.B; b += 64) kmax = max(kmax, min(ds.n[b], ds.cap));
+#pragma unroll
+  for (int o = 32; o > 0; o >>= 1) kmax = max(kmax, __shfl_xor(kmax, o));
+  kmax = __builtin_amdgcn_readfirstlane(kmax);
+  return min(ntiles, ((kmax + 7) >> 3) * ds.B);
+}
+
+template <class P, bool TRANS, bool ROT, bool GATHER = false, bool SAMPLE = false, bool JUNC = false>
 __device__ __forceinline__ void gemmr_body(const GemmArgs& a, char* smem, int group, int first, int per_group, int ntiles, const DescSample* dsp = nullptr) {
   static_assert(!GATHER || (!TRANS && !ROT), "the gather form is the plain K = 256 linear with fp32 rows out");
   static_assert(!SAMPLE || GATHER, "sampling finishes the gather form's rows");
+  static_assert(!JUNC || SAMPLE, "the junction layout is a slot layout of the sampling form");
+  if constexpr (JUNC) ntiles = gr_junc_live_tiles(*dsp, ntiles);
   constexpr int GR_SLOT = GR_XBYTES + (ROT ? GR_RBYTES : 0);
   constexpr int GR_SLOTS = ROT ? 6 : SAMPLE ? GR_SAMPLE_SLOTS : 8;
   constexpr int PER = ROT ? 3 : 2;
@@ -60,13 +71,32 @@
   [[maybe_unused]] float* stage = reinterpret_cast<float*>(smem + GR_SLOTS * GR_SLOT);
   [[maybe_unused]] int* idx_lds = reinterpret_cast<int*>(smem + GR_SLOTS * GR_SLOT + (SAMPLE ? GR_STAGE_BYTES : 0));
   [[maybe_unused]] GrKeypoint* kp_lds = reinterpret_cast<GrKeypoint*>(idx_lds + n * GR_TT);
-  if constexpr (GATHER) {
+  if constexpr (GATHER && !JUNC) {
     for (int e = tid; e < n * GR_TT; e += 512) {
       const int r = (first + (e >> 5) * per_group) * GR_TT + (e & 31);
       idx_lds[e] = a.rowidx ? a.rowidx[r] : r;
     }
   }
-  if constexpr (SAMPLE) {
+  if constexpr (JUNC) {
+    const DescSample& ds = *dsp;
+    const int cells = ds.HC * ds.WC;
+    for (int e = tid; e < n * 8; e += 512) {
+      const int T = first + (e >> 3) * per_group;
+      const int b = T % ds.B, k = (T / ds.B) * 8 + (e & 7);
+      GrKeypoint kp{0.f, 0.f, -1, 0};
+      int r0 = 0, r1 = 0, r2 = 0, r3 = 0;
+      if (k < ds.cap && k < ds.n[b]) {
+        const float* f = ds.feat + ((size_t)b * ds.cap + k) * 259;
+        kp.row = b * ds.cap + k;
+        kp.x = f[1];
+        kp.y = f[2];
+        const DescTaps t = desc_taps(kp.x, kp.y, ds.sx, ds.bx, ds.sy, ds.by, ds.HC, ds.WC);
+        r0 = b * cells + t.c[0]; r1 = b * cells + t.c[1]; r2 = b * cells + t.c[2]; r3 = b * cells + t.c[3];
+      }
+      kp_lds[e] = kp;
+      *reinterpret_cast<int4*>(idx_lds + e * 4) = make_int4(r0, r1, r2, r3);
+    }
+  } else if constexpr (SAMPLE) {
     const DescSample& ds = *dsp;
     for (int e = tid; e < n * 8; e += 512) {
       const int s = (first + (e >> 3) * per_group) * 8 + (e & 7);
diff --git a/airslam_amd/csrc/kernels.h b/airslam_amd/csrc/kernels.h
--- a/airslam_amd/csrc/kernels.h
+++ b/airslam_amd/csrc/kernels.h
@@ -119,9 +119,12 @@
   float w_scale = 1.f, h_scale = 1.f;
   int* flag = nullptr;
   float sx = 0.f, bx = 0.f, sy = 0.f, by = 0.f;
+  int junc = 0;
 };
 bool gemmr_gather_sample_applicable(const GemmArgs& a);
 void launch_gemmr_gather_sample(int prec, const GemmArgs& a, const DescSample& ds, hipStream_t st);
+bool gemmr_gather_sample_junc_applicable(const GemmArgs& a, const DescSample& ds);
+void launch_gemmr_gather_sample_junc(int prec, const GemmArgs& a, const DescSample& ds, hipStream_t st);
 
 struct LgPrepArgs {
   const float* f0; const float* f1;
@@ -179,6 +182,9 @@
 void launch_zero16(void* p, size_t bytes, hipStream_t st);
 void launch_junction_scan(const unsigned char* jmap, const float* heat, int R, int border, float* feat, int cap, int* n_kept, int* n_found,
                           int* wg_counts, int B, hipStream_t st, const unsigned long long* mask = nullptr);
+void launch_line_filter_junc(const float* la, const float* sc, const int* counts, int border, float line_thr, float len_thr, float w_scale, float h_scale,
+                             double* lines_out, int capL, int* nlines, int* nfound, int line_cap, int B, int nj, const float* heat, const unsigned long long* mask,
+                             float* feat, int capJ, int* n_kept, int* n_jfound, hipStream_t st);
 
 struct GemmF32Args {
   const float* X1 = nullptr; int ld1 = 0, K1 = 0;
diff --git a/airslam_amd/csrc/kernels_ext.hip b/airslam_amd/csrc/kernels_ext.hip
--- a/airslam_amd/csrc/kernels_ext.hip
+++ b/airslam_amd/csrc/kernels_ext.hip
@@ -888,6 +888,110 @@
                      h_scale, R, jmap, lines_out, capL, nlines, nfound, line_cap, nj);
 }
 
+constexpr int LFJ_R = 512, LFJ_WORDS = LFJ_R * LFJ_R / 32;
+__global__ __launch_bounds__(1024) void line_filter_junc_kernel(const float* __restrict__ la, const float* __restrict__ sc, const int* __restrict__ counts, int border,
+                                                                float line_thr, float len_thr, float w_scale, float h_scale, double* __restrict__ lines_out, int capL,
+                                                                int* __restrict__ nlines, int* __restrict__ nfound, int line_cap, int nj,
+                                                                const float* __restrict__ heat, const unsigned long long* __restrict__ mask,
+                                                                float* __restrict__ feat, int capJ, int* __restrict__ n_kept, int* __restrict__ n_jfound) {
+  constexpr int R = LFJ_R;
+  __shared__ unsigned wsum[16];
+  __shared__ __attribute__((aligned(16))) unsigned bits[LFJ_WORDS];
+  const bool mark = (int)blockIdx.x < nj;
+  {
+    const size_t img = blockIdx.x;
+    la += img * line_cap * 4; sc += img * line_cap; counts += img * LINE_CNT_LD;
+    lines_out += img * capL * 4; nlines += img;
+    if (nfound) nfound += img;
+    if (mark) {
+      heat += img * R * R; feat += img * capJ * 259; n_kept += img; n_jfound += img;
+      if (mask) mask += img * (size_t)(R / 8) * (R / 8);
+    }
+  }
+  const int tid = threadIdx.x, m2 = counts[1];
+  const int per = (m2 + 1023) / 1024, lo = tid * per, hi = min(lo + per, m2);
+  const float thr2 = __fmul_rn(len_thr, len_thr);
+  border = max(border, 0);
+  if (mark) {
+#pragma unroll
+    for (int k = 0; k < 2; ++k) reinterpret_cast<uint4*>(bits)[k * 1024 + tid] = make_uint4(0, 0, 0, 0);
+    __syncthreads();
+  }
+  unsigned cnt = 0;
+  for (int pass = 0; pass < 2; ++pass) {
+    unsigned off = 0, tot = 0;
+    if (pass == 1) off = block_excl_scan_1024(cnt, wsum, &tot);
+    for (int i = lo; i < hi; ++i) {
+      const float s = sc[i];
+      if (s < 0.5f) continue;
+      const float x1 = __fmul_rn(la[i * 4], 4.f), y1 = __fmul_rn(la[i * 4 + 1], 4.f);
+      const float x2 = __fmul_rn(la[i * 4 + 2], 4.f), y2 = __fmul_rn(la[i * 4 + 3], 4.f);
+      if (pass == 0 && mark) {
+        const int xi1 = (int)((double)x1 + 0.1), yi1 = (int)((double)y1 + 0.1);
+        const int xi2 = (int)((double)x2 + 0.1), yi2 = (int)((double)y2 + 0.1);
+        const bool p1 = xi1 > border && xi1 < R - border && yi1 > border && yi1 < R - border;
+        const bool p2 = xi2 > border && xi2 < R - border && yi2 > border && yi2 < R - border;
+        if (p1) atomicOr(&bits[(yi1 * R + xi1) >> 5], 1u << (xi1 & 31));
+        if (p2) atomicOr(&bits[(yi2 * R + xi2) >> 5], 1u << (xi2 & 31));
+      }
+      if (s < line_thr) continue;
+      const float dx = __fsub_rn(x2, x1), dy = __fsub_rn(y2, y1);
+      const float l2 = __fadd_rn(__fmul_rn(dx, dx), __fmul_rn(dy, dy));
+      if (l2 < thr2) continue;
+      if (pass == 0) ++cnt;
+      else {
+        if (off < (unsigned)capL) {
+          lines_out[(size_t)off * 4 + 0] = (double)x1 * (double)w_scale;
+          lines_out[(size_t)off * 4 + 1] = (double)y1 * (double)h_scale;
+          lines_out[(size_t)off * 4 + 2] = (double)x2 * (double)w_scale;
+          lines_out[(size_t)off * 4 + 3] = (double)y2 * (double)h_scale;
+        }
+        ++off;
+      }
+    }
+    if (pass == 1 && tid == 0) {
+      *nlines = min((int)tot, capL);
+      if (nfound) *nfound = (int)tot;
+    }
+  }
+  if (!mark) return;
+  __syncthreads();
+  unsigned w[8];
+  {
+    const uint4 q0 = reinterpret_cast<const uint4*>(bits)[tid * 2], q1 = reinterpret_cast<const uint4*>(bits)[tid * 2 + 1];
+    w[0] = q0.x; w[1] = q0.y; w[2] = q0.z; w[3] = q0.w; w[4] = q1.x; w[5] = q1.y; w[6] = q1.z; w[7] = q1.w;
+  }
+  unsigned jc = 0;
+#pragma unroll
+  for (int k = 0; k < 8; ++k) jc += __builtin_popcount(w[k]);
+  unsigned jtot = 0;
+  unsigned joff = block_excl_scan_1024(jc, wsum, &jtot);
+#pragma unroll
+  for (int k = 0; k < 8; ++k) {
+    unsigned m = w[k];
+    while (m) {
+      const int bit = __builtin_ctz(m);
+      m &= m - 1;
+      const int i = (tid * 8 + k) * 32 + bit, y = i / R, x = i - y * R;
+      if (joff < (unsigned)capJ) {
+        float* f = feat + (size_t)joff * 259;
+        f[0] = (!mask || ((mask[(size_t)(y >> 3) * (R / 8) + (x >> 3)] >> (8 * (y & 7) + (x & 7))) & 1ull)) ? heat[i] : 0.f;
+        f[1] = (float)x;
+        f[2] = (float)y;
+      }
+      ++joff;
+    }
+  }
+  if (tid == 0) { *n_kept = min((int)jtot, capJ); *n_jfound = (int)jtot; }
+}
+
+void launch_line_filter_junc(const float* la, const float* sc, const int* counts, int border, float line_thr, float len_thr, float w_scale, float h_scale,
+                             double* lines_out, int capL, int* nlines, int* nfound, int line_cap, int B, int nj, const float* heat, const unsigned long long* mask,
+                             float* feat, int capJ, int* n_kept, int* n_jfound, hipStream_t st) {
+  hipLaunchKernelGGL(line_filter_junc_kernel, dim3(B), dim3(1024), 0, st, la, sc, counts, border, line_thr, len_thr, w_scale, h_scale, lines_out, capL, nlines,
+                     nfound, line_cap, nj, heat, mask, feat, capJ, n_kept, n_jfound);
+}
+
 __global__ __launch_bounds__(256) void zero16_kernel(uint4* __restrict__ p, size_t n16) {
   for (size_t i = (size_t)blockIdx.x * 256 + threadIdx.x; i < n16; i += (size_t)gridDim.x * 256) p[i] = make_uint4(0, 0, 0, 0);
 }
diff --git a/airslam_amd/csrc/kernels_gemmr_sample.hip b/airslam_amd/csrc/kernels_gemmr_sample.hip
--- a/airslam_amd/csrc/kernels_gemmr_sample.hip
+++ b/airslam_amd/csrc/kernels_gemmr_sample.hip
@@ -8,6 +8,11 @@
   gemmr_body<P, false, false, true, true>(a, smem, 0, blockIdx.x, gridDim.x, ntiles, &ds);
 }
 
+template <class P>
+__global__ __launch_bounds__(512, 1) void gemmr_gather_kernel_sample_junc(GemmArgs a, int ntiles, DescSample ds) {
+  extern __shared__ __attribute__((aligned(16))) char smem[];
+  gemmr_body<P, false, false, true, true, true>(a, smem, 0, blockIdx.x, gridDim.x, ntiles, &ds);
+}
 
 constexpr int GR_SAMPLE_MAX_TILES = 60;
 bool gemmr_gather_sample_applicable(const GemmArgs& a) {
@@ -33,4 +38,28 @@
   }
 }
 
+bool gemmr_gather_sample_junc_applicable(const GemmArgs& a, const DescSample& ds) {
+  const int wgs = std::max(a.gr_wgs, 1);
+  return gemmr_gather_applicable(256, a) && !a.rowidx && ds.junc && !ds.feat1 && ds.B >= 1 && ds.cap >= 1 && a.M == (ds.cap + 7) / 8 * ds.B * GR_TT &&
+         (a.M / GR_TT + wgs - 1) / wgs <= GR_SAMPLE_MAX_TILES;
 }
+
+void launch_gemmr_gather_sample_junc(int prec, const GemmArgs& a, const DescSample& ds0, hipStream_t st) {
+  DescSample ds = ds0;
+  desc_grid_coeffs(ds.HC, ds.WC, ds.sx, ds.bx, ds.sy, ds.by);
+  const int ntiles = a.M / GR_TT;
+  const int nwg = std::max(std::min(a.gr_wgs, ntiles), 1);
+  const int nmax = (ntiles + nwg - 1) / nwg;
+  const int lds = GR_SAMPLE_SLOTS * GR_XBYTES + GR_STAGE_BYTES + nmax * (GR_TT * 4 + 8 * (int)sizeof(GrKeypoint));
+  if (prec == 1) {
+    static PerDeviceOnce once;
+    if (auto once_token = once.first()) (void)hipFuncSetAttribute(reinterpret_cast<const void*>(gemmr_gather_kernel_sample_junc<PF16>), hipFuncAttributeMaxDynamicSharedMemorySize, 160 * 1024);
+    hipLaunchKernelGGL(gemmr_gather_kernel_sample_junc<PF16>, dim3((unsigned)nwg), dim3(512), lds, st, a, ntiles, ds);
+  } else {
+    static PerDeviceOnce once;
+    if (auto once_token = once.first()) (void)hipFuncSetAttribute(reinterpret_cast<const void*>(gemmr_gather_kernel_sample_junc<PBF16>), hipFuncAttributeMaxDynamicSharedMemorySize, 160 * 1024);
+    hipLaunchKernelGGL(gemmr_gather_kernel_sample_junc<PBF16>, dim3((unsigned)nwg), dim3(512), lds, st, a, ntiles, ds);
+  }
+}
+
+}
diff --git a/include/airfe_debug.h b/include/airfe_debug.h
--- a/include/airfe_debug.h
+++ b/include/airfe_debug.h
@@ -159,6 +159,19 @@
   const unsigned char* jmap;
 } airfe_debug_line_post_args;
 int airfe_debug_line_post(airfe_ctx* ctx, airfe_debug_line_post_args* a);
+typedef struct airfe_debug_junction_tail_args {
+  int B, nj, ld, h, w, capL, capJ;
+  const float *la, *sc;
+  const int* m2;
+  const float* heat;
+  const float* act;
+  double* lines;
+  int *nlines, *nfound;
+  float* junc;
+  int *njunc, *jfound;
+  int fused;
+} airfe_debug_junction_tail_args;
+int airfe_debug_junction_tail(airfe_ctx* ctx, airfe_debug_junction_tail_args* a);
 int airfe_debug_junctions_topk(airfe_ctx* ctx, const float* jloc, const float* joff, int B, float* juncs_pred);
 typedef struct airfe_debug_line_mid_args {
   int B, j2l, s1_form, wgs;
```

Result: faster. 8121, median of 6 (+1.7%).
